# faithokamoto/panman

Measured on NVIDIA B200. Metric: fitch_sankoff_node_column_updates_per_sec, higher is better.
Workload: dtype u16 Fitch sets as 16 bit-planes

## Files before the change

panman_b200/csrc/plane_math.h:

```cpp
#pragma once
#include <stdint.h>

#if defined(__CUDACC__)
#define PMB_HD __host__ __device__ __forceinline__
#else
#define PMB_HD inline
#endif

namespace pmb {

PMB_HD void decode16(const uint32_t c[4], uint32_t d[16]) {
    uint32_t lo[4], hi[4];
    lo[0] = ~c[0] & ~c[1];
    lo[1] = c[0] & ~c[1];
    lo[2] = ~c[0] & c[1];
    lo[3] = c[0] & c[1];
    hi[0] = ~c[2] & ~c[3];
    hi[1] = c[2] & ~c[3];
    hi[2] = ~c[2] & c[3];
    hi[3] = c[2] & c[3];
#pragma unroll
    for (int k = 0; k < 16; k++) d[k] = lo[k & 3] & hi[k >> 2];
}

// ... 10 lines not shown

PMB_HD void lowest16(const uint32_t X[16], uint32_t code[4], uint32_t& any) {
    uint32_t any2[8], any4[4], any8[2];
    uint32_t b0_2[4], b0_3[2], b1_3[2];
#pragma unroll
    for (int j = 0; j < 8; j++) any2[j] = X[2 * j] | X[2 * j + 1];
#pragma unroll
    for (int j = 0; j < 4; j++) {
        any4[j] = any2[2 * j] | any2[2 * j + 1];
        b0_2[j] = (any2[2 * j] & ~X[4 * j]) | (~any2[2 * j] & ~X[4 * j + 2]);
    }
#pragma unroll
    for (int j = 0; j < 2; j++) {
        any8[j] = any4[2 * j] | any4[2 * j + 1];
        b0_3[j] = (any4[2 * j] & b0_2[2 * j]) | (~any4[2 * j] & b0_2[2 * j + 1]);
        b1_3[j] = (any4[2 * j] & ~any2[4 * j]) | (~any4[2 * j] & ~any2[4 * j + 2]);
    }
    any = any8[0] | any8[1];
    code[0] = (any8[0] & b0_3[0]) | (~any8[0] & b0_3[1]);
    code[1] = (any8[0] & b1_3[0]) | (~any8[0] & b1_3[1]);
    code[2] = (any8[0] & ~any4[0]) | (~any8[0] & ~any4[2]);
    code[3] = ~any8[0];
#pragma unroll
    for (int b = 0; b < 4; b++) code[b] &= any;
}

PMB_HD uint32_t differs4(const uint32_t a[4], const uint32_t b[4]) {
    return (a[0] ^ b[0]) | (a[1] ^ b[1]) | (a[2] ^ b[2]) | (a[3] ^ b[3]);
}

PMB_HD uint32_t less4(const uint32_t a[4], const uint32_t b[4]) {
    uint32_t lt = 0;
#pragma unroll
    for (int k = 0; k < 4; k++) {
        uint32_t x = a[k] ^ b[k];
        lt = (x & b[k]) | (~x & lt);
    }
    return lt;
}


struct FitchFold {
    uint32_t A[16], O[16];
    PMB_HD void reset() {
#pragma unroll
        for (int k = 0; k < 16; k++) { A[k] = 0xFFFFFFFFu; O[k] = 0; }
    }
    PMB_HD void add_set(const uint32_t S[16]) {
#pragma unroll
        for (int k = 0; k < 16; k++) { A[k] &= S[k]; O[k] |= S[k]; }
    }
    PMB_HD void add_leaf(const uint32_t c[4], uint32_t present) {
        uint32_t d[16];
        decode16(c, d);
#pragma unroll
        for (int k = 0; k < 16; k++) { A[k] &= d[k] & present; O[k] |= d[k] & present; }
    }
    PMB_HD void finish(uint32_t S[16]) const {
        uint32_t nz = 0;
#pragma unroll
        for (int k = 0; k < 16; k++) nz |= A[k];
#pragma unroll
        for (int k = 0; k < 16; k++) S[k] = A[k] | (O[k] & ~nz);
    }
};

PMB_HD void fitch_leaf_leaf(const uint32_t c1[4], const uint32_t c2[4], uint32_t S[16]) {
    uint32_t d1[16], d2[16];
    decode16(c1, d1);
    decode16(c2, d2);
    const uint32_t ne = differs4(c1, c2);
#pragma unroll
    for (int k = 0; k < 16; k++) S[k] = d1[k] | (d2[k] & ne);
}
PMB_HD void fitch_leaf_set(const uint32_t c[4], const uint32_t X[16], uint32_t S[16]) {
    uint32_t d[16];
    decode16(c, d);
    const uint32_t hit = mux16(X, c);
#pragma unroll
    for (int k = 0; k < 16; k++) S[k] = d[k] | (X[k] & ~hit);
}
PMB_HD void fitch_set_set(const uint32_t X[16], const uint32_t Y[16], uint32_t S[16]) {
    uint32_t nz = 0;
#pragma unroll
    for (int k = 0; k < 16; k++) nz |= X[k] & Y[k];
#pragma unroll
    for (int k = 0; k < 16; k++) S[k] = (X[k] & Y[k]) | ((X[k] | Y[k]) & ~nz);
}

struct FitchInterval {
    uint32_t lo[16], hi[16];
    PMB_HD void reset() {
#pragma unroll
        for (int k = 0; k < 16; k++) { lo[k] = 0; hi[k] = 0xFFFFFFFFu; }
    }
    PMB_HD void step(const uint32_t A[16], const uint32_t O[16]) {
        uint32_t sure = 0, maybe = 0, one = 0, two = 0;
#pragma unroll
        for (int k = 0; k < 16; k++) {
            const uint32_t h = hi[k] & A[k];
            sure |= lo[k] & A[k];
            maybe |= h;
            two |= one & h;
            one |= h;
        }
        const uint32_t single = one & ~two, uni = ~maybe, either = maybe & ~sure;
#pragma unroll
        for (int k = 0; k < 16; k++) {
            const uint32_t l = lo[k], h = hi[k];
            lo[k] = (sure & l & A[k]) | (uni & (l | O[k])) | (either & single & h & A[k] & (l | O[k]));
            hi[k] = (sure & h & A[k]) | (~sure & (h | O[k]));
        }
    }
    PMB_HD uint32_t open() const {
        uint32_t d = 0;
#pragma unroll
        for (int k = 0; k < 16; k++) d |= lo[k] ^ hi[k];
        return d;
    }
};

PMB_HD void fitch_candidates_step(uint32_t Q[16], const uint32_t S[16]) {
    uint32_t outside = 0;
#pragma unroll
    for (int k = 0; k < 16; k++) outside |= Q[k] & ~S[k];
    uint32_t seen = 0;
#pragma unroll
    for (int k = 0; k < 16; k++) {
        const uint32_t lowest = S[k] & ~seen;
        seen |= S[k];
        Q[k] = (Q[k] & S[k]) | (outside & lowest);
    }
}
PMB_HD uint32_t candidates_open(const uint32_t Q[16]) {
    uint32_t one = 0, two = 0;
#pragma unroll
    for (int k = 0; k < 16; k++) {
        two |= one & Q[k];
        one |= Q[k];
    }
    return ~one | two;
}
PMB_HD void encode16(const uint32_t d[16], uint32_t c[4]) {
    c[0] = c[1] = c[2] = c[3] = 0;
#pragma unroll
    for (int k = 0; k < 16; k++) {
        if (k & 1) c[0] |= d[k];
        if (k & 2) c[1] |= d[k];
        if (k & 4) c[2] |= d[k];
        if (k & 8) c[3] |= d[k];
    }
}

PMB_HD void fitch_assign(const uint32_t S[16], const uint32_t P[4], uint32_t pvis, uint32_t F[4], uint32_t& vis) {
    uint32_t low[4], any;
    lowest16(S, low, any);
    uint32_t hit = mux16(S, P);
    vis = pvis & any;
#pragma unroll
    for (int b = 0; b < 4; b++) F[b] = ((hit & P[b]) | (~hit & low[b])) & vis;
}

PMB_HD void fitch_assign_root(const uint32_t S[16], const uint32_t ov[4], uint32_t ov_valid, uint32_t colmask,
                              uint32_t F[4], uint32_t& vis) {
    uint32_t low[4], any;
    lowest16(S, low, any);
    vis = (ov_valid | any) & colmask;
#pragma unroll
    for (int b = 0; b < 4; b++) F[b] = ((ov_valid & ov[b]) | (~ov_valid & low[b])) & vis;
}

PMB_HD void mutation_type(const uint32_t P[4], const uint32_t F[4], uint32_t& t0, uint32_t& t1) {
    uint32_t pgap = ~(P[0] | P[1] | P[2] | P[3]);
    uint32_t fgap = ~(F[0] | F[1] | F[2] | F[3]);
    t1 = pgap;
    t0 = ~pgap & fgap;
}


PMB_HD uint32_t sankoff_none(const uint32_t G[16], const uint32_t H[16]) { return H[0] & ~G[0]; }

template <int B>
struct SankoffFold {
    uint32_t cnt[16][B];
    uint32_t all_none;
    PMB_HD void reset() {
#pragma unroll
        for (int k = 0; k < 16; k++)
#pragma unroll
            for (int b = 0; b < B; b++) cnt[k][b] = 0;
        all_none = 0xFFFFFFFFu;
    }
    PMB_HD void add_bit(int k, uint32_t g) {
        uint32_t carry = g;
#pragma unroll
        for (int b = 0; b < B; b++) {
            uint32_t t = cnt[k][b] & carry;
            cnt[k][b] ^= carry;
            carry = t;
        }
    }
    PMB_HD void add_set(const uint32_t G[16], uint32_t none) {
#pragma unroll
        for (int k = 0; k < 16; k++) add_bit(k, G[k] & ~none);
        all_none &= none;
    }
    PMB_HD void add_leaf(const uint32_t c[4], uint32_t present) {
        uint32_t d[16];
        decode16(c, d);
#pragma unroll
        for (int k = 0; k < 16; k++) add_bit(k, ~d[k] & present);
        all_none &= ~present;
    }
    PMB_HD void finish(uint32_t G[16], uint32_t H[16]) const {
        uint32_t alive[16];
        uint32_t minbit[B];
#pragma unroll
        for (int k = 0; k < 16; k++) alive[k] = 0xFFFFFFFFu;
#pragma unroll
        for (int b = B - 1; b >= 0; b--) {
            uint32_t anyzero = 0;
#pragma unroll
            for (int k = 0; k < 16; k++) anyzero |= alive[k] & ~cnt[k][b];
            minbit[b] = ~anyzero;
#pragma unroll
            for (int k = 0; k < 16; k++) alive[k] &= ~(anyzero & cnt[k][b]);
        }
        uint32_t mp1[B];
        uint32_t carry = 0xFFFFFFFFu;
#pragma unroll
        for (int b = 0; b < B; b++) {
            mp1[b] = minbit[b] ^ carry;
            carry &= minbit[b];
        }
#pragma unroll
        for (int k = 0; k < 16; k++) {
            uint32_t eq1 = ~carry;
#pragma unroll
            for (int b = 0; b < B; b++) eq1 &= ~(cnt[k][b] ^ mp1[b]);
            G[k] = ~alive[k];
            H[k] = ~alive[k] & ~eq1;
        }
        H[0] |= all_none;
        G[0] &= ~all_none;
    }
};

PMB_HD void sankoff_pair(const uint32_t g1[16], uint32_t none1, const uint32_t g2[16], uint32_t none2, uint32_t G[16],
                         uint32_t H[16]) {
    uint32_t any0 = 0, all2 = 0xFFFFFFFFu;
#pragma unroll
    for (int k = 0; k < 16; k++) {
        const uint32_t a = g1[k] & ~none1, b = g2[k] & ~none2;
        any0 |= ~(a | b);
        all2 &= a & b;
    }
#pragma unroll
    for (int k = 0; k < 16; k++) {
        const uint32_t a = g1[k] & ~none1, b = g2[k] & ~none2;
        G[k] = (any0 & (a | b)) | (~any0 & a & b & ~all2);
        H[k] = any0 & a & b;
    }
    const uint32_t both_none = none1 & none2;
    H[0] |= both_none;
    G[0] &= ~both_none;
}
PMB_HD void sankoff_leaf_g(const uint32_t c[4], uint32_t present, uint32_t g[16]) {
    uint32_t d[16];
    decode16(c, d);
#pragma unroll
    for (int k = 0; k < 16; k++) g[k] = ~d[k] & present;
}

PMB_HD void sankoff_assign(const uint32_t G[16], const uint32_t H[16], const uint32_t P[4], uint32_t pvis,
                           uint32_t F[4], uint32_t& vis) {
    uint32_t zero[16], z[4], any;
#pragma unroll
    for (int k = 0; k < 16; k++) zero[k] = ~G[k];
    lowest16(zero, z, any);
    uint32_t gt0 = mux16(G, P), eq2 = mux16(H, P);
    uint32_t keep = ~gt0 | (~eq2 & less4(P, z));
    vis = pvis & ~sankoff_none(G, H);
#pragma unroll
    for (int b = 0; b < 4; b++) F[b] = ((keep & P[b]) | (~keep & z[b])) & vis;
}

PMB_HD void sankoff_candidates_step(uint32_t Q[16], const uint32_t G[16], const uint32_t H[16]) {
    uint32_t to_z = 0, seen = 0;
    uint32_t keep[16], zhot[16];
#pragma unroll
    for (int k = 0; k < 16; k++) {
        const uint32_t zero = ~G[k];
        zhot[k] = zero & ~seen;
        seen |= zero;
        const uint32_t one = G[k] & ~H[k];
        keep[k] = Q[k] & (zero | (one & ~seen));
        to_z |= Q[k] & (H[k] | (one & seen));
    }
#pragma unroll
    for (int k = 0; k < 16; k++) Q[k] = keep[k] | (to_z & zhot[k]);
}

PMB_HD void sankoff_assign_root(const uint32_t G[16], const uint32_t H[16], const uint32_t ov[4], uint32_t ov_valid,
                                uint32_t colmask, uint32_t F[4], uint32_t& vis, uint32_t& undefined) {
    uint32_t zero[16], z[4], any;
#pragma unroll
    for (int k = 0; k < 16; k++) zero[k] = ~G[k];
    lowest16(zero, z, any);
    uint32_t none = sankoff_none(G, H);
    undefined = none & ~ov_valid & colmask;
    vis = (ov_valid | ~none) & colmask;
#pragma unroll
    for (int b = 0; b < 4; b++) F[b] = ((ov_valid & ov[b]) | (~ov_valid & z[b])) & vis;
// ... 4 lines not shown
```

panman_b200/csrc/pmb_api.cu:

```cuda
#include <cuda_runtime.h>

#include <algorithm>
#include <cstdio>
#include <cstdlib>
#include <cstring>
#include <string>
#include <vector>

#include "../../include/panman_b200.h"
#include "pmb_kernels.cuh"
#include "pmb_runs.h"
#include "tree_program.h"

using namespace pmb;

namespace {

struct DevBuf;
static bool g_canary = getenv("PMB_DEBUG_CANARY") != nullptr && getenv("PMB_DEBUG_CANARY")[0] == '1';
static std::vector<DevBuf*> g_canary_bufs;
constexpr size_t CANARY = 256;

struct DevBuf {
    void* p = nullptr;
    size_t cap = 0;
    void* raw = nullptr;
    cudaError_t ensure(size_t bytes) {
        if (bytes <= cap) return cudaSuccess;
        release();
        if (!g_canary) {
            cudaError_t e = cudaMalloc(&p, bytes);
            if (e == cudaSuccess) cap = bytes;
            return e;
        }
        const size_t body = (bytes + 255) / 256 * 256;
        cudaError_t e = cudaMalloc(&raw, body + 2 * CANARY);
        if (e != cudaSuccess) return e;
        cudaMemset(raw, 0xC5, CANARY);
        cudaMemset(static_cast<char*>(raw) + CANARY, 0xAB, body);
        cudaMemset(static_cast<char*>(raw) + CANARY + body, 0xC5, CANARY);
        cudaDeviceSynchronize();
        p = static_cast<char*>(raw) + CANARY;
        cap = bytes;
        g_canary_bufs.push_back(this);
        return cudaSuccess;
    }
    void release() {
        if (raw) {
            cudaFree(raw);
            g_canary_bufs.erase(std::remove(g_canary_bufs.begin(), g_canary_bufs.end(), this), g_canary_bufs.end());
        } else if (p) {
            cudaFree(p);
        }
        p = raw = nullptr;
        cap = 0;
    }
    long long bad_guard_bytes() const {
        if (!raw) return 0;
        const size_t body = (cap + 255) / 256 * 256;
        std::vector<unsigned char> g(2 * CANARY);
        cudaMemcpy(g.data(), raw, CANARY, cudaMemcpyDeviceToHost);
        cudaMemcpy(g.data() + CANARY, static_cast<char*>(raw) + CANARY + body, CANARY, cudaMemcpyDeviceToHost);
        long long bad = 0;
        for (unsigned char c : g) bad += c != 0xC5;
        return bad;
    }
    template <class T> T* as() const { return static_cast<T*>(p); }
};

struct HostBuf {
    void* p = nullptr;
    size_t cap = 0;
    cudaError_t ensure(size_t bytes) {
        if (bytes <= cap) return cudaSuccess;
        if (p) cudaFreeHost(p);
        p = nullptr;
        cap = 0;
        cudaError_t e = cudaMallocHost(&p, bytes ? bytes : 1);
        if (e == cudaSuccess) cap = bytes;
        return e;
    }
    void release() {
        if (p) cudaFreeHost(p);
        p = nullptr;
        cap = 0;
    }
    template <class T> T* as() const { return static_cast<T*>(p); }
};

}

struct pmb_ctx {
    int device = 0;
    cudaStream_t stream = nullptr;
    cudaEvent_t ev[4] = {nullptr, nullptr, nullptr, nullptr};
    std::string err;

    int64_t opt_chunk_nodes = 0;
    int64_t opt_staging_records = 0;
    int64_t opt_inline_nodes = 3;
    int64_t opt_schedule = 1;
    int64_t opt_trace = 0;
    DevBuf d_trace;
    std::vector<unsigned long long> h_trace;
    DevBuf d_scan_state;
    int64_t opt_target_items = 0;
    int64_t opt_reserve_sms = 0;
    int64_t opt_bwd_tail = 20;
    int64_t opt_col_groups = 0;
    static constexpr int MAX_GROUPS = 16;
    cudaStream_t gstream[MAX_GROUPS] = {};
    cudaEvent_t gev_fwd[MAX_GROUPS] = {}, gev_done[MAX_GROUPS] = {}, ev_fork = nullptr;
    cudaEvent_t ev_slab_copied[2] = {nullptr, nullptr}, ev_slab_packed[2] = {nullptr, nullptr};
    int n_sms = 0;
    size_t total_mem = 0;
    struct Occupancy { const void* kernel; size_t smem; int per_sm; };
    std::vector<Occupancy> occupancy;
    unsigned int epoch = 0;
    unsigned int dir_clean_epoch = 0;
    unsigned int dir2_clean_epoch = 0;
    bool sticky_dirty = false;
    bool state_dirty = true;
    unsigned int pack_seq = 0;
    bool async_pending = false;
    bool upload_pending = false;
    cudaStream_t cstream = nullptr;
    cudaStream_t bstream = nullptr;
    cudaEvent_t ev_fwd_done = nullptr, ev_bwd_done = nullptr, ev_compact_done[2] = {nullptr, nullptr};
    DevBuf d_sets2, d_dir2, d_staging2;
    int64_t opt_grid_pct = 0;
    int cur_grid_pct = 100;
    int64_t opt_overlap = 1;
    unsigned int run_seq = 0;
    cudaStream_t merge_stream = nullptr;
    cudaEvent_t ev_merge = nullptr, ev_rm = nullptr;
    cudaStream_t rm_stream = nullptr;
    DevBuf d_merge_err, d_mblock_sums, d_mrel;
    bool async_phase_events = true;
    int async_groups = 1;

    bool have_tree = false;
    int32_t n_nodes = 0, root = -1;
    std::vector<int32_t> child_off, child_idx, leaf_row;
    TreeProgram prog;
    int32_t prog_chunk_nodes = -1, prog_inline_nodes = -1, prog_tail = -1;
    struct ProgramSlot {
        int32_t k = -1, inl = -1, tail = -1;
        unsigned long long used = 0;
        TreeProgram prog;
        DevBuf bufs[9];
    };
    std::vector<ProgramSlot> prog_cache;
    unsigned long long prog_clock = 0;
    static constexpr size_t PROG_CACHE_SLOTS = 6;
    DevBuf d_fwd_ops, d_refs, d_bwd_ops, d_bwd_leaves, d_chunks, d_bwd_order, d_level_order, d_row_slot, d_deps;

    bool have_input = false;
    int64_t n_cols = 0, col_base = 0;
    int32_t T = 0;
    bool have_present = false;
    DevBuf d_leaf_planes, d_present, d_colparams, d_tmp_codes, d_tmp_cols;
    pmb_ctx* lane = nullptr;
    bool is_lane = false;
    int64_t opt_lanes = 1;
    unsigned lane_seq = 0;
    pmb_ctx* last = nullptr;
    unsigned long long input_gen = 1, lane_mirror_gen = 0;
    cudaEvent_t ev_input_ready = nullptr;
    std::vector<int32_t> dfs_rows, h_dfs_slot;
    uint64_t dfs_hash = 0;
    DevBuf d_run_events, d_run_off, d_dfs_slot;

    DevBuf d_done, d_fdone, d_ticket, d_block_sums;
    DevBuf d_mcounts, d_moff, d_mpos, d_mtc;
    DevBuf d_rm_counts, d_rm_off, d_rm_pos, d_rm_info, d_rm_nucs, d_rm_wire, d_rm_flags, d_rm_oidx;
    DevBuf d_col_break;
    bool have_col_break = false;
    HostBuf h_rm_off, h_rm_pos, h_rm_info, h_rm_nucs, h_rm_wire;
    HostBuf h_pack_header;
    DevBuf d_sets, d_fstore, d_states_planes, d_dir, d_staging, d_counters, d_offsets, d_pos, d_tc,
        d_states_u8;
    unsigned long long staging_cap = 0;
    bool staging_floor_dirty = false;
    bool have_result = false;
    int last_algo = 0, last_flags = 0;
    int64_t n_mut = 0;
    pmb_timings timings{};
    HostBuf h_offsets, h_pos, h_tc, h_states, h_counters;
};

namespace {

int fail(pmb_ctx* c, int code, const std::string& msg) {
    if (c) c->err = msg;
    return code;
}

int cuda_fail(pmb_ctx* c, cudaError_t e, const char* what) {
    std::string m = std::string(what) + ": " + cudaGetErrorString(e);
    cudaGetLastError();
    return fail(c, e == cudaErrorMemoryAllocation ? PMB_ERR_OOM : PMB_ERR_CUDA, m);
}

#define PMB_CUDA(call)                                         \
    do {                                                       \
        cudaError_t e__ = (call);                              \
        if (e__ != cudaSuccess) return cuda_fail(c, e__, #call); \
    } while (0)

template <class T>
int upload_vec(pmb_ctx* c, DevBuf& buf, const std::vector<T>& v) {
    size_t bytes = std::max<size_t>(v.size() * sizeof(T), 16);
    PMB_CUDA(buf.ensure(bytes));
    if (!v.empty()) PMB_CUDA(cudaMemcpyAsync(buf.p, v.data(), v.size() * sizeof(T), cudaMemcpyHostToDevice, c->stream));
    return PMB_OK;
}

int32_t pick_chunk_nodes(const pmb_ctx* c) {
    if (c->opt_chunk_nodes > 0) return int32_t(std::min<int64_t>(c->opt_chunk_nodes, 1 << 30));
    const int64_t target_warps = c->opt_target_items > 0 ? c->opt_target_items : 148LL * 32;
    int64_t want_chunks = std::max<int64_t>(1, (target_warps + c->T - 1) / std::max(1, c->T));
    int64_t n_internal = 0;
    for (int32_t v = 0; v < c->n_nodes; v++) n_internal += c->child_off[v + 1] > c->child_off[v];
    if (c->opt_target_items <= 0 && c->opt_overlap > 0 && size_t(n_internal) * size_t(c->T) * 4096 <= (size_t(4) << 30))
        want_chunks = std::min<int64_t>(want_chunks, 160);
    int64_t k = n_internal / want_chunks;
    return int32_t(std::max<int64_t>(8, std::min<int64_t>(k, 512)));
}

int ensure_program(pmb_ctx* c) {
    int32_t k = pick_chunk_nodes(c);
    int32_t inl = int32_t(std::max<int64_t>(0, std::min<int64_t>(c->opt_inline_nodes, 1 << 20)));
    const int64_t resident_warps = int64_t(c->n_sms) * 5 * WARPS_PER_BLOCK;
    const int32_t tail = int32_t(std::min<int64_t>(1 << 30, std::max<int64_t>(0, c->opt_bwd_tail) * resident_warps / 10 / std::max(1, c->T)));
    if (k == c->prog_chunk_nodes && inl == c->prog_inline_nodes && tail == c->prog_tail) return PMB_OK;
    {
        DevBuf* cur[9] = {&c->d_fwd_ops, &c->d_refs, &c->d_bwd_ops, &c->d_bwd_leaves, &c->d_chunks, &c->d_bwd_order, &c->d_level_order,
                          &c->d_row_slot, &c->d_deps};
        auto swap_with = [&](pmb_ctx::ProgramSlot& s) {
            std::swap(s.prog, c->prog);
            for (int i = 0; i < 9; i++) std::swap(s.bufs[i], *cur[i]);
            std::swap(s.k, c->prog_chunk_nodes);
            std::swap(s.inl, c->prog_inline_nodes);
            std::swap(s.tail, c->prog_tail);
            s.used = ++c->prog_clock;
        };
        if (c->prog_chunk_nodes >= 0) {
            if (c->prog_cache.size() < pmb_ctx::PROG_CACHE_SLOTS) {
                c->prog_cache.emplace_back();
                swap_with(c->prog_cache.back());
            } else {
                size_t lru = 0;
                for (size_t i = 1; i < c->prog_cache.size(); i++)
                    if (c->prog_cache[i].used < c->prog_cache[lru].used) lru = i;
                swap_with(c->prog_cache[lru]);
                c->prog_chunk_nodes = -1;
            }
        }
        for (size_t i = 0; i < c->prog_cache.size(); i++) {
            pmb_ctx::ProgramSlot& s = c->prog_cache[i];
            if (s.k == k && s.inl == inl && s.tail == tail) {
                swap_with(s);
                if (s.k < 0) {
                    for (DevBuf& b : s.bufs) b.release();
                    c->prog_cache.erase(c->prog_cache.begin() + long(i));
                }
                return PMB_OK;
            }
        }
        c->prog_chunk_nodes = -1;
    }
    std::string e = build_tree_program(c->n_nodes, c->root, c->child_off.data(), c->child_idx.data(), c->leaf_row.data(), k,
                                       inl, &c->prog, tail);
    if (e.empty() && c->opt_chunk_nodes <= 0 && c->prog.n_chain_segments > 0 && k > 128) {
        e = build_tree_program(c->n_nodes, c->root, c->child_off.data(), c->child_idx.data(), c->leaf_row.data(), 128, inl, &c->prog,
                               tail);
    }
    if (!e.empty()) return fail(c, PMB_ERR_INVALID, e);
    int rc;
    if ((rc = upload_vec(c, c->d_fwd_ops, c->prog.fwd_ops))) return rc;
    if ((rc = upload_vec(c, c->d_refs, c->prog.refs))) return rc;
    if ((rc = upload_vec(c, c->d_bwd_ops, c->prog.bwd_ops))) return rc;
    if ((rc = upload_vec(c, c->d_bwd_leaves, c->prog.bwd_leaves))) return rc;
    if ((rc = upload_vec(c, c->d_chunks, c->prog.chunks))) return rc;
    if ((rc = upload_vec(c, c->d_bwd_order, c->prog.bwd_order))) return rc;
    if ((rc = upload_vec(c, c->d_level_order, c->prog.level_order))) return rc;
    if ((rc = upload_vec(c, c->d_row_slot, c->prog.row_slot))) return rc;
    if ((rc = upload_vec(c, c->d_deps, c->prog.deps))) return rc;
    PMB_CUDA(cudaStreamSynchronize(c->stream));
    c->prog_chunk_nodes = k;
    c->prog_inline_nodes = inl;
    c->prog_tail = tail;
    return PMB_OK;
}

int ensure_flags(pmb_ctx* c, DevBuf& buf, size_t words) {
    size_t bytes = std::max<size_t>(16, words * sizeof(unsigned int));
    if (bytes <= buf.cap) return PMB_OK;
    PMB_CUDA(buf.ensure(bytes));
    PMB_CUDA(cudaMemsetAsync(buf.p, 0, buf.cap, c->stream));
    return PMB_OK;
}

template <class K>
int launch_kernel(pmb_ctx* c, cudaStream_t stream, K kernel, size_t smem, const RunParams& rp_in, int chunk_begin, int n_chunks,
                  int* n_launches) {
    RunParams rp = rp_in;
    dim3 block(WARPS_PER_BLOCK * 32);
    long long warps = (long long)n_chunks * rp.tile_count;
    if (warps <= 0) return PMB_OK;
    unsigned blocks;
    if (rp.ticket) {
        int per_sm = -1;
        const void* key = reinterpret_cast<const void*>(kernel);
        for (const auto& e : c->occupancy)
            if (e.kernel == key && e.smem == smem) per_sm = e.per_sm;
        if (per_sm < 0) {
            PMB_CUDA(cudaOccupancyMaxActiveBlocksPerMultiprocessor(&per_sm, kernel, WARPS_PER_BLOCK * 32, smem));
            c->occupancy.push_back({key, smem, per_sm});
        }
        const long long sms = std::max<long long>(1, c->n_sms - std::max<int64_t>(0, std::min<int64_t>(c->opt_reserve_sms, c->n_sms - 1)));
        long long resident = (long long)std::max(1, per_sm) * sms;
        resident = std::max<long long>(sms, resident * std::max(1, std::min(100, c->cur_grid_pct)) / 100);
        blocks = unsigned(std::min<long long>(resident, (warps + WARPS_PER_BLOCK - 1) / WARPS_PER_BLOCK));
    } else {
        blocks = unsigned((warps + WARPS_PER_BLOCK - 1) / WARPS_PER_BLOCK);
    }
    kernel<<<blocks, block, smem, stream>>>(rp, chunk_begin, n_chunks);
    (*n_launches)++;
    return PMB_OK;
}

template <class K>
int launch_schedule(pmb_ctx* c, cudaStream_t stream, int ticket_slot, K kernel, size_t smem, RunParams rp, bool forward,
                    int* n_launches) {
    const TreeProgram& P = c->prog;
    int rc;
    if (smem > 48 * 1024) PMB_CUDA(cudaFuncSetAttribute(kernel, cudaFuncAttributeMaxDynamicSharedMemorySize, int(smem)));
    if (c->opt_schedule == 1) {
        rp.ticket = c->d_ticket.as<unsigned long long>() + ticket_slot;
        rp.order = forward ? nullptr : c->d_bwd_order.as<int>();
        rp.stage_block = 512;
        if ((rc = launch_kernel(c, stream, kernel, smem, rp, 0, int(P.chunks.size()), n_launches))) return rc;
    } else {
        rp.ticket = nullptr;
        rp.order = c->d_level_order.as<int>();
        rp.stage_block = 32;
        const int L = P.n_levels();
        for (int i = 0; i < L; i++) {
            int l = forward ? i : L - 1 - i;
            int cb = P.level_chunk_begin[l], nc = P.level_chunk_begin[l + 1] - cb;
            if ((rc = launch_kernel(c, stream, kernel, smem, rp, cb, nc, n_launches))) return rc;
        }
    }
    PMB_CUDA(cudaGetLastError());
    return PMB_OK;
}

int launch_pass(pmb_ctx* c, cudaStream_t stream, int ticket_slot, const RunParams& rp, int algo, bool forward, int* n_launches) {
    const TreeProgram& P = c->prog;
    const size_t fwd_smem = size_t(WARPS_PER_BLOCK) * (FWD_DEPTH * (2 + 4) * 32 + FWD_META_U4) * sizeof(uint4);
    const size_t fwd_smem_s = size_t(WARPS_PER_BLOCK) * (FWD_DEPTH * (2 + 5) * 32 + FWD_META_U4) * sizeof(uint4);
    const size_t bwd_smem_f = size_t(WARPS_PER_BLOCK) * FITCH_BWD_PER_WARP * sizeof(uint4);
    const size_t bwd_smem_s = size_t(WARPS_PER_BLOCK) * (BWD_DEPTH * (8 + 2) * 32 + BWD_META_U4 + BWD_STACK_U4) * sizeof(uint4);
    if (algo == PMB_ALGO_FITCH) {
        if (P.n_chain_segments > 0)
            return forward ? launch_schedule(c, stream, ticket_slot, fitch_forward_kernel<true>, fwd_smem, rp, true, n_launches)
                           : launch_schedule(c, stream, ticket_slot, fitch_backward_kernel<true>, bwd_smem_f, rp, false, n_launches);
        return forward ? launch_schedule(c, stream, ticket_slot, fitch_forward_kernel<false>, fwd_smem, rp, true, n_launches)
                       : launch_schedule(c, stream, ticket_slot, fitch_backward_kernel<false>, bwd_smem_f, rp, false, n_launches);
    }
    const bool chains = P.n_chain_segments > 0;
    if (!forward)
        return chains ? launch_schedule(c, stream, ticket_slot, sankoff_backward_kernel<true>, bwd_smem_s, rp, false, n_launches)
                      : launch_schedule(c, stream, ticket_slot, sankoff_backward_kernel<false>, bwd_smem_s, rp, false, n_launches);
#define PMB_SANKOFF_FWD(B)                                                                                                    \
    return chains ? launch_schedule(c, stream, ticket_slot, sankoff_forward_kernel<B, true>, fwd_smem_s, rp, true, n_launches) \
                  : launch_schedule(c, stream, ticket_slot, sankoff_forward_kernel<B, false>, fwd_smem_s, rp, true, n_launches)
    if (P.max_arity <= 3) PMB_SANKOFF_FWD(2);
    if (P.max_arity <= 15) PMB_SANKOFF_FWD(4);
    if (P.max_arity <= 255) PMB_SANKOFF_FWD(8);
    PMB_SANKOFF_FWD(20);
#undef PMB_SANKOFF_FWD
}

int pick_groups(const pmb_ctx* c) {
    int64_t g = c->opt_col_groups;
    if (g <= 0) g = 1;
    g = std::min<int64_t>(g, std::min<int64_t>(c->T, pmb_ctx::MAX_GROUPS));
    return int(std::max<int64_t>(1, g));
}

}

extern "C" {

const char* pmb_version(void) { return "panman_b200 0.1 (sm_100a)"; }

int pmb_create(pmb_ctx** out, int device) {
    if (!out) return PMB_ERR_INVALID;
    *out = nullptr;
    pmb_ctx* c = new pmb_ctx();
    c->device = device;
    cudaError_t e = cudaSetDevice(device);
    if (e == cudaSuccess) e = cudaStreamCreateWithFlags(&c->stream, cudaStreamNonBlocking);
    for (int i = 0; i < 4 && e == cudaSuccess; i++) e = cudaEventCreate(&c->ev[i]);
    if (e != cudaSuccess) {
        c->err = std::string("no usable CUDA device: ") + cudaGetErrorString(e);
        cudaGetLastError();
        c->stream = nullptr;
        *out = c;
        return PMB_ERR_CUDA;
    }
    for (int g = 0; g < pmb_ctx::MAX_GROUPS && e == cudaSuccess; g++) {
        e = cudaStreamCreateWithFlags(&c->gstream[g], cudaStreamNonBlocking);
        if (e == cudaSuccess) e = cudaEventCreateWithFlags(&c->gev_fwd[g], cudaEventDefault);
        if (e == cudaSuccess) e = cudaEventCreateWithFlags(&c->gev_done[g], cudaEventDefault);
    }
    if (e == cudaSuccess) e = cudaEventCreateWithFlags(&c->ev_fork, cudaEventDisableTiming);
    if (e == cudaSuccess) e = cudaEventCreateWithFlags(&c->ev_merge, cudaEventDisableTiming);
    if (e == cudaSuccess) e = cudaEventCreateWithFlags(&c->ev_fwd_done, cudaEventDisableTiming);
    if (e == cudaSuccess) e = cudaEventCreateWithFlags(&c->ev_bwd_done, cudaEventDisableTiming);
    for (int k = 0; k < 2 && e == cudaSuccess; k++) e = cudaEventCreateWithFlags(&c->ev_compact_done[k], cudaEventDisableTiming);
    if (e == cudaSuccess) {
        int lo = 0, hi = 0;
        e = cudaDeviceGetStreamPriorityRange(&lo, &hi);
        if (e == cudaSuccess) e = cudaStreamCreateWithPriority(&c->cstream, cudaStreamNonBlocking, hi);
        if (e == cudaSuccess) e = cudaStreamCreateWithPriority(&c->bstream, cudaStreamNonBlocking, hi < lo ? hi + 1 : hi);
    }
    if (e == cudaSuccess) e = cudaEventCreateWithFlags(&c->ev_rm, cudaEventDisableTiming);
    if (e == cudaSuccess) e = cudaEventCreateWithFlags(&c->ev_input_ready, cudaEventDisableTiming);
    if (e != cudaSuccess) {
        c->err = std::string("stream/event creation failed: ") + cudaGetErrorString(e);
        cudaGetLastError();
        c->stream = nullptr;
        *out = c;
        return PMB_ERR_CUDA;
    }
    cudaDeviceGetAttribute(&c->n_sms, cudaDevAttrMultiProcessorCount, device);
    if (c->n_sms <= 0) c->n_sms = 148;
    {
        size_t free_b = 0;
        if (cudaMemGetInfo(&free_b, &c->total_mem) != cudaSuccess) {
            cudaGetLastError();
            c->total_mem = size_t(64) << 30;
        }
    }
    *out = c;
    return PMB_OK;
}

static void lane_borrowed(pmb_ctx* L, DevBuf** out) {
    DevBuf* b[13] = {&L->d_fwd_ops, &L->d_refs, &L->d_bwd_ops, &L->d_bwd_leaves, &L->d_chunks, &L->d_bwd_order, &L->d_level_order,
                     &L->d_row_slot, &L->d_deps, &L->d_leaf_planes, &L->d_present, &L->d_colparams, &L->d_col_break};
    for (int i = 0; i < 13; i++) out[i] = b[i];
}

static void drop_lane(pmb_ctx* c);
void pmb_destroy(pmb_ctx* c) {
    if (!c) return;
    drop_lane(c);
    if (c->stream) {
        cudaSetDevice(c->device);
        cudaStreamSynchronize(c->stream);
        for (DevBuf* b : {&c->d_fwd_ops, &c->d_refs, &c->d_bwd_ops, &c->d_bwd_leaves, &c->d_chunks, &c->d_bwd_order,
                          &c->d_level_order, &c->d_row_slot, &c->d_deps, &c->d_block_sums, &c->d_leaf_planes,
                          &c->d_present, &c->d_colparams, &c->d_tmp_codes, &c->d_tmp_cols, &c->d_sets, &c->d_sets2, &c->d_fstore,
                          &c->d_states_planes, &c->d_dir, &c->d_staging, &c->d_counters, &c->d_offsets,
                          &c->d_pos, &c->d_tc, &c->d_states_u8, &c->d_done, &c->d_fdone, &c->d_ticket, &c->d_mcounts, &c->d_moff,
                          &c->d_mpos, &c->d_mtc, &c->d_scan_state, &c->d_trace, &c->d_rm_counts, &c->d_rm_off, &c->d_rm_pos,
                          &c->d_rm_info, &c->d_rm_nucs, &c->d_rm_wire, &c->d_rm_flags, &c->d_rm_oidx, &c->d_col_break, &c->d_merge_err, &c->d_mblock_sums, &c->d_mrel,
                          &c->d_run_events, &c->d_run_off, &c->d_dfs_slot, &c->d_dir2, &c->d_staging2})
            b->release();
        for (auto& s : c->prog_cache)
            for (DevBuf& b : s.bufs) b.release();
        for (HostBuf* b : {&c->h_offsets, &c->h_pos, &c->h_tc, &c->h_states, &c->h_counters, &c->h_pack_header, &c->h_rm_off, &c->h_rm_pos,
                           &c->h_rm_info, &c->h_rm_nucs, &c->h_rm_wire}) b->release();
        for (int i = 0; i < 4; i++)
            if (c->ev[i]) cudaEventDestroy(c->ev[i]);
        for (int g = 0; g < pmb_ctx::MAX_GROUPS; g++) {
            if (c->gev_fwd[g]) cudaEventDestroy(c->gev_fwd[g]);
            if (c->gev_done[g]) cudaEventDestroy(c->gev_done[g]);
            if (c->gstream[g]) cudaStreamDestroy(c->gstream[g]);
        }
        if (c->ev_fork) cudaEventDestroy(c->ev_fork);
        if (c->ev_merge) cudaEventDestroy(c->ev_merge);
        if (c->bstream) cudaStreamSynchronize(c->bstream);
        if (c->cstream) cudaStreamSynchronize(c->cstream);
        if (c->ev_fwd_done) cudaEventDestroy(c->ev_fwd_done);
        if (c->ev_bwd_done) cudaEventDestroy(c->ev_bwd_done);
        for (int k = 0; k < 2; k++)
            if (c->ev_compact_done[k]) cudaEventDestroy(c->ev_compact_done[k]);
        if (c->cstream) cudaStreamDestroy(c->cstream);
        if (c->bstream) cudaStreamDestroy(c->bstream);
        if (c->ev_rm) cudaEventDestroy(c->ev_rm);
        if (c->ev_input_ready) cudaEventDestroy(c->ev_input_ready);
        for (int k = 0; k < 2; k++) {
            if (c->ev_slab_copied[k]) cudaEventDestroy(c->ev_slab_copied[k]);
            if (c->ev_slab_packed[k]) cudaEventDestroy(c->ev_slab_packed[k]);
        }
        cudaStreamDestroy(c->stream);
    }
    delete c;
}

const char* pmb_last_error(const pmb_ctx* c) { return c ? c->err.c_str() : "null context"; }

void* pmb_host_alloc(size_t bytes) {
    void* p = nullptr;
    if (cudaMallocHost(&p, bytes ? bytes : 1) != cudaSuccess) {
        cudaGetLastError();
        return nullptr;
    }
    return p;
}

void pmb_host_free(void* p) {
    if (p) cudaFreeHost(p);
}

int pmb_set_option(pmb_ctx* c, const char* key, int64_t value) {
    if (!c || !key) return PMB_ERR_INVALID;
    std::string k(key);
    if (k == "chunk_nodes") c->opt_chunk_nodes = value;
    else if (k == "staging_records") {
        c->opt_staging_records = value;
        c->staging_cap = 0;
    }
    else if (k == "inline_nodes") c->opt_inline_nodes = value;
    else if (k == "schedule") c->opt_schedule = value;
    else if (k == "col_groups") c->opt_col_groups = value;
    else if (k == "bwd_tail") c->opt_bwd_tail = value;
    else if (k == "reserve_sms") c->opt_reserve_sms = value;
    else if (k == "target_items") c->opt_target_items = value;
    else if (k == "trace") c->opt_trace = value;
    else if (k == "overlap") c->opt_overlap = value;
    else if (k == "grid_pct") c->opt_grid_pct = value;
    else if (k == "lanes") c->opt_lanes = value;
    else return fail(c, PMB_ERR_INVALID, "unknown option " + k);
    return PMB_OK;
}

static int set_tree_impl(pmb_ctx* c, int32_t n_nodes, int32_t root, const int32_t* child_offsets, const int32_t* child_index,
                         const int32_t* leaf_row) {
    if (!c) return PMB_ERR_INVALID;
    if (!c->stream) return fail(c, PMB_ERR_CUDA, "no usable CUDA device (pmb_create failed); there is no CPU fallback");
    if (n_nodes < 2 || !child_offsets || !child_index || !leaf_row) return fail(c, PMB_ERR_INVALID, "bad tree arguments");
    TreeProgram probe;
    std::string e = build_tree_program(n_nodes, root, child_offsets, child_index, leaf_row, 64, 3, &probe);
    if (!e.empty()) return fail(c, PMB_ERR_INVALID, e);
    c->n_nodes = n_nodes;
    c->root = root;
    c->child_off.assign(child_offsets, child_offsets + n_nodes + 1);
    c->child_idx.assign(child_index, child_index + child_offsets[n_nodes]);
    c->leaf_row.assign(leaf_row, leaf_row + n_nodes);
    c->dfs_rows = dfs_leaf_rows(n_nodes, root, child_offsets, child_index, leaf_row);
    c->dfs_hash = leaf_order_hash(c->dfs_rows);
    c->prog = std::move(probe);
    c->prog_chunk_nodes = -1;
    if (!c->prog_cache.empty()) {
        cudaDeviceSynchronize();
        for (auto& s : c->prog_cache)
            for (DevBuf& b : s.bufs) b.release();
        c->prog_cache.clear();
    }
    c->have_tree = true;
    c->have_input = false;
    c->have_result = false;
    c->last = nullptr;
    c->input_gen++;
    if (c->lane && c->lane->stream) {
        cudaStreamSynchronize(c->lane->stream);
        cudaStreamSynchronize(c->lane->bstream);
        cudaStreamSynchronize(c->lane->cstream);
        c->lane->have_input = false;
        c->lane->have_result = false;
    }
    return PMB_OK;
}

#define PMB_GUARDED(c, expr)                                                       \
    try {                                                                          \
        return (expr);                                                             \
    } catch (const std::bad_alloc&) {                                              \
        return fail((c), PMB_ERR_OOM, "out of host memory");                       \
    } catch (const std::exception& ex) {                                           \
        return fail((c), PMB_ERR_INVALID, std::string("internal: ") + ex.what()); \
    }

int pmb_set_tree(pmb_ctx* c, int32_t n_nodes, int32_t root, const int32_t* child_offsets, const int32_t* child_index,
                 const int32_t* leaf_row) {
    PMB_GUARDED(c, set_tree_impl(c, n_nodes, root, child_offsets, child_index, leaf_row))
}

static int upload_impl(pmb_ctx* c, int64_t n_cols, int32_t n_rows, const uint8_t* leaf_codes_4bit, int64_t row_stride_bytes,
                       const uint8_t* leaf_present, const uint8_t* parent_code, const int8_t* root_override,
                       const int8_t* fwd_root_ref, int64_t col_base, bool sync, const pmb_runs* runs = nullptr,
                       int64_t runs_col_begin = 0) {
    if (!c) return PMB_ERR_INVALID;
    if (!c->stream) return fail(c, PMB_ERR_CUDA, "no usable CUDA device; there is no CPU fallback");
    if (!c->have_tree) return fail(c, PMB_ERR_NO_TREE, "pmb_set_tree has not been called");
    if (n_cols <= 0 || (!leaf_codes_4bit && !runs) || !parent_code) return fail(c, PMB_ERR_INVALID, "bad input arguments");
    if (n_rows != c->prog.n_rows) return fail(c, PMB_ERR_INVALID, "n_rows does not match the tree's leaf count");
    if (!runs && row_stride_bytes < (n_cols + 1) / 2) return fail(c, PMB_ERR_INVALID, "row_stride_bytes too small");
    if (runs) {
        if (runs->order_hash != c->dfs_hash || runs->n_rows != n_rows)
            return fail(c, PMB_ERR_INVALID, "the batch was encoded for another tree (leaf order differs)");
        if (runs_col_begin < 0 || runs_col_begin % TILE_COLS != 0 || runs_col_begin + n_cols > runs->n_cols ||
            (runs_col_begin + n_cols != runs->n_cols && n_cols % TILE_COLS != 0))
            return fail(c, PMB_ERR_INVALID, "a column range of an encoded batch starts on a multiple of 1024 and ends on one or with the batch");
    }
    if (n_cols > (int64_t(1) << 40)) return fail(c, PMB_ERR_INVALID, "n_cols too large");
    PMB_CUDA(cudaSetDevice(c->device));
    PMB_CUDA(cudaStreamWaitEvent(c->stream, c->ev_bwd_done, 0));
    for (int k = 0; k < 2; k++) PMB_CUDA(cudaStreamWaitEvent(c->stream, c->ev_compact_done[k], 0));
    if (c->lane && c->lane->stream) {
        PMB_CUDA(cudaStreamWaitEvent(c->stream, c->lane->ev_bwd_done, 0));
        for (int k = 0; k < 2; k++) PMB_CUDA(cudaStreamWaitEvent(c->stream, c->lane->ev_compact_done[k], 0));
    }
    c->last = nullptr;
    c->input_gen++;
    c->have_input = false;
    c->have_result = false;
    c->have_col_break = false;
    c->staging_floor_dirty = true;
    c->n_cols = n_cols;
    c->col_base = col_base;
    c->T = int32_t((n_cols + TILE_COLS - 1) / TILE_COLS);
    int rc = ensure_program(c);
    if (rc) return rc;
    const size_t plane_bytes = size_t(n_rows) * c->T * 32 * sizeof(uint4);
    PMB_CUDA(c->d_leaf_planes.ensure(plane_bytes));
    PMB_CUDA(c->d_tmp_cols.ensure(size_t(n_cols) * 3));
    uint8_t* t = c->d_tmp_cols.as<uint8_t>();
    PMB_CUDA(cudaMemcpyAsync(t, parent_code, size_t(n_cols), cudaMemcpyDefault, c->stream));
    if (root_override) PMB_CUDA(cudaMemcpyAsync(t + n_cols, root_override, size_t(n_cols), cudaMemcpyDefault, c->stream));
    if (fwd_root_ref) PMB_CUDA(cudaMemcpyAsync(t + 2 * n_cols, fwd_root_ref, size_t(n_cols), cudaMemcpyDefault, c->stream));
    PMB_CUDA(c->d_colparams.ensure(size_t(c->T) * 128 * sizeof(uint4)));
    {
        long long threads = (long long)c->T * 32 * 32;
        unsigned blocks = unsigned((threads + 255) / 256);
        pack_colparams_kernel<<<blocks, 256, 0, c->stream>>>(t, root_override ? reinterpret_cast<const int8_t*>(t + n_cols) : nullptr,
                                                             fwd_root_ref ? reinterpret_cast<const int8_t*>(t + 2 * n_cols) : nullptr,
                                                             n_cols, c->T, c->d_colparams.as<uint4>());
    }
    PMB_CUDA(cudaGetLastError());
    bool on_device = false;
    if (!runs) {
        cudaPointerAttributes attr{};
        if (cudaPointerGetAttributes(&attr, leaf_codes_4bit) == cudaSuccess)
            on_device = attr.type == cudaMemoryTypeDevice || attr.type == cudaMemoryTypeManaged;
        else
            cudaGetLastError();
    }
    auto pack = [&](const uint8_t* src, int64_t src_stride, int32_t r0, int32_t nr) {
        long long total = (long long)nr * c->T * 32;
        unsigned blocks = unsigned((total + 255) / 256);
        pack_leaves_kernel<<<blocks, 256, 0, c->stream>>>(src, src_stride, r0, nr, n_rows, n_cols, c->T, c->d_row_slot.as<int>(),
                                                          c->d_leaf_planes.as<uint4>());
    };
    if (runs) {
        const long long n_items = (long long)c->T * runs->n_seg, item0 = (runs_col_begin / TILE_COLS) * runs->n_seg;
        const long long ev_base = runs->item_off[item0], n_ev = runs->item_off[item0 + n_items] - ev_base;
        PMB_CUDA(c->d_run_events.ensure(size_t(std::max<long long>(n_ev, 4)) * sizeof(uint32_t)));
        PMB_CUDA(c->d_run_off.ensure(size_t(n_items + 1) * sizeof(long long)));
        PMB_CUDA(c->d_dfs_slot.ensure(size_t(n_rows) * sizeof(int)));
        c->h_dfs_slot.resize(size_t(n_rows));
        for (int32_t i = 0; i < n_rows; i++) c->h_dfs_slot[size_t(i)] = c->prog.row_slot[size_t(c->dfs_rows[size_t(i)])];
        PMB_CUDA(cudaMemcpyAsync(c->d_run_off.p, runs->item_off + item0, size_t(n_items + 1) * sizeof(long long), cudaMemcpyHostToDevice, c->stream));
        PMB_CUDA(cudaMemcpyAsync(c->d_dfs_slot.p, c->h_dfs_slot.data(), size_t(n_rows) * sizeof(int), cudaMemcpyHostToDevice, c->stream));
        const int n_slabs = int(std::max<long long>(1, std::min<long long>(std::min<long long>(8, c->T), n_ev * 4 / (4 << 20))));
        cudaStream_t copy = c->gstream[0];
        for (int k = 0; k < 2; k++)
            if (!c->ev_slab_copied[k]) PMB_CUDA(cudaEventCreateWithFlags(&c->ev_slab_copied[k], cudaEventDisableTiming));
        PMB_CUDA(cudaEventRecord(c->ev_fork, c->stream));
        PMB_CUDA(cudaStreamWaitEvent(copy, c->ev_fork, 0));
        for (int sl = 0; sl < n_slabs; sl++) {
            const long long ia = (long long)c->T * sl / n_slabs * runs->n_seg, ib = (long long)c->T * (sl + 1) / n_slabs * runs->n_seg;
            const long long ea = runs->item_off[item0 + ia] - ev_base, eb = runs->item_off[item0 + ib] - ev_base;
            if (eb > ea) {
                PMB_CUDA(cudaMemcpyAsync(c->d_run_events.as<uint32_t>() + ea, runs->events + ev_base + ea, size_t(eb - ea) * sizeof(uint32_t),
                                         cudaMemcpyHostToDevice, copy));
                PMB_CUDA(cudaEventRecord(c->ev_slab_copied[sl & 1], copy));
                PMB_CUDA(cudaStreamWaitEvent(c->stream, c->ev_slab_copied[sl & 1], 0));
            }
            if (ib > ia) {
                const unsigned blocks = unsigned(((ib - ia) * 32 + 255) / 256);
                expand_runs_kernel<<<blocks, 256, 0, c->stream>>>(c->d_run_events.as<uint32_t>(), c->d_run_off.as<long long>(), ev_base, ia, ib,
                                                                  runs->n_seg, runs->seg_rows, n_rows, c->d_dfs_slot.as<int>(),
                                                                  c->d_colparams.as<uint4>(), c->d_leaf_planes.as<uint4>());
            }
        }
        PMB_CUDA(cudaEventRecord(c->ev_fork, copy));
        PMB_CUDA(cudaStreamWaitEvent(c->stream, c->ev_fork, 0));
    } else if (on_device) {
        pack(leaf_codes_4bit, row_stride_bytes, 0, n_rows);
    } else {
        const size_t row_bytes = size_t((n_cols + 1) / 2), pitch = (row_bytes + 15) / 16 * 16;
        const size_t slab_budget = size_t(32) << 20;
        const int32_t slab_rows = int32_t(std::max<size_t>(1, std::min<size_t>(size_t(n_rows), slab_budget / pitch)));
        const size_t slab_bytes = size_t(slab_rows) * pitch;
        PMB_CUDA(c->d_tmp_codes.ensure(2 * slab_bytes));
        cudaStream_t copy = c->gstream[0];
        for (int k = 0; k < 2; k++) {
            if (!c->ev_slab_copied[k]) PMB_CUDA(cudaEventCreateWithFlags(&c->ev_slab_copied[k], cudaEventDisableTiming));
            if (!c->ev_slab_packed[k]) PMB_CUDA(cudaEventCreateWithFlags(&c->ev_slab_packed[k], cudaEventDisableTiming));
        }
        PMB_CUDA(cudaEventRecord(c->ev_fork, c->stream));
        PMB_CUDA(cudaStreamWaitEvent(copy, c->ev_fork, 0));
        const bool tight = size_t(row_stride_bytes) == pitch;
        int slab = 0;
        for (int32_t r0 = 0; r0 < n_rows; r0 += slab_rows, slab++) {
            const int k = slab & 1;
            const int32_t nr = std::min(slab_rows, n_rows - r0);
            uint8_t* buf = c->d_tmp_codes.as<uint8_t>() + size_t(k) * slab_bytes;
            if (slab >= 2) PMB_CUDA(cudaStreamWaitEvent(copy, c->ev_slab_packed[k], 0));
            const uint8_t* src = leaf_codes_4bit + size_t(r0) * size_t(row_stride_bytes);
            if (tight)
                PMB_CUDA(cudaMemcpyAsync(buf, src, size_t(nr - 1) * pitch + row_bytes, cudaMemcpyHostToDevice, copy));
            else
                PMB_CUDA(cudaMemcpy2DAsync(buf, pitch, src, size_t(row_stride_bytes), row_bytes, size_t(nr), cudaMemcpyHostToDevice, copy));
            PMB_CUDA(cudaEventRecord(c->ev_slab_copied[k], copy));
            PMB_CUDA(cudaStreamWaitEvent(c->stream, c->ev_slab_copied[k], 0));
            pack(buf, int64_t(pitch), r0, nr);
            PMB_CUDA(cudaEventRecord(c->ev_slab_packed[k], c->stream));
        }
    }
    PMB_CUDA(cudaGetLastError());
    c->have_present = leaf_present != nullptr;
    if (leaf_present) {
        std::vector<uint8_t> tmp(static_cast<size_t>(n_rows)), by_slot(static_cast<size_t>(n_rows));
        PMB_CUDA(cudaMemcpy(tmp.data(), leaf_present, size_t(n_rows), cudaMemcpyDefault));
        for (int32_t r = 0; r < n_rows; r++) by_slot[c->prog.row_slot[r]] = tmp[r];
        PMB_CUDA(c->d_present.ensure(size_t(n_rows)));
        PMB_CUDA(cudaMemcpy(c->d_present.p, by_slot.data(), size_t(n_rows), cudaMemcpyHostToDevice));
    }
    PMB_CUDA(cudaEventRecord(c->ev_input_ready, c->stream));
    if (sync) PMB_CUDA(cudaStreamSynchronize(c->stream));
    c->upload_pending = !sync;
    c->have_input = true;
    return PMB_OK;
}

int pmb_upload_nuc(pmb_ctx* c, int64_t n_cols, int32_t n_rows, const uint8_t* leaf_codes_4bit, int64_t row_stride_bytes,
                   const uint8_t* leaf_present, const uint8_t* parent_code, const int8_t* root_override,
                   const int8_t* fwd_root_ref, int64_t col_base) {
    PMB_GUARDED(c, upload_impl(c, n_cols, n_rows, leaf_codes_4bit, row_stride_bytes, leaf_present, parent_code, root_override,
                               fwd_root_ref, col_base, true))
}

int pmb_upload_nuc_async(pmb_ctx* c, int64_t n_cols, int32_t n_rows, const uint8_t* leaf_codes_4bit, int64_t row_stride_bytes,
                         const uint8_t* leaf_present, const uint8_t* parent_code, const int8_t* root_override,
                         const int8_t* fwd_root_ref, int64_t col_base) {
    PMB_GUARDED(c, upload_impl(c, n_cols, n_rows, leaf_codes_4bit, row_stride_bytes, leaf_present, parent_code, root_override,
                               fwd_root_ref, col_base, false))
}

static int run_impl(pmb_ctx* c, int algo, int flags, bool async) {
    if (!c) return PMB_ERR_INVALID;
    if (!c->stream) return fail(c, PMB_ERR_CUDA, "no usable CUDA device; there is no CPU fallback");
    if (!c->have_tree) return fail(c, PMB_ERR_NO_TREE, "pmb_set_tree has not been called");
    if (!c->have_input) return fail(c, PMB_ERR_NO_INPUT, "pmb_upload_nuc has not been called");
    if (algo != PMB_ALGO_FITCH && algo != PMB_ALGO_SANKOFF) return fail(c, PMB_ERR_INVALID, "unknown algo");
    PMB_CUDA(cudaSetDevice(c->device));
    c->have_result = false;
    const TreeProgram& P = c->prog;
    const size_t T = size_t(c->T);
    const size_t set_bytes_per = (algo == PMB_ALGO_FITCH ? 128 : 256) * sizeof(uint4);
    const size_t set_bytes = size_t(P.n_internal) * T * set_bytes_per;
    bool overlap = c->opt_overlap > 0 && c->opt_schedule == 1 && pick_groups(c) == 1 && set_bytes <= std::min(size_t(48) << 30, c->total_mem / 4);
    if (overlap && set_bytes > c->d_sets2.cap && set_bytes > (size_t(8) << 30)) {
        size_t free_b = 0, total_b = 0;
        const size_t need = set_bytes + (set_bytes > c->d_sets.cap ? set_bytes - c->d_sets.cap : 0) + (size_t(16) << 30);
        if (cudaMemGetInfo(&free_b, &total_b) != cudaSuccess) {
            cudaGetLastError();
            overlap = false;
        } else if (free_b + c->d_sets2.cap < need) {
            overlap = false;
        }
    }
    if (set_bytes > c->d_sets.cap || (overlap && set_bytes > c->d_sets2.cap)) {
        PMB_CUDA(cudaStreamSynchronize(c->bstream));
        PMB_CUDA(cudaStreamSynchronize(c->cstream));
    }
    PMB_CUDA(c->d_sets.ensure(set_bytes));
    if (overlap) PMB_CUDA(c->d_sets2.ensure(set_bytes));
    PMB_CUDA(c->d_fstore.ensure(std::max<size_t>(16, size_t(P.n_fslots) * T * FSLOT_WORDS * sizeof(uint32_t))));
    const bool want_states = flags & PMB_FLAG_WANT_STATES;
    if (want_states) PMB_CUDA(c->d_states_planes.ensure(size_t(P.n_nodes) * T * 64 * sizeof(uint4)));
    const size_t dir_bytes = size_t(P.n_nodes) * T * sizeof(unsigned long long);
    if (dir_bytes > c->d_dir.cap) c->dir_clean_epoch = 0;
    PMB_CUDA(c->d_dir.ensure(dir_bytes));
    const bool dbl = overlap;
    if (dbl) {
        if (dir_bytes > c->d_dir2.cap) c->dir2_clean_epoch = 0;
        PMB_CUDA(c->d_dir2.ensure(dir_bytes));
    }
    if (!c->d_counters.p) {
        PMB_CUDA(c->d_counters.ensure(128));
        c->state_dirty = true;
    }
    PMB_CUDA(c->h_counters.ensure(128));
    if (!c->d_ticket.p) c->state_dirty = true;
    PMB_CUDA(c->d_ticket.ensure(128 * sizeof(unsigned long long)));
    {
        int rcf;
        if ((rcf = ensure_flags(c, c->d_done, size_t(P.n_internal) * T))) return rcf;
        if ((rcf = ensure_flags(c, c->d_fdone, size_t(std::max(1, P.n_fslots)) * T))) return rcf;
    }
    PMB_CUDA(c->d_offsets.ensure(size_t(P.n_nodes + 1) * sizeof(long long)));
    if (c->staging_cap == 0 || c->staging_floor_dirty) {
        unsigned long long cells = (unsigned long long)P.n_nodes * (unsigned long long)c->n_cols;
        unsigned long long cap = c->opt_staging_records > 0 ? (unsigned long long)c->opt_staging_records
                                                            : std::max<unsigned long long>(1ull << 20, cells / 32) +
                                                                  (unsigned long long)c->n_sms * 8 * WARPS_PER_BLOCK * 512ull;
        c->staging_cap = c->opt_staging_records > 0 && c->staging_cap == 0 ? cap : std::max(c->staging_cap, cap);
        c->staging_floor_dirty = false;
    }

    RunParams rp{};
    rp.fwd_ops = c->d_fwd_ops.as<FwdOp>();
    rp.refs = c->d_refs.as<uint32_t>();
    rp.bwd_ops = c->d_bwd_ops.as<BwdOp>();
    rp.bwd_leaves = c->d_bwd_leaves.as<BwdLeaf>();
    rp.chunks = c->d_chunks.as<Chunk>();
    rp.deps = c->d_deps.as<int>();
    rp.leaf_planes = c->d_leaf_planes.as<uint4>();
    rp.leaf_present = c->have_present ? c->d_present.as<uint8_t>() : nullptr;
    const int parity = int(c->run_seq & 1u);
    const bool second = dbl && parity;
    rp.sets = (overlap && parity) ? c->d_sets2.as<uint4>() : c->d_sets.as<uint4>();
    rp.fstore = c->d_fstore.as<uint32_t>();
    rp.order = nullptr;
    rp.stage_block = 512;
    rp.colparams = c->d_colparams.as<uint4>();
    rp.states = want_states ? c->d_states_planes.as<uint4>() : nullptr;
    rp.dir = second ? c->d_dir2.as<unsigned long long>() : c->d_dir.as<unsigned long long>();
    unsigned long long* const run_words = c->d_counters.as<unsigned long long>() + (second ? 8 : 0);
    rp.pool_count = run_words;
    rp.error = reinterpret_cast<unsigned int*>(run_words + 1);
    rp.done = c->d_done.as<unsigned int>();
    rp.fdone = c->d_fdone.as<unsigned int>();
    rp.ticket = nullptr;
    rp.T = c->T;
    rp.n_ops = P.n_internal;
    rp.n_rows = P.n_rows;
    rp.n_fslots = std::max(1, P.n_fslots);
    rp.n_refs_total = int(P.refs.size());
    rp.flags = ((flags & PMB_FLAG_BLOCK_MODE) ? RUN_BLOCK_MODE : 0) | (want_states ? RUN_WANT_STATES : 0);

    int n_launches = 0;
    int rc = 0;
    const size_t trace_items = size_t(P.chunks.size()) * T;
    rp.trace = nullptr;
    if (c->opt_trace) {
        PMB_CUDA(c->d_trace.ensure(trace_items * 2 * 4 * sizeof(unsigned long long)));
        PMB_CUDA(cudaMemsetAsync(c->d_trace.p, 0, trace_items * 2 * 4 * sizeof(unsigned long long), c->stream));
        rp.trace = c->d_trace.as<unsigned long long>();
    }
    const int G = pick_groups(c);
    auto group_range = [&](int g, int* tb, int* tc) {
        *tb = int((long long)c->T * g / G);
        *tc = int((long long)c->T * (g + 1) / G) - *tb;
    };
    if (c->state_dirty) {
        PMB_CUDA(cudaStreamSynchronize(c->bstream));
        PMB_CUDA(cudaStreamSynchronize(c->cstream));
        PMB_CUDA(cudaMemsetAsync(c->d_ticket.p, 0, 128 * sizeof(unsigned long long), c->stream));
        PMB_CUDA(cudaMemsetAsync(c->d_counters.p, 0, 128, c->stream));
        unsigned int* init = c->h_counters.as<unsigned int>() + 16;
        init[0] = 0xFFFFFFFFu;
        PMB_CUDA(cudaMemcpyAsync(c->d_counters.as<char>() + 12, init, 4, cudaMemcpyHostToDevice, c->stream));
        PMB_CUDA(cudaMemcpyAsync(c->d_counters.as<char>() + 20, init, 4, cudaMemcpyHostToDevice, c->stream));
        PMB_CUDA(cudaMemcpyAsync(c->d_counters.as<char>() + 64 + 12, init, 4, cudaMemcpyHostToDevice, c->stream));
        c->dir_clean_epoch = 0;
        c->dir2_clean_epoch = 0;
    }
    if (c->sticky_dirty && !c->async_pending) {
        unsigned int* init = c->h_counters.as<unsigned int>() + 18;
        init[0] = 0u;
        init[1] = 0xFFFFFFFFu;
        PMB_CUDA(cudaMemcpyAsync(c->d_counters.as<char>() + 16, init, 8, cudaMemcpyHostToDevice, c->stream));
        c->sticky_dirty = false;
    }
    c->state_dirty = true;
    PMB_CUDA(cudaStreamWaitEvent(c->stream, c->ev_compact_done[parity], 0));
    if (!overlap) PMB_CUDA(cudaStreamWaitEvent(c->stream, c->ev_bwd_done, 0));
    PMB_CUDA(cudaEventRecord(c->ev[0], c->stream));
    rp.epoch = ++c->epoch;
    const unsigned int fwd_epoch = rp.epoch;
    const int ticket_set = 64 * parity;
    c->run_seq++;
    cudaStream_t const bwd_stream = G == 1 ? c->bstream : c->stream;
    c->cur_grid_pct = c->opt_grid_pct > 0 ? int(c->opt_grid_pct)
                                          : (async && overlap && P.n_chain_segments == 0 ? (c->T < 24 ? 70 : 80) : 100);
    unsigned int* const run_error = rp.error;
    unsigned int* const fwd_error = reinterpret_cast<unsigned int*>(c->d_counters.as<unsigned long long>() + 2);
    for (int attempt = 0;; attempt++) {
        PMB_CUDA(c->d_staging.ensure(size_t(c->staging_cap) * sizeof(uint16_t)));
        if (dbl) PMB_CUDA(c->d_staging2.ensure(size_t(c->staging_cap) * sizeof(uint16_t)));
        PMB_CUDA(c->d_pos.ensure(size_t(c->staging_cap) * sizeof(int32_t)));
        PMB_CUDA(c->d_tc.ensure(size_t(c->staging_cap)));
        rp.staging = second ? c->d_staging2.as<uint16_t>() : c->d_staging.as<uint16_t>();
        rp.staging_cap = c->staging_cap;
        const unsigned int bwd_epoch = ++c->epoch;
        rp.dir_tag = bwd_epoch & DIR_TAG_MASK;
        const bool phase_events = !async || G > 1;
        if (G > 1) PMB_CUDA(cudaEventRecord(c->ev_fork, c->stream));
        for (int g = 0; g < G; g++) {
            cudaStream_t st = G == 1 ? c->stream : c->gstream[g];
            if (G > 1) PMB_CUDA(cudaStreamWaitEvent(st, c->ev_fork, 0));
            group_range(g, &rp.tile_begin, &rp.tile_count);
            rp.trace_base = (unsigned long long)P.chunks.size() * rp.tile_begin;
            if (attempt == 0) {
                rp.epoch = fwd_epoch;
                rp.error = fwd_error;
                if ((rc = launch_pass(c, st, ticket_set + 2 * g, rp, algo, true, &n_launches))) return rc;
                rp.error = run_error;
            }
            if (phase_events) PMB_CUDA(cudaEventRecord(c->gev_fwd[g], st));
            if (G == 1) {
                PMB_CUDA(cudaEventRecord(c->ev_fwd_done, st));
                st = bwd_stream;
                PMB_CUDA(cudaStreamWaitEvent(st, c->ev_fwd_done, 0));
            }
            for (int k = 0; k < 2; k++)
                if (!dbl || k == parity) PMB_CUDA(cudaStreamWaitEvent(st, c->ev_compact_done[k], 0));
            unsigned int& clean_epoch = second ? c->dir2_clean_epoch : c->dir_clean_epoch;
            if (g == 0 && (clean_epoch == 0 || bwd_epoch - clean_epoch >= DIR_TAG_MASK - 8u)) {
                DevBuf& dirbuf = second ? c->d_dir2 : c->d_dir;
                PMB_CUDA(cudaMemsetAsync(dirbuf.p, 0, dirbuf.cap, st));
                clean_epoch = bwd_epoch;
                if (G > 1) {
                    PMB_CUDA(cudaEventRecord(c->ev_fork, st));
                    for (int g2 = 1; g2 < G; g2++) PMB_CUDA(cudaStreamWaitEvent(c->gstream[g2], c->ev_fork, 0));
                }
            }
            rp.epoch = bwd_epoch;
            rp.trace_base = trace_items + (unsigned long long)P.chunks.size() * rp.tile_begin;
            if ((rc = launch_pass(c, st, ticket_set + 2 * g + 1 + 32 * (attempt & 1), rp, algo, false, &n_launches))) return rc;
            if (phase_events) PMB_CUDA(cudaEventRecord(c->gev_done[g], st));
            if (G > 1) PMB_CUDA(cudaStreamWaitEvent(c->stream, c->gev_done[g], 0));
        }
        if (phase_events) PMB_CUDA(cudaEventRecord(c->ev[2], bwd_stream));
        c->async_phase_events = phase_events;
        PMB_CUDA(cudaEventRecord(c->ev_bwd_done, bwd_stream));
        PMB_CUDA(cudaStreamWaitEvent(c->cstream, c->ev_bwd_done, 0));
        {
            const unsigned long long n_entries = (unsigned long long)P.n_nodes * (unsigned long long)c->T;
            const unsigned groups = unsigned((n_entries + CPT_GROUP - 1) / CPT_GROUP);
            if (size_t(groups) * 12 + 16 > c->d_scan_state.cap) PMB_CUDA(cudaStreamSynchronize(c->cstream));
            PMB_CUDA(c->d_scan_state.ensure(size_t(groups) * 12 + 16));
            unsigned long long* gprefix = c->d_scan_state.as<unsigned long long>();
            unsigned int* gtotals = reinterpret_cast<unsigned int*>(gprefix + groups);
            compact_count_kernel<<<(groups + 7) / 8, 256, 0, c->cstream>>>(n_entries, rp.dir, rp.dir_tag, gtotals, groups);
            compact_scan_kernel<<<1, 1024, 0, c->cstream>>>(gtotals, int(groups), gprefix, c->d_offsets.as<long long>() + P.n_nodes);
            compact_copy_kernel<<<groups, CPT_GROUP, 0, c->cstream>>>(
                P.n_nodes, c->T, gprefix, c->d_offsets.as<long long>(), rp.dir, rp.dir_tag, rp.staging, c->col_base,
                c->d_pos.as<int32_t>(), c->d_tc.as<uint8_t>(), c->d_counters.as<unsigned long long>(), run_words, rp.staging_cap,
                c->d_ticket.as<unsigned long long>() + ticket_set, 64);
            n_launches += 2;
            n_launches += 1;
        }
        PMB_CUDA(cudaGetLastError());
        PMB_CUDA(cudaEventRecord(c->ev[3], c->cstream));
        PMB_CUDA(cudaEventRecord(c->ev_compact_done[parity], c->cstream));
        c->state_dirty = false;
        if (async) {
            c->async_pending = true;
            c->async_groups = G;
            c->timings.n_launches = n_launches;
            c->timings.n_levels = P.n_levels();
            c->last_algo = algo;
            c->last_flags = flags;
            c->n_mut = -1;
            c->have_result = true;
            return PMB_OK;
        }
        PMB_CUDA(cudaMemcpyAsync(c->h_counters.p, c->d_counters.as<char>() + 32, 16, cudaMemcpyDeviceToHost, c->cstream));
        PMB_CUDA(cudaMemcpyAsync(c->h_counters.as<char>() + 16, c->d_offsets.as<long long>() + P.n_nodes, 8, cudaMemcpyDeviceToHost,
                                 c->cstream));
        PMB_CUDA(cudaMemcpyAsync(c->h_counters.as<char>() + 24, c->d_counters.as<char>() + 16, 4, cudaMemcpyDeviceToHost, c->cstream));
        PMB_CUDA(cudaStreamSynchronize(c->cstream));
        PMB_CUDA(cudaStreamSynchronize(c->stream));
        c->upload_pending = false;
        unsigned long long total = *c->h_counters.as<unsigned long long>();
        unsigned int eflags = c->h_counters.as<unsigned int>()[2], ecol = c->h_counters.as<unsigned int>()[3];
        eflags |= c->h_counters.as<unsigned int>()[6] & 2u;
        if (eflags || total > c->staging_cap) c->sticky_dirty = true;
        if (eflags & 2u) return fail(c, PMB_ERR_INTERNAL, "scheduler watchdog fired: a dependency flag never arrived");
        if (eflags & 1u) {
            char buf[160];
            snprintf(buf, sizeof buf, "Sankoff root has no finite cost at column %lld and no root override was given",
                     (long long)ecol + (long long)c->col_base);
            return fail(c, PMB_ERR_SANKOFF_ROOT, buf);
        }
        if (total > c->staging_cap) {
            if (attempt >= 4) return fail(c, PMB_ERR_INTERNAL, "staging pool overflow persisted");
            c->staging_cap = total + total / 8 + (unsigned long long)c->n_sms * 8 * WARPS_PER_BLOCK * 512ull;
            continue;
        }
        c->n_mut = *reinterpret_cast<long long*>(c->h_counters.as<char>() + 16);
        break;
    }
    float to_bwd_end = 0.f;
    c->timings.forward_ms = 0.f;
    for (int g = 0; g < G; g++) {
        float f = 0.f;
        PMB_CUDA(cudaEventElapsedTime(&f, c->ev[0], c->gev_fwd[g]));
        c->timings.forward_ms = std::max(c->timings.forward_ms, f);
    }
    PMB_CUDA(cudaEventElapsedTime(&to_bwd_end, c->ev[0], c->ev[2]));
    c->timings.backward_ms = to_bwd_end - c->timings.forward_ms;
    PMB_CUDA(cudaEventElapsedTime(&c->timings.compact_ms, c->ev[2], c->ev[3]));
    PMB_CUDA(cudaEventElapsedTime(&c->timings.total_ms, c->ev[0], c->ev[3]));
    if (c->opt_trace) {
        c->h_trace.resize(trace_items * 2 * 4);
        PMB_CUDA(cudaMemcpy(c->h_trace.data(), c->d_trace.p, c->h_trace.size() * sizeof(unsigned long long), cudaMemcpyDeviceToHost));
    }
    c->timings.n_launches = n_launches;
    c->timings.n_levels = P.n_levels();
    c->last_algo = algo;
    c->last_flags = flags;
    c->have_result = true;
    return PMB_OK;
}

static pmb_ctx* result_ctx(pmb_ctx* c) { return c && c->last ? c->last : c; }
static const pmb_ctx* result_cctx(const pmb_ctx* c) { return c && c->last ? c->last : c; }
static bool lane_pending(const pmb_ctx* c) { return c && c->lane && (c->lane->async_pending || c->lane->upload_pending); }

int pmb_run_resident(pmb_ctx* c, int algo, int flags) {
    if (c && (c->async_pending || lane_pending(c))) {
        int rc = pmb_wait(c);
        if (rc) return rc;
    }
    if (c) c->last = nullptr;
    return run_impl(c, algo, flags, false);
}

static bool lanes_apply(const pmb_ctx* c, int algo, int flags) {
    if (!c || !c->stream || c->is_lane || c->opt_lanes <= 0 || !c->have_tree || !c->have_input) return false;
    if (c->opt_schedule != 1 || c->opt_overlap <= 0 || c->opt_trace || (flags & PMB_FLAG_WANT_STATES)) return false;
    if (algo != PMB_ALGO_FITCH && algo != PMB_ALGO_SANKOFF) return false;
    if (c->prog.n_chain_segments > 0 || pick_groups(c) != 1) return false;
    const size_t set_bytes = size_t(c->prog.n_internal) * size_t(c->T) * (algo == PMB_ALGO_FITCH ? 128 : 256) * sizeof(uint4);
    return set_bytes <= std::min(size_t(4) << 30, c->total_mem / 16);
}

static int run_on_lane(pmb_ctx* c, int algo, int flags) {
    if (!c->lane) {
        pmb_ctx* L = nullptr;
        int rc = pmb_create(&L, c->device);
        if (rc) {
            c->err = std::string("second pass lane: ") + (L ? L->err : std::string("out of memory"));
            if (L) pmb_destroy(L);
            return rc;
        }
        L->is_lane = true;
        L->opt_lanes = 0;
        c->lane = L;
    }
    pmb_ctx* L = c->lane;
    PMB_CUDA(cudaSetDevice(c->device));
    L->opt_chunk_nodes = c->opt_chunk_nodes;
    L->opt_staging_records = c->opt_staging_records;
    L->opt_inline_nodes = c->opt_inline_nodes;
    L->opt_schedule = c->opt_schedule;
    L->opt_target_items = c->opt_target_items;
    L->opt_reserve_sms = c->opt_reserve_sms;
    L->opt_bwd_tail = c->opt_bwd_tail;
    L->opt_col_groups = c->opt_col_groups;
    L->opt_grid_pct = c->opt_grid_pct;
    L->opt_overlap = c->opt_overlap;
    if (L->lane_mirror_gen != c->input_gen) {
        L->n_nodes = c->n_nodes;
        L->root = c->root;
        L->prog = c->prog;
        L->have_tree = true;
        L->n_cols = c->n_cols;
        L->col_base = c->col_base;
        L->T = c->T;
        L->have_present = c->have_present;
        L->have_input = true;
        L->staging_floor_dirty = true;
        DevBuf* dst[13];
        lane_borrowed(L, dst);
        DevBuf* src[13];
        lane_borrowed(c, src);
        for (int i = 0; i < 13; i++) {
            dst[i]->p = src[i]->p;
            dst[i]->cap = src[i]->cap;
            dst[i]->raw = nullptr;
        }
        L->have_col_break = c->have_col_break;
        L->lane_mirror_gen = c->input_gen;
    }
    L->staging_cap = std::max(L->staging_cap, c->staging_cap);
    PMB_CUDA(cudaStreamWaitEvent(L->stream, c->ev_input_ready, 0));
    int rc = run_impl(L, algo, flags, true);
    if (rc) {
        c->err = L->err;
        return rc;
    }
    c->last = L;
    c->have_result = true;
    c->last_algo = algo;
    c->last_flags = flags;
    return PMB_OK;
}

static void drop_lane(pmb_ctx* c) {
    if (!c->lane) return;
    pmb_ctx* L = c->lane;
    if (L->stream) {
        cudaSetDevice(c->device);
        cudaStreamSynchronize(L->stream);
        cudaStreamSynchronize(L->bstream);
        cudaStreamSynchronize(L->cstream);
    }
    DevBuf* b[13];
    lane_borrowed(L, b);
    for (DevBuf* x : b) { x->p = nullptr; x->raw = nullptr; x->cap = 0; }
    if (c->last == L) c->last = nullptr;
    c->lane = nullptr;
    pmb_destroy(L);
}

int pmb_run_resident_async(pmb_ctx* c, int algo, int flags) {
    if (lanes_apply(c, algo, flags)) {
        if (c->lane_seq++ & 1u) {
            int rc;
            try {
                rc = run_on_lane(c, algo, flags);
            } catch (const std::bad_alloc&) {
                rc = PMB_ERR_OOM;
            } catch (const std::exception& ex) {
                return fail(c, PMB_ERR_INVALID, std::string("internal: ") + ex.what());
            }
            if (rc != PMB_ERR_OOM) return rc;
            drop_lane(c);
            c->opt_lanes = 0;
            c->err.clear();
        }
    } else if (c) {
        c->lane_seq = 0;
    }
    if (c) c->last = nullptr;
    return run_impl(c, algo, flags, true);
}

static int wait_one(pmb_ctx* c);

int pmb_wait(pmb_ctx* c) {
    if (!c) return PMB_ERR_INVALID;
    int rc = wait_one(c);
    if (c->lane && c->lane->stream) {
        const int rc2 = wait_one(c->lane);
        if (rc2 && !rc) {
            c->err = c->lane->err;
            rc = rc2;
        }
    }
    return rc;
}

int pmb_join(pmb_ctx* c) {
    if (!c) return PMB_ERR_INVALID;
    if (!c->stream) return fail(c, PMB_ERR_CUDA, "no usable CUDA device; there is no CPU fallback");
    PMB_CUDA(cudaSetDevice(c->device));
    PMB_CUDA(cudaStreamWaitEvent(c->stream, c->ev[3], 0));
    if (c->lane && c->lane->stream) PMB_CUDA(cudaStreamWaitEvent(c->stream, c->lane->ev[3], 0));
    return PMB_OK;
}

static int wait_one(pmb_ctx* c) {
    if (!c) return PMB_ERR_INVALID;
    if (!c->stream) return fail(c, PMB_ERR_CUDA, "no usable CUDA device; there is no CPU fallback");
    if (!c->async_pending) {
        if (c->upload_pending) {
            PMB_CUDA(cudaSetDevice(c->device));
            PMB_CUDA(cudaStreamSynchronize(c->stream));
            c->upload_pending = false;
        }
        return PMB_OK;
    }
    PMB_CUDA(cudaSetDevice(c->device));
    c->upload_pending = false;
    const int N = c->prog.n_nodes;
    PMB_CUDA(cudaStreamSynchronize(c->stream));
    PMB_CUDA(cudaMemcpyAsync(c->h_counters.p, c->d_counters.as<char>() + 32, 8, cudaMemcpyDeviceToHost, c->cstream));
    PMB_CUDA(cudaMemcpyAsync(c->h_counters.as<char>() + 16, c->d_counters.as<char>() + 16, 8, cudaMemcpyDeviceToHost, c->cstream));
    PMB_CUDA(cudaMemcpyAsync(c->h_counters.as<char>() + 32, c->d_offsets.as<long long>() + N, 8, cudaMemcpyDeviceToHost, c->cstream));
    PMB_CUDA(cudaStreamSynchronize(c->cstream));
    c->async_pending = false;
    const unsigned int sticky = c->h_counters.as<unsigned int>()[4], scol = c->h_counters.as<unsigned int>()[5];
    unsigned int sticky_init[2] = {0u, 0xFFFFFFFFu};
    PMB_CUDA(cudaMemcpy(c->d_counters.as<char>() + 16, sticky_init, 8, cudaMemcpyHostToDevice));
    if (sticky & 2u) { c->have_result = false; return fail(c, PMB_ERR_INTERNAL, "scheduler watchdog fired: a dependency flag never arrived"); }
    if (sticky & 1u) {
        char buf[160];
        snprintf(buf, sizeof buf, "Sankoff root has no finite cost at column %lld and no root override was given",
                 (long long)scol + (long long)c->col_base);
        c->have_result = false;
        return fail(c, PMB_ERR_SANKOFF_ROOT, buf);
    }
    if (sticky & 4u) {
        c->have_result = false;
        const unsigned long long total = *c->h_counters.as<unsigned long long>();
        c->staging_cap = std::max<unsigned long long>(c->staging_cap * 4, total + total / 8 + (unsigned long long)c->n_sms * 8 * WARPS_PER_BLOCK * 512ull);
        return fail(c, PMB_ERR_STAGING, "the mutation staging pool overflowed during an asynchronous run; rerun (the pool was grown)");
    }
    c->n_mut = *reinterpret_cast<long long*>(c->h_counters.as<char>() + 32);
    PMB_CUDA(cudaEventElapsedTime(&c->timings.total_ms, c->ev[0], c->ev[3]));
    c->timings.forward_ms = c->timings.backward_ms = c->timings.compact_ms = 0.f;
    if (!c->async_phase_events) return PMB_OK;
    PMB_CUDA(cudaEventElapsedTime(&c->timings.compact_ms, c->ev[2], c->ev[3]));
    float to_bwd_end = 0.f;
    for (int g = 0; g < c->async_groups; g++) {
        float f = 0.f;
        PMB_CUDA(cudaEventElapsedTime(&f, c->ev[0], c->gev_fwd[g]));
        c->timings.forward_ms = std::max(c->timings.forward_ms, f);
    }
    PMB_CUDA(cudaEventElapsedTime(&to_bwd_end, c->ev[0], c->ev[2]));
    c->timings.backward_ms = to_bwd_end - c->timings.forward_ms;
    return PMB_OK;
}

static int result_device_one(pmb_ctx* c, pmb_result* out);
int pmb_result_device(pmb_ctx* c, pmb_result* out) {
    pmb_ctx* r = result_ctx(c);
    const int rc = result_device_one(r, out);
    if (rc && r != c) c->err = r->err;
    return rc;
}
static int result_device_one(pmb_ctx* c, pmb_result* out) {
    if (!c || !out) return PMB_ERR_INVALID;
    if (!c->have_result) return fail(c, PMB_ERR_NO_INPUT, "no result: call pmb_run_resident first");
    out->n_mut = c->n_mut;
    out->n_nodes = c->prog.n_nodes;
    out->reserved = 0;
    out->node_offsets = reinterpret_cast<const int64_t*>(c->d_offsets.p);
    out->pos = c->d_pos.as<int32_t>();
    out->type_code = c->d_tc.as<uint8_t>();
    out->states = nullptr;
    out->n_cols = c->n_cols;
    return PMB_OK;
}

static int download_one(pmb_ctx* c, pmb_result* out);
int pmb_download(pmb_ctx* c, pmb_result* out) {
    if (!c || !out) return PMB_ERR_INVALID;
    if (c->stream && c->have_result && (c->async_pending || lane_pending(c))) {
        int rcw = pmb_wait(c);
        if (rcw) return rcw;
    }
    pmb_ctx* r = result_ctx(c);
    const int rc = download_one(r, out);
    if (rc && r != c) c->err = r->err;
    return rc;
}
static int download_one(pmb_ctx* c, pmb_result* out) {
    if (!c || !out) return PMB_ERR_INVALID;
    if (!c->stream) return fail(c, PMB_ERR_CUDA, "no usable CUDA device; there is no CPU fallback");
    if (!c->have_result) return fail(c, PMB_ERR_NO_INPUT, "no result: call pmb_run_resident first");
    if (c->async_pending) {
        int rcw = wait_one(c);
        if (rcw) return rcw;
    }
    PMB_CUDA(cudaSetDevice(c->device));
    const size_t n = size_t(c->n_mut), N = size_t(c->prog.n_nodes);
    PMB_CUDA(c->h_offsets.ensure((N + 1) * sizeof(int64_t)));
    PMB_CUDA(c->h_pos.ensure(std::max<size_t>(n, 1) * sizeof(int32_t)));
    PMB_CUDA(c->h_tc.ensure(std::max<size_t>(n, 1)));
    PMB_CUDA(cudaMemcpyAsync(c->h_offsets.p, c->d_offsets.p, (N + 1) * sizeof(int64_t), cudaMemcpyDeviceToHost, c->cstream));
    if (n) {
        PMB_CUDA(cudaMemcpyAsync(c->h_pos.p, c->d_pos.p, n * sizeof(int32_t), cudaMemcpyDeviceToHost, c->cstream));
        PMB_CUDA(cudaMemcpyAsync(c->h_tc.p, c->d_tc.p, n, cudaMemcpyDeviceToHost, c->cstream));
    }
    out->states = nullptr;
    if (c->last_flags & PMB_FLAG_WANT_STATES) {
        const size_t cells = N * size_t(c->n_cols);
        PMB_CUDA(c->d_states_u8.ensure(cells));
        PMB_CUDA(c->h_states.ensure(cells));
        unsigned blocks = unsigned((cells + 255) / 256);
        unpack_states_kernel<<<blocks, 256, 0, c->cstream>>>(c->d_states_planes.as<uint4>(), c->prog.n_nodes, c->n_cols, c->T,
                                                            c->d_states_u8.as<uint8_t>());
        PMB_CUDA(cudaGetLastError());
        PMB_CUDA(cudaMemcpyAsync(c->h_states.p, c->d_states_u8.p, cells, cudaMemcpyDeviceToHost, c->cstream));
        out->states = c->h_states.as<uint8_t>();
    }
    PMB_CUDA(cudaStreamSynchronize(c->cstream));
    out->n_mut = c->n_mut;
    out->n_nodes = c->prog.n_nodes;
    out->reserved = 0;
    out->node_offsets = c->h_offsets.as<int64_t>();
    out->pos = c->h_pos.as<int32_t>();
    out->type_code = c->h_tc.as<uint8_t>();
    out->n_cols = c->n_cols;
    return PMB_OK;
}

int pmb_run_nuc(pmb_ctx* c, int algo, int64_t n_cols, int32_t n_rows, const uint8_t* leaf_codes_4bit, int64_t row_stride_bytes,
                const uint8_t* leaf_present, const uint8_t* parent_code, const int8_t* root_override,
                const int8_t* fwd_root_ref, int64_t col_base, int flags, pmb_result* out) {
    int rc = pmb_upload_nuc(c, n_cols, n_rows, leaf_codes_4bit, row_stride_bytes, leaf_present, parent_code, root_override,
                            fwd_root_ref, col_base);
    if (rc) return rc;
    if ((rc = pmb_run_resident(c, algo, flags))) return rc;
    return pmb_download(c, out);
}

int pmb_upload_runs(pmb_ctx* c, const pmb_runs* runs, int64_t col_begin, int64_t n_cols, const uint8_t* leaf_present,
                    const uint8_t* parent_code, const int8_t* root_override, const int8_t* fwd_root_ref, int64_t col_base) {
    if (!runs) return c ? fail(c, PMB_ERR_INVALID, "null runs") : PMB_ERR_INVALID;
    PMB_GUARDED(c, upload_impl(c, n_cols, runs->n_rows, nullptr, 0, leaf_present, parent_code, root_override, fwd_root_ref, col_base, true,
                               runs, col_begin))
}

int pmb_upload_runs_async(pmb_ctx* c, const pmb_runs* runs, int64_t col_begin, int64_t n_cols, const uint8_t* leaf_present,
                          const uint8_t* parent_code, const int8_t* root_override, const int8_t* fwd_root_ref, int64_t col_base) {
    if (!runs) return c ? fail(c, PMB_ERR_INVALID, "null runs") : PMB_ERR_INVALID;
    PMB_GUARDED(c, upload_impl(c, n_cols, runs->n_rows, nullptr, 0, leaf_present, parent_code, root_override, fwd_root_ref, col_base, false,
                               runs, col_begin))
}

int pmb_run_runs(pmb_ctx* c, int algo, const pmb_runs* runs, const uint8_t* leaf_present, const uint8_t* parent_code,
                 const int8_t* root_override, const int8_t* fwd_root_ref, int64_t col_base, int flags, pmb_result* out) {
    if (!runs) return c ? fail(c, PMB_ERR_INVALID, "null runs") : PMB_ERR_INVALID;
    int rc = pmb_upload_runs(c, runs, 0, runs->n_cols, leaf_present, parent_code, root_override, fwd_root_ref, col_base);
    if (rc) return rc;
    if ((rc = pmb_run_resident(c, algo, flags))) return rc;
    return pmb_download(c, out);
}

static int run_block_impl(pmb_ctx* c, int algo, int64_t n_blocks, int32_t n_rows, const uint8_t* leaf_block_state,
                          const int8_t* root_override, pmb_result* out) {
    if (!c || !leaf_block_state || !out || n_blocks <= 0 || n_rows <= 0) return c ? fail(c, PMB_ERR_INVALID, "bad block arguments") : PMB_ERR_INVALID;
    const int64_t stride = (n_blocks + 1) / 2;
    std::vector<uint8_t> codes4(size_t(n_rows) * size_t(stride), 0), parent(size_t(n_blocks), 0);
    for (int32_t r = 0; r < n_rows; r++)
        for (int64_t b = 0; b < n_blocks; b++) {
            const uint8_t st = leaf_block_state[size_t(r) * size_t(n_blocks) + size_t(b)];
            if (st > 2) return fail(c, PMB_ERR_INVALID, "block states are 0 (absent), 1 (forward) or 2 (reverse)");
            codes4[size_t(r) * size_t(stride) + size_t(b >> 1)] |= uint8_t(st << (4 * (b & 1)));
        }
    return pmb_run_nuc(c, algo, n_blocks, n_rows, codes4.data(), stride, nullptr, parent.data(), root_override, nullptr, 0,
                       PMB_FLAG_BLOCK_MODE, out);
}

int pmb_run_block(pmb_ctx* c, int algo, int64_t n_blocks, int32_t n_rows, const uint8_t* leaf_block_state, const int8_t* root_override,
                  pmb_result* out) {
    PMB_GUARDED(c, run_block_impl(c, algo, n_blocks, n_rows, leaf_block_state, root_override, out))
}

long long pmb_debug_trace(const pmb_ctx* c, unsigned long long* out, long long max_words) {
    if (!c || !out) return 0;
    long long n = std::min<long long>(max_words, (long long)c->h_trace.size());
// ... 88 lines not shown
    out->pos = c->d_mpos.as<int32_t>();
    out->type_code = c->d_mtc.as<uint8_t>();
    out->states = nullptr;
    out->n_cols = 0;
    return PMB_OK;
}

int pmb_merge_status(pmb_ctx* c) {
    if (!c) return PMB_ERR_INVALID;
    if (!c->stream) return fail(c, PMB_ERR_CUDA, "no usable CUDA device; there is no CPU fallback");
    if (!c->merge_stream || !c->d_merge_err.p) return PMB_OK;
    PMB_CUDA(cudaSetDevice(c->device));
    unsigned int flags = 0;
    PMB_CUDA(cudaMemcpyAsync(&flags, c->d_merge_err.p, 4, cudaMemcpyDeviceToHost, c->merge_stream));
    PMB_CUDA(cudaStreamSynchronize(c->merge_stream));
    if (!flags) return PMB_OK;
    PMB_CUDA(cudaMemsetAsync(c->d_merge_err.p, 0, 16, c->merge_stream));
    if (flags & 2u) return fail(c, PMB_ERR_INVALID, "a merged shard was packed for a different tree (node count mismatch)");
    return fail(c, PMB_ERR_CAPACITY, "a column-range shard held more records than the capacity it was packed with (or its pass "
                                     "overflowed the staging pool): it was skipped; reserve more and repeat the step");
}

int pmb_set_column_breaks(pmb_ctx* c, const uint8_t* col_break) {
    if (!c) return PMB_ERR_INVALID;
    if (!c->stream) return fail(c, PMB_ERR_CUDA, "no usable CUDA device; there is no CPU fallback");
    if (!c->have_input) return fail(c, PMB_ERR_NO_INPUT, "pmb_upload_nuc has not been called");
    PMB_CUDA(cudaSetDevice(c->device));
    c->have_col_break = false;
    if (!col_break) return PMB_OK;
    PMB_CUDA(c->d_col_break.ensure(size_t(c->n_cols)));
    PMB_CUDA(cudaMemcpyAsync(c->d_col_break.p, col_break, size_t(c->n_cols), cudaMemcpyDefault, c->stream));
    PMB_CUDA(cudaStreamSynchronize(c->stream));
    c->have_col_break = true;
    c->input_gen++;
    return PMB_OK;
}

static int merge_runs_one(pmb_ctx* c, int source, int to_host, pmb_nucmut_result* out);
int pmb_merge_runs(pmb_ctx* c, int source, int to_host, pmb_nucmut_result* out) {
    pmb_ctx* r = source == 0 ? result_ctx(c) : c;
    if (r != c) {
        if (c->async_pending || lane_pending(c)) {
            int rcw = pmb_wait(c);
            if (rcw) return rcw;
        }
        r->have_col_break = c->have_col_break;
        r->d_col_break.p = c->d_col_break.p;
        r->d_col_break.cap = c->d_col_break.cap;
        r->d_col_break.raw = nullptr;
    }
    const int rc = merge_runs_one(r, source, to_host, out);
    if (rc && r != c) c->err = r->err;
    return rc;
}
static int merge_runs_one(pmb_ctx* c, int source, int to_host, pmb_nucmut_result* out) {
    if (!c || !out || (source != 0 && source != 1)) return PMB_ERR_INVALID;
    if (!c->stream) return fail(c, PMB_ERR_CUDA, "no usable CUDA device; there is no CPU fallback");
    if (!c->have_tree) return fail(c, PMB_ERR_NO_TREE, "pmb_set_tree has not been called");
    if (source == 0 && !c->have_result) return fail(c, PMB_ERR_NO_INPUT, "no result: call pmb_run_resident first");
    if (source == 1 && (!c->d_moff.p || !c->merge_stream)) return fail(c, PMB_ERR_NO_INPUT, "no merged shards: call pmb_merge_packed first");
    PMB_CUDA(cudaSetDevice(c->device));
    if (source == 0 && c->async_pending) {
        int rcw = wait_one(c);
        if (rcw) return rcw;
    }
    cudaStream_t st = source == 0 ? c->cstream : c->merge_stream;
    if (c->rm_stream && c->rm_stream != st) PMB_CUDA(cudaStreamWaitEvent(st, c->ev_rm, 0));
    const int N = c->prog.n_nodes;
    const long long* off = source == 0 ? c->d_offsets.as<long long>() : c->d_moff.as<long long>();
    const int32_t* pos = source == 0 ? c->d_pos.as<int32_t>() : c->d_mpos.as<int32_t>();
    const uint8_t* tc = source == 0 ? c->d_tc.as<uint8_t>() : c->d_mtc.as<uint8_t>();
    const size_t cap = std::max<size_t>(1, source == 0 ? size_t(c->n_mut) : c->d_mtc.cap);
    const size_t n_blocks = (cap + RM_BLOCK - 1) / RM_BLOCK;
    const size_t scratch_bytes = n_blocks * (8 + 8 + 8 + 4) + 64;
    const bool grow = size_t(N + 1) * sizeof(long long) > c->d_rm_off.cap || cap * sizeof(int32_t) > c->d_rm_pos.cap ||
                      cap > c->d_rm_info.cap || cap * sizeof(uint32_t) > c->d_rm_nucs.cap || cap * sizeof(uint32_t) > c->d_rm_wire.cap ||
                      cap > c->d_rm_flags.cap || cap * sizeof(long long) > c->d_rm_oidx.cap || scratch_bytes > c->d_rm_counts.cap;
    if (grow && c->rm_stream) PMB_CUDA(cudaStreamSynchronize(c->rm_stream));
    PMB_CUDA(c->d_rm_off.ensure(size_t(N + 1) * sizeof(long long)));
    PMB_CUDA(c->d_rm_pos.ensure(cap * sizeof(int32_t)));
    PMB_CUDA(c->d_rm_info.ensure(cap));
    PMB_CUDA(c->d_rm_nucs.ensure(cap * sizeof(uint32_t)));
    PMB_CUDA(c->d_rm_wire.ensure(cap * sizeof(uint32_t)));
    PMB_CUDA(c->d_rm_flags.ensure(cap));
    PMB_CUDA(c->d_rm_oidx.ensure(cap * sizeof(long long)));
    PMB_CUDA(c->d_rm_counts.ensure(scratch_bytes));
    long long* last = c->d_rm_counts.as<long long>();
    long long* carry = last + n_blocks;
    unsigned long long* base = reinterpret_cast<unsigned long long*>(carry + n_blocks);
    unsigned int* counts = reinterpret_cast<unsigned int*>(base + n_blocks);
    uint8_t* flags = c->d_rm_flags.as<uint8_t>();
    const uint8_t* brk = (source == 0 && c->have_col_break) ? c->d_col_break.as<uint8_t>() : nullptr;
    PMB_CUDA(cudaMemsetAsync(flags, 0, cap, st));
    rm_mark_starts_kernel<<<(N + 255) / 256, 256, 0, st>>>(off, N, flags);
    rm_block_last_kernel<<<unsigned(n_blocks), RM_THREADS, 0, st>>>(off, N, pos, tc, flags, brk, c->col_base, last);
    rm_scan_max_kernel<<<1, 1024, 0, st>>>(last, int(n_blocks), carry);
    rm_flags_kernel<<<unsigned(n_blocks), RM_THREADS, 0, st>>>(off, N, pos, tc, flags, brk, c->col_base, carry, counts);
    compact_scan_kernel<<<1, 1024, 0, st>>>(counts, int(n_blocks), base, c->d_rm_off.as<long long>() + N);
    rm_fill_kernel<<<unsigned(n_blocks), RM_THREADS, 0, st>>>(off, N, pos, tc, flags, base, c->d_rm_oidx.as<long long>(),
                                                             c->d_rm_pos.as<int32_t>(), c->d_rm_info.as<uint8_t>(), c->d_rm_nucs.as<uint32_t>(),
                                                             c->d_rm_wire.as<uint32_t>());
    rm_node_offsets_kernel<<<(N + 255) / 256, 256, 0, st>>>(off, N, c->d_rm_oidx.as<long long>(), c->d_rm_off.as<long long>());
    PMB_CUDA(cudaGetLastError());
    PMB_CUDA(cudaEventRecord(c->ev_rm, st));
    c->rm_stream = st;
    out->n_nodes = N;
    out->reserved = 0;
    if (!to_host) {
        out->n = -1;
        out->node_offsets = reinterpret_cast<const int64_t*>(c->d_rm_off.p);
        out->nuc_position = c->d_rm_pos.as<int32_t>();
        out->mut_info = c->d_rm_info.as<uint8_t>();
        out->nucs = c->d_rm_nucs.as<uint32_t>();
        out->mut_info_wire = c->d_rm_wire.as<uint32_t>();
        return PMB_OK;
    }
    if (source == 1) {
        int rcm = pmb_merge_status(c);
        if (rcm) return rcm;
    }
    PMB_CUDA(c->h_rm_off.ensure(size_t(N + 1) * sizeof(int64_t)));
    PMB_CUDA(cudaMemcpyAsync(c->h_rm_off.p, c->d_rm_off.p, size_t(N + 1) * sizeof(int64_t), cudaMemcpyDeviceToHost, st));
    PMB_CUDA(cudaStreamSynchronize(st));
    const size_t m = size_t(c->h_rm_off.as<int64_t>()[N]);
    PMB_CUDA(c->h_rm_pos.ensure(std::max<size_t>(m, 1) * sizeof(int32_t)));
    PMB_CUDA(c->h_rm_info.ensure(std::max<size_t>(m, 1)));
    PMB_CUDA(c->h_rm_nucs.ensure(std::max<size_t>(m, 1) * sizeof(uint32_t)));
    PMB_CUDA(c->h_rm_wire.ensure(std::max<size_t>(m, 1) * sizeof(uint32_t)));
    if (m) {
        PMB_CUDA(cudaMemcpyAsync(c->h_rm_pos.p, c->d_rm_pos.p, m * sizeof(int32_t), cudaMemcpyDeviceToHost, st));
        PMB_CUDA(cudaMemcpyAsync(c->h_rm_info.p, c->d_rm_info.p, m, cudaMemcpyDeviceToHost, st));
        PMB_CUDA(cudaMemcpyAsync(c->h_rm_nucs.p, c->d_rm_nucs.p, m * sizeof(uint32_t), cudaMemcpyDeviceToHost, st));
        PMB_CUDA(cudaMemcpyAsync(c->h_rm_wire.p, c->d_rm_wire.p, m * sizeof(uint32_t), cudaMemcpyDeviceToHost, st));
        PMB_CUDA(cudaStreamSynchronize(st));
    }
    out->n = int64_t(m);
    out->node_offsets = c->h_rm_off.as<int64_t>();
    out->nuc_position = c->h_rm_pos.as<int32_t>();
    out->mut_info = c->h_rm_info.as<uint8_t>();
    out->nucs = c->h_rm_nucs.as<uint32_t>();
    out->mut_info_wire = c->h_rm_wire.as<uint32_t>();
    return PMB_OK;
}

int pmb_last_timings(const pmb_ctx* c, pmb_timings* out) {
    if (!c || !out) return PMB_ERR_INVALID;
    *out = result_cctx(c)->timings;
    return PMB_OK;
}

int64_t pmb_algorithmic_bytes(const pmb_ctx* c, int algo) {
    if (!c || !c->have_tree || !c->have_input) return 0;
    const int64_t L = c->prog.n_rows, I = c->prog.n_internal;
    const int64_t per_col = L + (algo == PMB_ALGO_SANKOFF ? 8 : 4) * I;
    const pmb_ctx* r = result_cctx(c);
    return c->n_cols * per_col + 8 * (r->have_result ? std::max<int64_t>(0, r->n_mut) : 0);
}

}
```

panman_b200/csrc/pmb_kernels.cuh:

```cuda
#pragma once
#include <cuda_runtime.h>
#include <stdint.h>

#include "plane_math.h"
#include "tree_program.h"

namespace pmb {

constexpr int TILE_COLS = 1024;
constexpr int WARPS_PER_BLOCK = 4;
constexpr unsigned FULL = 0xFFFFFFFFu;
constexpr int FSLOT_WORDS = 160;

enum : int { RUN_BLOCK_MODE = 1, RUN_WANT_STATES = 2 };

struct RunParams {
    const FwdOp* fwd_ops;
    const uint32_t* refs;
    const BwdOp* bwd_ops;
    const BwdLeaf* bwd_leaves;
    const Chunk* chunks;
    const int* deps;
    const uint4* leaf_planes;
    const uint8_t* leaf_present;
    uint4* sets;
    uint32_t* fstore;
    const uint4* colparams;
    uint4* states;
    unsigned long long* dir;
    uint16_t* staging;
    unsigned long long* pool_count;
    unsigned long long staging_cap;
    unsigned int* error;
    unsigned int* done;
    unsigned int* fdone;
    unsigned long long* ticket;
    const int* order;
    unsigned int epoch;
    unsigned int dir_tag;
    int T;
    int n_ops, n_rows, n_fslots;
    int n_refs_total;
    int flags;
    int stage_block;
    int tile_begin, tile_count;
    unsigned long long* trace;
    unsigned long long trace_base;
};

struct TraceItem {
    unsigned long long t0 = 0, w = 0;
    unsigned waited = 0;
};
__device__ __forceinline__ unsigned smid() {
    unsigned r;
    asm volatile("mov.u32 %0, %%smid;" : "=r"(r));
    return r;
}

__device__ __forceinline__ size_t set_index(const RunParams& p, unsigned op, int tile) { return (size_t)tile * p.n_ops + op; }
__device__ __forceinline__ size_t leaf_index(const RunParams& p, unsigned slot, int tile) { return (size_t)tile * p.n_rows + slot; }
__device__ __forceinline__ size_t fslot_index(const RunParams& p, unsigned f, int tile) { return (size_t)tile * p.n_fslots + f; }

__device__ __forceinline__ uint4 ld_stream(const uint4* p) { return __ldcs(p); }
__device__ __forceinline__ uint4 ld_l2(const uint4* p) { return __ldcg(p); }

__device__ __forceinline__ void load_planes16(const uint4* base, int lane, uint32_t S[16]) {
#pragma unroll
    for (int j = 0; j < 4; j++) {
        uint4 v = ld_l2(base + j * 32 + lane);
        S[4 * j + 0] = v.x; S[4 * j + 1] = v.y; S[4 * j + 2] = v.z; S[4 * j + 3] = v.w;
    }
}
__device__ __forceinline__ void store_planes16(uint4* base, int lane, const uint32_t S[16]) {
#pragma unroll
    for (int j = 0; j < 4; j++) base[j * 32 + lane] = make_uint4(S[4 * j], S[4 * j + 1], S[4 * j + 2], S[4 * j + 3]);
}
__device__ __forceinline__ void unpack16(const uint4 v[4], uint32_t S[16]) {
#pragma unroll
    for (int j = 0; j < 4; j++) { S[4 * j] = v[j].x; S[4 * j + 1] = v[j].y; S[4 * j + 2] = v[j].z; S[4 * j + 3] = v[j].w; }
}

__device__ __forceinline__ unsigned long long global_ns();
struct ItemIter {
    bool taken = false;
};
__device__ __forceinline__ bool next_item(const RunParams& p, ItemIter& it, int chunk_begin, int n_chunks, int& chunk,
                                          int& tile, int lane, TraceItem& tr) {
    unsigned long long w;
    if (p.ticket) {
        if (lane == 0) w = atomicAdd(p.ticket, 1ull);
        w = __shfl_sync(FULL, w, 0);
    } else {
        if (it.taken) return false;
        it.taken = true;
        w = (unsigned long long)blockIdx.x * WARPS_PER_BLOCK + (threadIdx.x >> 5);
    }
    if (w >= (unsigned long long)n_chunks * (unsigned long long)p.tile_count) return false;
    int c = chunk_begin + int(w / (unsigned)p.tile_count);
    chunk = p.order ? __ldg(p.order + c) : c;
    tile = p.tile_begin + int(w % (unsigned)p.tile_count);
    if (p.trace) {
        tr.t0 = global_ns();
        tr.w = w;
        tr.waited = 0;
    }
    return true;
}
__device__ __forceinline__ void trace_end(const RunParams& p, const TraceItem& tr, int chunk, int tile, int lane) {
    if (p.trace && lane == 0) {
        unsigned long long* q = p.trace + (p.trace_base + tr.w) * 4;
        q[0] = tr.t0;
        q[1] = global_ns();
        q[2] = ((unsigned long long)(unsigned)chunk << 32) | (unsigned)tile;
        q[3] = ((unsigned long long)smid() << 32) | tr.waited;
    }
}

__device__ __forceinline__ unsigned ld_acquire(const unsigned* p) {
    unsigned v;
    asm volatile("ld.acquire.gpu.global.u32 %0, [%1];" : "=r"(v) : "l"(p) : "memory");
    return v;
}
__device__ __forceinline__ void st_release(unsigned* p, unsigned v) {
    asm volatile("st.release.gpu.global.u32 [%0], %1;" ::"l"(p), "r"(v) : "memory");
}
__device__ __forceinline__ unsigned long long global_ns() {
    unsigned long long t;
    asm volatile("mov.u64 %0, %%globaltimer;" : "=l"(t));
    return t;
}

__device__ __noinline__ bool wait_flag_slow(const unsigned* flag, unsigned epoch, unsigned* error, int lane, unsigned* waited) {
    unsigned ok = 1;
    if (lane == 0) {
        unsigned long long t0 = global_ns();
        unsigned spins = 0;
        while (ld_acquire(flag) != epoch) {
            __nanosleep(64);
            if ((++spins & 255u) == 0) {
                if ((*reinterpret_cast<volatile unsigned*>(error) & 2u) || global_ns() - t0 > 20000000000ull) {
                    atomicOr(error, 2u);
                    ok = 0;
                    break;
                }
            }
        }
        *waited += unsigned(global_ns() - t0);
    }
    ok = __shfl_sync(FULL, ok, 0);
    __syncwarp();
    return ok != 0;
}
__device__ __forceinline__ bool wait_flag(const unsigned* flag, unsigned epoch, unsigned* error, int lane, TraceItem& tr) {
    unsigned v = 0;
    if (lane == 0) v = ld_acquire(flag);
    v = __shfl_sync(FULL, v, 0);
    if (v == epoch) {
        __syncwarp();
        return true;
    }
    return wait_flag_slow(flag, epoch, error, lane, &tr.waited);
}
struct DepCursor {
    int upto = 0;
};
__device__ __forceinline__ bool wait_dep(const RunParams& p, const Chunk& ck, const unsigned* done_tile, DepCursor& dc, int k,
                                         int lane, TraceItem& tr) {
    if (k < dc.upto) return true;
    unsigned long long t0 = 0;
    unsigned spins = 0;
    for (;;) {
        const int i = dc.upto + lane;
        bool ok = false;
        if (i < ck.dep_count) ok = ld_acquire(done_tile + __ldg(p.deps + ck.dep_begin + i)) == p.epoch;
        const unsigned b = __ballot_sync(FULL, ok);
        dc.upto += (b == FULL) ? 32 : (__ffs(~b) - 1);
        if (k < dc.upto) break;
// ... 31 lines not shown
struct StageCursor {
    unsigned long long base = 0;
    int left = 0;
};
__device__ __forceinline__ void emit(const RunParams& p, StageCursor& sc, int node, int tile, int lane, uint32_t mut,
                                     const uint32_t P[4], const uint32_t F[4]) {
    if (__ballot_sync(FULL, mut != 0) == 0) return;
    int cnt = __popc(mut);
    int incl = cnt;
#pragma unroll
    for (int d = 1; d < 32; d <<= 1) {
        int t = __shfl_up_sync(FULL, incl, d);
        if (lane >= d) incl += t;
    }
    const int total = __shfl_sync(FULL, incl, 31);
    if (total > sc.left) {
        const int take = max(total, p.stage_block);
        unsigned long long b = 0;
        if (lane == 0) b = atomicAdd(p.pool_count, (unsigned long long)take);
        sc.base = __shfl_sync(FULL, b, 0);
        sc.left = take;
    }
    const unsigned long long base = sc.base;
    sc.base += total;
    sc.left -= total;
    if (lane == 0)
        p.dir[(size_t)node * p.T + tile] = ((unsigned long long)p.dir_tag << DIR_TAG_SHIFT) | (base << 11) | (unsigned long long)total;
    if (base + (unsigned long long)total > p.staging_cap) return;
    uint32_t t0, t1;
    mutation_type(P, F, t0, t1);
    uint16_t* dst = p.staging + base + (incl - cnt);
    uint32_t m = mut;
    while (m) {
        int b = __ffs(m) - 1;
        m &= m - 1;
        uint32_t code = ((F[0] >> b) & 1u) | (((F[1] >> b) & 1u) << 1) | (((F[2] >> b) & 1u) << 2) | (((F[3] >> b) & 1u) << 3);
        uint32_t type = ((t0 >> b) & 1u) | (((t1 >> b) & 1u) << 1);
        *dst++ = uint16_t((lane * 32 + b) | (code << 10) | (type << 14));
    }
}

__device__ __forceinline__ void store_state(const RunParams& p, int node, int tile, int lane, const uint32_t F[4], uint32_t vis) {
    uint4* s = p.states + ((size_t)node * p.T + tile) * 64;
    s[lane] = make_uint4(F[0], F[1], F[2], F[3]);
    s[32 + lane] = make_uint4(vis, 0, 0, 0);
}

__device__ __forceinline__ void cp_async16(uint4* smem_dst, const uint4* gsrc) {
    unsigned d = (unsigned)__cvta_generic_to_shared(smem_dst);
    asm volatile("cp.async.cg.shared.global [%0], [%1], 16;" ::"r"(d), "l"(gsrc) : "memory");
}
__device__ __forceinline__ void cp_async_commit() { asm volatile("cp.async.commit_group;" ::: "memory"); }
__device__ __forceinline__ void cp_async_wait_pending(int n) {
    switch (n) {
    case 0: asm volatile("cp.async.wait_group 0;" ::: "memory"); break;
    case 1: asm volatile("cp.async.wait_group 1;" ::: "memory"); break;
    case 2: asm volatile("cp.async.wait_group 2;" ::: "memory"); break;
    case 3: asm volatile("cp.async.wait_group 3;" ::: "memory"); break;
    case 4: asm volatile("cp.async.wait_group 4;" ::: "memory"); break;
    case 5: asm volatile("cp.async.wait_group 5;" ::: "memory"); break;
    case 6: asm volatile("cp.async.wait_group 6;" ::: "memory"); break;
    default: asm volatile("cp.async.wait_group 7;" ::: "memory"); break;
    }
}

#ifndef PMB_BULK
#define PMB_BULK 0
#endif
__device__ __forceinline__ unsigned smem_addr(const void* p) { return (unsigned)__cvta_generic_to_shared(p); }
__device__ __forceinline__ void mbar_init(unsigned long long* bar, unsigned count) {
    asm volatile("mbarrier.init.shared::cta.b64 [%0], %1;" ::"r"(smem_addr(bar)), "r"(count) : "memory");
}
__device__ __forceinline__ void mbar_expect_tx(unsigned long long* bar, unsigned bytes) {
    asm volatile("mbarrier.arrive.expect_tx.shared::cta.b64 _, [%0], %1;" ::"r"(smem_addr(bar)), "r"(bytes) : "memory");
}
__device__ __forceinline__ void bulk_copy(void* smem_dst, const void* gsrc, unsigned bytes, unsigned long long* bar) {
    asm volatile("cp.async.bulk.shared::cluster.global.mbarrier::complete_tx::bytes [%0], [%1], %2, [%3];" ::"r"(smem_addr(smem_dst)),
                 "l"(gsrc), "r"(bytes), "r"(smem_addr(bar))
                 : "memory");
}
__device__ __forceinline__ void mbar_wait(unsigned long long* bar, unsigned parity) {
    asm volatile(
        "{\n"
        ".reg .pred P1;\n"
        "WAIT_%=:\n"
        "mbarrier.try_wait.parity.shared::cta.b64 P1, [%0], %1;\n"
        "@P1 bra DONE_%=;\n"
        "bra WAIT_%=;\n"
        "DONE_%=:\n"
        "}\n" ::"r"(smem_addr(bar)),
        "r"(parity)
        : "memory");
}

#ifndef PMB_BWD_DEPTH
#define PMB_BWD_DEPTH 2
#endif
#ifndef PMB_FWD_DEPTH
#define PMB_FWD_DEPTH 3
#endif
#ifndef PMB_META_OPS
#define PMB_META_OPS 16
#endif
constexpr int FWD_DEPTH = PMB_FWD_DEPTH;
constexpr int BWD_DEPTH = PMB_BWD_DEPTH;

template <int N>
__device__ __forceinline__ void cp_async_wait() { asm volatile("cp.async.wait_group %0;" ::"n"(N) : "memory"); }
template <int DEPTH>
__device__ __forceinline__ void cp_async_wait_stage(int ops_left_after) {
    if (ops_left_after >= DEPTH - 1) cp_async_wait<DEPTH - 1>();
    else cp_async_wait<0>();
}

constexpr int META_OPS = PMB_META_OPS, META_REFS = 3 * PMB_META_OPS, META_LEAVES = 2 * PMB_META_OPS;
constexpr int FWD_META_U4 = 2 * META_OPS + META_REFS / 4;
constexpr int BWD_META_U4 = 2 * META_OPS + META_LEAVES / 2;
constexpr int BWD_STACK_U4 = BWD_STACK_DEPTH * FSLOT_WORDS / 4;

struct FwdMeta {
    int4* ops;
    uint32_t* refs;
    int wb;
    unsigned rb;
};
__device__ __forceinline__ void fwd_meta_load(const RunParams& p, FwdMeta& m, int wb, int op_end, int lane) {
    __syncwarp();
    m.wb = wb;
    int4 h0 = make_int4(0, 0, 0, 0), h1 = h0;
    if (lane < META_OPS && wb + lane < op_end) {
        h0 = __ldg(reinterpret_cast<const int4*>(p.fwd_ops + wb + lane));
        h1 = __ldg(reinterpret_cast<const int4*>(p.fwd_ops + wb + lane) + 1);
    }
    if (lane < META_OPS) {
        m.ops[2 * lane] = h0;
        m.ops[2 * lane + 1] = h1;
    }
    m.rb = (unsigned)__shfl_sync(FULL, h0.x, 0);
#pragma unroll
    for (int d = lane; d < META_REFS; d += 32) {
        const unsigned i = m.rb + d;
        m.refs[d] = i < (unsigned)p.n_refs_total ? __ldg(p.refs + i) : 0u;
    }
    __syncwarp();
}
__device__ __forceinline__ uint32_t fwd_ref(const RunParams& p, const FwdMeta& m, unsigned i) {
    const unsigned d = i - m.rb;
    return d < (unsigned)META_REFS ? m.refs[d] : __ldg(p.refs + i);
}

struct BwdMeta {
    int4* ops;
    int2* leaves;
    int lo;
    unsigned lb;
};
__device__ __forceinline__ void bwd_meta_load(const RunParams& p, BwdMeta& m, int top, int op_begin, int lane) {
    __syncwarp();
    m.lo = max(op_begin, top - (META_OPS - 1));
    int4 h0 = make_int4(0, 0, 0, 0), h1 = h0;
    if (lane < META_OPS && m.lo + lane <= top) {
        h0 = __ldg(reinterpret_cast<const int4*>(p.bwd_ops + m.lo + lane));
        h1 = __ldg(reinterpret_cast<const int4*>(p.bwd_ops + m.lo + lane) + 1);
    }
    if (lane < META_OPS) {
        m.ops[2 * lane] = h0;
        m.ops[2 * lane + 1] = h1;
    }
    m.lb = (unsigned)__shfl_sync(FULL, h0.w, 0);
#pragma unroll
    for (int d = lane; d < META_LEAVES; d += 32) {
        const unsigned i = m.lb + d;
        m.leaves[d] = i < (unsigned)p.n_rows ? __ldg(reinterpret_cast<const int2*>(p.bwd_leaves + i)) : make_int2(0, 0);
    }
    __syncwarp();
}
struct BwdHead {
    int4 b0;
    int4 b1;
};
__device__ __forceinline__ int2 bwd_leaf(const RunParams& p, const BwdMeta& m, unsigned i) {
    const unsigned d = i - m.lb;
    return d < (unsigned)META_LEAVES ? m.leaves[d] : __ldg(reinterpret_cast<const int2*>(p.bwd_leaves + i));
}

struct TileCtx {
    const uint4* leaf;
    uint4* sets;
    unsigned* done;
};
template <int JROW>
__device__ __forceinline__ TileCtx tile_ctx(const RunParams& p, int tile, int lane) {
    TileCtx t;
    t.leaf = p.leaf_planes + (size_t)tile * p.n_rows * 32 + lane;
    t.sets = p.sets + (size_t)tile * p.n_ops * (JROW * 32) + lane;
    t.done = p.done + (size_t)tile * p.n_ops;
    return t;
}

__device__ __forceinline__ bool fwd_set_prefetched(uint32_t ref, int op) {
    return (ref & REF_EXT) || int(ref & REF_IDX_MASK) + FWD_DEPTH <= op;
}
template <int JS, int JROW>
__device__ __forceinline__ bool fwd_issue_set(const RunParams& p, const Chunk& ck, const TileCtx& tc, DepCursor& dc, uint4* st,
                                              uint32_t ref, uint32_t row_idx, int op, int lane, TraceItem& tr) {
    if (!fwd_set_prefetched(ref, op)) return true;
    if (ref & REF_EXT) {
        if (!wait_dep(p, ck, tc.done, dc, int(ref & REF_IDX_MASK), lane, tr)) return false;
    }
    const uint4* row = tc.sets + (size_t)row_idx * (JROW * 32);
#pragma unroll
    for (int j = 0; j < JS; j++) cp_async16(st + (2 + j) * 32, row + j * 32);
    return true;
}
template <int JS, int JROW>
__device__ __forceinline__ bool fwd_issue(const RunParams& p, const Chunk& ck, const FwdMeta& m, const TileCtx& tc, DepCursor& dc,
                                          uint4* st, int op, int lane, TraceItem& tr) {
    const int4 w0 = m.ops[2 * (op - m.wb)], w1 = m.ops[2 * (op - m.wb) + 1];
    const uint32_t r0 = (uint32_t)w1.x, r1 = (uint32_t)w1.y;
    bool ok = true;
    switch ((w0.z >> OPF_TYPE_SHIFT) & 15) {
    case FT_LEAF_LEAF:
        cp_async16(st, tc.leaf + (size_t)(r0 & REF_IDX_MASK) * 32);
        cp_async16(st + 32, tc.leaf + (size_t)(r1 & REF_IDX_MASK) * 32);
        break;
    case FT_LEAF_ACC:
        cp_async16(st, tc.leaf + (size_t)(r0 & REF_IDX_MASK) * 32);
        break;
    case FT_LEAF_INT:
        cp_async16(st, tc.leaf + (size_t)(r0 & REF_IDX_MASK) * 32);
        ok = fwd_issue_set<JS, JROW>(p, ck, tc, dc, st, r1, (uint32_t)w1.w, op, lane, tr);
        break;
    case FT_INT_ACC:
        ok = fwd_issue_set<JS, JROW>(p, ck, tc, dc, st, r0, (uint32_t)w1.z, op, lane, tr);
        break;
    default: {
        int nl = 0, ni = 0;
        for (int r = 0; r < w0.y && (nl < 2 || ni < 1); r++) {
            const uint32_t ref = fwd_ref(p, m, w0.x + r);
            const uint32_t kind = ref >> 30;
            if (kind == REF_LEAF) {
                if (nl < 2) cp_async16(st + nl * 32, tc.leaf + (size_t)(ref & REF_IDX_MASK) * 32);
                nl++;
            } else if (kind == REF_INT) {
                if (ni == 0) ok = fwd_issue_set<JS, JROW>(p, ck, tc, dc, st, ref, ref_row(p, ck, ref), op, lane, tr) && ok;
                ni++;
            }
        }
    }
    }
    cp_async_commit();
    return ok;
}
__device__ __forceinline__ void stage_set16(const uint4* st, uint32_t X[16]) {
#pragma unroll
    for (int j = 0; j < 4; j++) {
        const uint4 v = st[(2 + j) * 32];
        X[4 * j] = v.x; X[4 * j + 1] = v.y; X[4 * j + 2] = v.z; X[4 * j + 3] = v.w;
    }
}
__device__ __forceinline__ void row_set16(const uint4* row, uint32_t X[16]) {
#pragma unroll
    for (int j = 0; j < 4; j++) {
        const uint4 v = ld_l2(row + j * 32);
        X[4 * j] = v.x; X[4 * j + 1] = v.y; X[4 * j + 2] = v.z; X[4 * j + 3] = v.w;
    }
}

__device__ __forceinline__ bool fwd_on_path(const RunParams& p, const int4 w0, int op, int head) {
    for (int r = 0; r < w0.y; r++) {
        const uint32_t ref = __ldg(p.refs + w0.x + r), kind = ref >> 30;
        if (kind == REF_CHAIN) return true;
        if (head < 0) continue;
        if (kind == REF_ACC && head == op - 1) return true;
        if (kind == REF_INT && !(ref & REF_EXT) && int(ref & REF_IDX_MASK) == head) return true;
    }
    return false;
}
template <bool ACC_REGS>
__device__ __forceinline__ bool fitch_fold_known(const RunParams& p, const Chunk& ck, const TileCtx& tc, DepCursor& dc, const int4 w0,
                                                 int op, int head, const uint32_t acc[16], int lane, FitchFold& fold, TraceItem& tr) {
    fold.reset();
    for (int r = 0; r < w0.y; r++) {
        const uint32_t ref = __ldg(p.refs + w0.x + r), kind = ref >> 30, idx = ref & REF_IDX_MASK;
        if (kind == REF_CHAIN) continue;
        if (kind == REF_LEAF) {
            const uint4 c = ld_stream(tc.leaf + (size_t)idx * 32);
            const uint32_t cc[4] = {c.x, c.y, c.z, c.w};
            fold.add_leaf(cc, FULL);
        } else if (kind == REF_ACC) {
            if (head >= 0 && head == op - 1) continue;
            if (ACC_REGS) {
                fold.add_set(acc);
            } else {
                uint32_t S[16];
                row_set16(tc.sets + (size_t)(op - 1) * 128, S);
                fold.add_set(S);
            }
        } else {
            if (!(ref & REF_EXT) && head >= 0 && int(idx) == head) continue;
            if (ref & REF_EXT) {
                if (!wait_dep(p, ck, tc.done, dc, int(idx), lane, tr)) return false;
            }
            uint32_t S[16];
            row_set16(tc.sets + (size_t)ref_row(p, ck, ref) * 128, S);
            fold.add_set(S);
        }
    }
    return true;
}
__device__ __forceinline__ void fitch_root_ref(const RunParams& p, int tile, int lane, uint32_t S[16]) {
    const uint4* cp = p.colparams + (size_t)tile * 128;
    uint4 rc = __ldg(cp + 64 + lane);
    uint32_t rv = __ldg(cp + 96 + lane).y;
    uint32_t r4[4] = {rc.x, rc.y, rc.z, rc.w}, d[16];
    decode16(r4, d);
#pragma unroll
    for (int k = 0; k < 16; k++) S[k] = (rv & d[k]) | (~rv & S[k]);
}
__device__ __forceinline__ void store_set16(uint4* out, const uint32_t S[16]) {
#pragma unroll
    for (int j = 0; j < 4; j++) out[j * 32] = make_uint4(S[4 * j], S[4 * j + 1], S[4 * j + 2], S[4 * j + 3]);
}

constexpr int FITCH_FWD_STAGE = (2 + 4) * 32, FITCH_FWD_PER_WARP = FWD_DEPTH * FITCH_FWD_STAGE + FWD_META_U4;
template <bool SPEC>
__device__ __forceinline__ bool fitch_forward_item(const RunParams& p, uint4* ring, int chunk, int tile, int lane, TraceItem& tr) {
    constexpr int JS = 4, STAGE = FITCH_FWD_STAGE;
    FwdMeta m;
    m.ops = reinterpret_cast<int4*>(ring + FWD_DEPTH * STAGE);
    m.refs = reinterpret_cast<uint32_t*>(m.ops + 2 * META_OPS);
    uint4* const ring_l = ring + lane;
    {
        const Chunk ck = p.chunks[chunk];
        const TileCtx tc = tile_ctx<4>(p, tile, lane);
        DepCursor dc;
        uint32_t acc[16];
#pragma unroll
        for (int k = 0; k < 16; k++) acc[k] = 0;
        const bool spec = SPEC && ck.chain_op >= 0 && p.leaf_present == nullptr;
        int first = ck.op_begin, resolved = -1;
        if (spec) {
            FitchInterval iv;
            iv.reset();
            int head = -1;
            first = ck.op_end;
            for (int op = ck.op_begin; op < ck.op_end; op++) {
                const int4 w0 = __ldg(reinterpret_cast<const int4*>(p.fwd_ops + op));
                const bool on_path = fwd_on_path(p, w0, op, head);
                FitchFold fold;
                if (!fitch_fold_known<true>(p, ck, tc, dc, w0, op, head, acc, lane, fold, tr)) return false;
                if (!on_path) {
                    fold.finish(acc);
                    store_set16(tc.sets + (size_t)op * 128, acc);
                    continue;
                }
                iv.step(fold.A, fold.O);
                if ((w0.z & OPF_ROOT) && !(p.flags & RUN_BLOCK_MODE)) {
                    fitch_root_ref(p, tile, lane, iv.lo);
                    fitch_root_ref(p, tile, lane, iv.hi);
                }
                head = op;
                if (!__any_sync(FULL, iv.open() != 0)) {
#pragma unroll
                    for (int k = 0; k < 16; k++) acc[k] = iv.lo[k];
                    store_set16(tc.sets + (size_t)op * 128, acc);
                    if (w0.z & OPF_SIGNAL) signal_flag(tc.done + op, p.epoch, lane);
                    resolved = op;
                    first = op + 1;
                    break;
                }
            }
        }
        if (first < ck.op_end) fwd_meta_load(p, m, first, ck.op_end, lane);
        for (int i = 0; i < FWD_DEPTH && first + i < ck.op_end; i++) {
            if (!fwd_issue<JS, 4>(p, ck, m, tc, dc, ring_l + i * STAGE, first + i, lane, tr)) return false;
        }
        int stage = 0;
        for (int op = first; op < ck.op_end; op++) {
            if (op + FWD_DEPTH >= m.wb + META_OPS && m.wb + META_OPS < ck.op_end) fwd_meta_load(p, m, op, ck.op_end, lane);
            const int4 w0 = m.ops[2 * (op - m.wb)], w1 = m.ops[2 * (op - m.wb) + 1];
            cp_async_wait_stage<FWD_DEPTH>(ck.op_end - 1 - op);
            uint4* st = ring_l + stage * STAGE;
            const int type = p.leaf_present ? FT_GENERIC : ((w0.z >> OPF_TYPE_SHIFT) & 15);
            if (type == FT_LEAF_LEAF) {
                const uint4 l0 = st[0], l1 = st[32];
                const uint32_t c0[4] = {l0.x, l0.y, l0.z, l0.w}, c1[4] = {l1.x, l1.y, l1.z, l1.w};
                fitch_leaf_leaf(c0, c1, acc);
            } else if (type == FT_LEAF_ACC) {
                const uint4 l0 = st[0];
                const uint32_t c0[4] = {l0.x, l0.y, l0.z, l0.w};
                uint32_t X[16];
#pragma unroll
                for (int k = 0; k < 16; k++) X[k] = acc[k];
                fitch_leaf_set(c0, X, acc);
            } else if (type == FT_LEAF_INT || type == FT_INT_ACC) {
                const uint32_t ref = (uint32_t)(type == FT_LEAF_INT ? w1.y : w1.x);
                uint32_t X[16];
                if (fwd_set_prefetched(ref, op)) stage_set16(st, X);
                else row_set16(tc.sets + (size_t)(ref & REF_IDX_MASK) * 128, X);
                if (type == FT_LEAF_INT) {
                    const uint4 l0 = st[0];
                    const uint32_t c0[4] = {l0.x, l0.y, l0.z, l0.w};
                    fitch_leaf_set(c0, X, acc);
                } else {
                    uint32_t Y[16];
#pragma unroll
                    for (int k = 0; k < 16; k++) Y[k] = acc[k];
                    fitch_set_set(X, Y, acc);
                }
            } else {
                FitchFold fold;
                fold.reset();
                int nl = 0, ni = 0;
                for (int r = 0; r < w0.y; r++) {
                    const uint32_t ref = fwd_ref(p, m, w0.x + r);
                    const uint32_t kind = ref >> 30, idx = ref & REF_IDX_MASK;
                    if (kind == REF_LEAF) {
                        uint4 c;
                        if (nl < 2) c = st[nl * 32];
                        else c = ld_stream(tc.leaf + (size_t)idx * 32);
                        nl++;
                        uint32_t cc[4] = {c.x, c.y, c.z, c.w};
                        fold.add_leaf(cc, leaf_present_mask(p, idx));
                    } else if (kind == REF_ACC) {
                        fold.add_set(acc);
                    } else if (SPEC && kind == REF_CHAIN) {
                        if (!wait_flag(tc.done + idx, p.epoch, p.error, lane, tr)) return false;
                        uint32_t S[16];
                        row_set16(tc.sets + (size_t)idx * 128, S);
                        fold.add_set(S);
                    } else {
                        uint32_t S[16];
                        if (ni == 0 && fwd_set_prefetched(ref, op)) {
                            stage_set16(st, S);
                        } else {
                            if (ref & REF_EXT) {
                                if (!wait_dep(p, ck, tc.done, dc, int(idx), lane, tr)) return false;
                            }
                            row_set16(tc.sets + (size_t)ref_row(p, ck, ref) * 128, S);
                        }
                        ni++;
                        fold.add_set(S);
                    }
                }
                fold.finish(acc);
            }
            if ((w0.z & OPF_ROOT) && !(p.flags & RUN_BLOCK_MODE)) fitch_root_ref(p, tile, lane, acc);
            store_set16(tc.sets + (size_t)op * 128, acc);
            if (w0.z & OPF_SIGNAL) signal_flag(tc.done + op, p.epoch, lane);
            if (op + FWD_DEPTH < ck.op_end) {
                if (!fwd_issue<JS, 4>(p, ck, m, tc, dc, st, op + FWD_DEPTH, lane, tr)) return false;
            }
            stage = (stage + 1 == FWD_DEPTH) ? 0 : stage + 1;
        }
        if (spec) {
            if (!wait_flag(tc.done + ck.chain_row, p.epoch, p.error, lane, tr)) return false;
            uint32_t S[16];
            row_set16(tc.sets + (size_t)ck.chain_row * 128, S);
            const int end = resolved >= 0 ? resolved : ck.op_end;
            int head = -1;
            for (int op = ck.chain_op; op < end; op++) {
                const int4 w0 = __ldg(reinterpret_cast<const int4*>(p.fwd_ops + op));
                if (!fwd_on_path(p, w0, op, head)) continue;
                FitchFold fold;
                if (!fitch_fold_known<false>(p, ck, tc, dc, w0, op, head, acc, lane, fold, tr)) return false;
                fold.add_set(S);
                fold.finish(S);
                if ((w0.z & OPF_ROOT) && !(p.flags & RUN_BLOCK_MODE)) fitch_root_ref(p, tile, lane, S);
                store_set16(tc.sets + (size_t)op * 128, S);
                if (w0.z & OPF_SIGNAL) signal_flag(tc.done + op, p.epoch, lane);
                head = op;
            }
        }
        trace_end(p, tr, chunk, tile, lane);
    }
    return true;
}

template <bool SPEC>
__global__ void __launch_bounds__(WARPS_PER_BLOCK * 32, SPEC ? 4 : 5) fitch_forward_kernel(RunParams p, int chunk_begin, int n_chunks) {
    extern __shared__ uint4 smem[];
    const int lane = threadIdx.x & 31;
    uint4* ring = smem + (size_t)(threadIdx.x >> 5) * FITCH_FWD_PER_WARP;
    ItemIter it;
    TraceItem tr;
    int chunk, tile;
    while (next_item(p, it, chunk_begin, n_chunks, chunk, tile, lane, tr))
        if (!fitch_forward_item<SPEC>(p, ring, chunk, tile, lane, tr)) return;
}

template <int J>
__device__ __forceinline__ void bwd_issue(const BwdMeta& m, const TileCtx& tc, uint4* st, int op) {
    const uint4* srow = tc.sets + (size_t)op * (J * 32);
#pragma unroll
    for (int j = 0; j < J; j++) cp_async16(st + j * 32, srow + j * 32);
    const int4 b1 = m.ops[2 * (op - m.lo) + 1];
    if (b1.x > 0) cp_async16(st + J * 32, tc.leaf + (size_t)b1.z * 32);
    if (b1.x > 1) cp_async16(st + (J + 1) * 32, tc.leaf + (size_t)b1.w * 32);
    cp_async_commit();
}

template <int J>
__device__ __forceinline__ void bwd_issue_bulk(const BwdMeta& m, const uint4* sets_base, const uint4* leaf_base, uint4* stage_base,
                                               unsigned long long* bar, int op, int lane) {
    __syncwarp();
    if (lane == 0) {
        const int4 b1 = m.ops[2 * (op - m.lo) + 1];
        const int nl = min(b1.x, 2);
        mbar_expect_tx(bar, unsigned(J * 512 + nl * 512));
        bulk_copy(stage_base, sets_base + (size_t)op * (J * 32), J * 512, bar);
        if (nl > 0) bulk_copy(stage_base + J * 32, leaf_base + (size_t)b1.z * 32, 512, bar);
        if (nl > 1) bulk_copy(stage_base + (J + 1) * 32, leaf_base + (size_t)b1.w * 32, 512, bar);
    }
}

__device__ __forceinline__ bool bwd_parent_slot(const RunParams& p, const BwdHead& h, int tile, int lane, uint32_t P[4],
                                                uint32_t& pvis, TraceItem& tr) {
    const size_t fi = fslot_index(p, h.b0.y, tile);
    if (h.b1.y & OPF_PARENT_EXT) {
        if (!wait_flag(p.fdone + fi, p.epoch, p.error, lane, tr)) return false;
    }
    const uint32_t* fs = p.fstore + fi * FSLOT_WORDS;
    uint4 a = ld_l2(reinterpret_cast<const uint4*>(fs) + lane);
    pvis = __ldcg(fs + 128 + lane);
    P[0] = a.x; P[1] = a.y; P[2] = a.z; P[3] = a.w;
    return true;
}

__device__ __forceinline__ void bwd_finish_op(const RunParams& p, const BwdMeta& m, const TileCtx& tc, StageCursor& sc,
                                              const BwdHead& h, const uint4* leaf_stage, uint32_t* stack, int tile, int lane,
                                              const uint32_t P[4], const uint32_t F[4], uint32_t vis, bool sankoff_block,
                                              bool own_record = true) {
    if (own_record) emit(p, sc, h.b0.x, tile, lane, vis & differs4(F, P), P, F);
    if (h.b1.y & OPF_PUSH) {
        uint32_t* e = stack + ((h.b1.y >> OPF_PUSH_SHIFT) & 15) * FSLOT_WORDS;
        reinterpret_cast<uint4*>(e)[lane] = make_uint4(F[0], F[1], F[2], F[3]);
        e[128 + lane] = vis;
    }
    if (h.b0.z >= 0) {
        const size_t fi = fslot_index(p, h.b0.z, tile);
        uint32_t* fs = p.fstore + fi * FSLOT_WORDS;
        reinterpret_cast<uint4*>(fs)[lane] = make_uint4(F[0], F[1], F[2], F[3]);
        fs[128 + lane] = vis;
        if (h.b1.y & OPF_SIGNAL_F) signal_flag(p.fdone + fi, p.epoch, lane);
    }
    const bool plain = p.states == nullptr && p.leaf_present == nullptr;
    if (p.states) store_state(p, h.b0.x, tile, lane, F, vis);
    int l0 = 0;
    if (plain) {
        const int nfast = min(h.b1.x, 2);
        for (; l0 < nfast; l0++) {
            const uint4 c = leaf_stage[l0 * 32];
            const uint32_t cc[4] = {c.x, c.y, c.z, c.w};
            const uint32_t mut = vis & differs4(cc, F);
            if (__ballot_sync(FULL, mut != 0)) emit(p, sc, bwd_leaf(p, m, h.b0.w + l0).y, tile, lane, mut, F, cc);
        }
    }
    for (int l = l0; l < h.b1.x; l++) {
        const int2 lf = bwd_leaf(p, m, h.b0.w + l);
        uint4 c;
        if (l < 2) c = leaf_stage[l * 32];
        else c = ld_stream(tc.leaf + (size_t)lf.x * 32);
        uint32_t cc[4] = {c.x, c.y, c.z, c.w};
        uint32_t present = leaf_present_mask(p, lf.x);
        if (sankoff_block && !present) {
            cc[0] = cc[1] = cc[2] = cc[3] = 0;
            present = FULL;
        }
        const uint32_t lvis = vis & present;
        emit(p, sc, lf.y, tile, lane, lvis & differs4(cc, F), F, cc);
        if (p.states) {
            uint32_t m4[4] = {cc[0] & lvis, cc[1] & lvis, cc[2] & lvis, cc[3] & lvis};
            store_state(p, lf.y, tile, lane, m4, lvis);
        }
    }
}

constexpr int FITCH_BWD_STAGE = (4 + 2) * 32,
              FITCH_BWD_PER_WARP = BWD_DEPTH * FITCH_BWD_STAGE + BWD_META_U4 + BWD_STACK_U4 + (PMB_BULK ? (BWD_DEPTH * 8 + 15) / 16 : 0);
template <bool SPEC>
__device__ __forceinline__ bool fitch_backward_item(const RunParams& p, uint4* ring, StageCursor& sc, int chunk, int tile, int lane,
                                                    TraceItem& tr, unsigned& phases) {
    constexpr int J = 4, STAGE = FITCH_BWD_STAGE;
    BwdMeta m;
    m.ops = reinterpret_cast<int4*>(ring + BWD_DEPTH * STAGE);
    m.leaves = reinterpret_cast<int2*>(m.ops + 2 * META_OPS);
    uint32_t* stack = reinterpret_cast<uint32_t*>(ring + BWD_DEPTH * STAGE + BWD_META_U4);
    uint4* const ring_l = ring + lane;
#if PMB_BULK
    unsigned long long* const bars = reinterpret_cast<unsigned long long*>(ring + BWD_DEPTH * STAGE + BWD_META_U4 + BWD_STACK_U4);
    const uint4* const sets_base = p.sets + (size_t)tile * p.n_ops * (J * 32);
    const uint4* const leaf_base = p.leaf_planes + (size_t)tile * p.n_rows * 32;
#endif
    {
        const Chunk ck = p.chunks[chunk];
        const TileCtx tc = tile_ctx<J>(p, tile, lane);
        const int last = ck.op_end - 1;
        uint32_t accF[4] = {0, 0, 0, 0}, accVis = 0;
        int resolved = -1;
        uint32_t specF[4] = {0, 0, 0, 0}, specVis = 0;
        if (SPEC && p.leaf_present == nullptr && (ck.flags & CHUNK_CHAIN_TOP)) {
            uint32_t Q[16];
#pragma unroll
            for (int k = 0; k < 16; k++) Q[k] = FULL;
            for (int op = last; op >= ck.op_begin; op--) {
                if (op != last && !(__ldg(&p.bwd_ops[op].flags) & OPF_HEAVY)) continue;
                uint32_t S[16];
                row_set16(tc.sets + (size_t)op * 128, S);
                fitch_candidates_step(Q, S);
                if (!__any_sync(FULL, candidates_open(Q) != 0)) {
                    resolved = op;
                    encode16(Q, specF);
                    specVis = __ldg(p.colparams + (size_t)tile * 128 + 96 + lane).z;
#pragma unroll
                    for (int k = 0; k < 4; k++) specF[k] &= specVis;
                    break;
                }
            }
        }
        for (int range = (resolved >= 0 ? 0 : 1); range < 2; range++) {
        const int hi = range == 0 ? resolved : last;
        const int lo = (range == 1 && resolved >= 0) ? resolved : ck.op_begin;
        bwd_meta_load(p, m, hi, lo, lane);
#if PMB_BULK
        for (int i = 0; i < BWD_DEPTH && hi - i >= lo; i++) bwd_issue_bulk<J>(m, sets_base, leaf_base, ring + i * STAGE, bars + i, hi - i, lane);
#else
        for (int i = 0; i < BWD_DEPTH && hi - i >= lo; i++) bwd_issue<J>(m, tc, ring_l + i * STAGE, hi - i);
#endif
        int stage = 0;
        for (int op = hi; op >= lo; op--) {
            if (op - BWD_DEPTH < m.lo && m.lo > lo) bwd_meta_load(p, m, op, lo, lane);
            BwdHead h;
            h.b0 = m.ops[2 * (op - m.lo)];
            h.b1 = m.ops[2 * (op - m.lo) + 1];
            const bool given = range == 0 && op == resolved, own_only = range == 1 && op == resolved;
            uint32_t P[4] = {0, 0, 0, 0}, pvis = 0, F[4], vis;
            if (given) {
            } else if (h.b0.y == PARENT_ACC) {
                P[0] = accF[0]; P[1] = accF[1]; P[2] = accF[2]; P[3] = accF[3];
                pvis = accVis;
            } else if (h.b0.y <= PARENT_STACK0) {
                const uint32_t* e = stack + (PARENT_STACK0 - h.b0.y) * FSLOT_WORDS;
                const uint4 a = reinterpret_cast<const uint4*>(e)[lane];
                pvis = e[128 + lane];
                P[0] = a.x; P[1] = a.y; P[2] = a.z; P[3] = a.w;
            } else if (h.b0.y >= 0) {
                if (!bwd_parent_slot(p, h, tile, lane, P, pvis, tr)) return false;
            }
#if PMB_BULK
            mbar_wait(bars + stage, (phases >> stage) & 1u);
            phases ^= 1u << stage;
#else
            cp_async_wait_stage<BWD_DEPTH>(op - lo);
#endif
            uint4* st = ring_l + stage * STAGE;
            uint32_t S[16];
#pragma unroll
            for (int j = 0; j < 4; j++) {
                const uint4 v = st[j * 32];
                S[4 * j] = v.x; S[4 * j + 1] = v.y; S[4 * j + 2] = v.z; S[4 * j + 3] = v.w;
            }
            if (given) {
                F[0] = specF[0]; F[1] = specF[1]; F[2] = specF[2]; F[3] = specF[3];
                vis = specVis;
            } else if (h.b0.y == PARENT_ROOT) {
                const uint4* cp = p.colparams + (size_t)tile * 128;
                uint4 pc = __ldg(cp + lane), ov = __ldg(cp + 32 + lane), fl = __ldg(cp + 96 + lane);
                P[0] = pc.x; P[1] = pc.y; P[2] = pc.z; P[3] = pc.w;
                uint32_t o4[4] = {ov.x, ov.y, ov.z, ov.w};
                const uint32_t ov_valid = fl.x & fl.z, colmask = fl.z;
                if (p.flags & RUN_BLOCK_MODE) {
                    uint32_t v0;
                    fitch_assign(S, P, colmask, F, v0);
                    vis = (v0 | ov_valid) & colmask;
#pragma unroll
                    for (int k = 0; k < 4; k++) F[k] = ((ov_valid & o4[k]) | (~ov_valid & F[k])) & vis;
                } else {
                    fitch_assign_root(S, o4, ov_valid, colmask, F, vis);
                }
            } else {
                fitch_assign(S, P, pvis, F, vis);
            }
            if (own_only) emit(p, sc, h.b0.x, tile, lane, vis & differs4(F, P), P, F);
            else bwd_finish_op(p, m, tc, sc, h, st + J * 32, stack, tile, lane, P, F, vis, false, !given);
#if PMB_BULK
            if (op - BWD_DEPTH >= lo) bwd_issue_bulk<J>(m, sets_base, leaf_base, ring + stage * STAGE, bars + stage, op - BWD_DEPTH, lane);
#else
            if (op - BWD_DEPTH >= lo) bwd_issue<J>(m, tc, st, op - BWD_DEPTH);
#endif
            stage = (stage + 1 == BWD_DEPTH) ? 0 : stage + 1;
            accF[0] = F[0]; accF[1] = F[1]; accF[2] = F[2]; accF[3] = F[3];
            accVis = vis;
        }
        }
        trace_end(p, tr, chunk, tile, lane);
    }
    return true;
}

template <bool SPEC>
__global__ void __launch_bounds__(WARPS_PER_BLOCK * 32) fitch_backward_kernel(RunParams p, int chunk_begin, int n_chunks) {
    extern __shared__ uint4 smem[];
    const int lane = threadIdx.x & 31;
    uint4* ring = smem + (size_t)(threadIdx.x >> 5) * FITCH_BWD_PER_WARP;
    unsigned phases = 0;
#if PMB_BULK
    {
        unsigned long long* bars = reinterpret_cast<unsigned long long*>(ring + BWD_DEPTH * FITCH_BWD_STAGE + BWD_META_U4 + BWD_STACK_U4);
        if (lane == 0) {
            for (int s = 0; s < BWD_DEPTH; s++) mbar_init(bars + s, 1);
            asm volatile("fence.mbarrier_init.release.cluster;" ::: "memory");
        }
        __syncwarp();
    }
#endif
    ItemIter it;
    TraceItem tr;
    StageCursor sc;
    int chunk, tile;
    while (next_item(p, it, chunk_begin, n_chunks, chunk, tile, lane, tr))
        if (!fitch_backward_item<SPEC>(p, ring, sc, chunk, tile, lane, tr, phases)) return;
}

template <int B>
__device__ __forceinline__ bool sankoff_forward_op(const RunParams& p, const Chunk& ck, DepCursor& dc, const FwdMeta& m,
                                                   const TileCtx& tc, const int4 w0, int op, const uint4* st, int lane,
                                                   uint32_t accG[16], uint32_t accH[16], TraceItem& tr) {
    SankoffFold<B> fold;
    fold.reset();
    int nl = 0, ni = 0;
    for (int r = 0; r < w0.y; r++) {
        const uint32_t ref = fwd_ref(p, m, w0.x + r);
        const uint32_t kind = ref >> 30, idx = ref & REF_IDX_MASK;
        if (kind == REF_LEAF) {
            uint4 c;
            if (nl < 2) c = st[nl * 32];
            else c = ld_stream(tc.leaf + (size_t)idx * 32);
            nl++;
            uint32_t present = leaf_present_mask(p, idx);
            uint32_t cc[4] = {c.x, c.y, c.z, c.w};
            if ((p.flags & RUN_BLOCK_MODE) && !present) {
                cc[0] = cc[1] = cc[2] = cc[3] = 0;
                present = FULL;
            }
            fold.add_leaf(cc, present);
        } else if (kind == REF_ACC) {
            fold.add_set(accG, sankoff_none(accG, accH));
        } else if (kind == REF_CHAIN) {
            if (!wait_flag(tc.done + idx, p.epoch, p.error, lane, tr)) return false;
            const uint4* row = tc.sets + (size_t)idx * 256;
            uint32_t G[16];
            row_set16(row, G);
            const uint32_t h0 = ld_l2(row + 128).x;
            fold.add_set(G, h0 & ~G[0]);
        } else {
            uint32_t G[16], h0;
            if (ni == 0 && fwd_set_prefetched(ref, op)) {
                stage_set16(st, G);
                h0 = st[(2 + 4) * 32].x;
            } else {
                if (ref & REF_EXT) {
                    if (!wait_dep(p, ck, tc.done, dc, int(idx), lane, tr)) return false;
                }
                const uint4* row = tc.sets + (size_t)ref_row(p, ck, ref) * 256;
                row_set16(row, G);
                h0 = ld_l2(row + 128).x;
            }
            ni++;
            fold.add_set(G, h0 & ~G[0]);
        }
    }
    fold.finish(accG, accH);
    return true;
}

__device__ __forceinline__ void store_gh(uint4* out, const uint32_t G[16], const uint32_t H[16]) {
#pragma unroll
    for (int j = 0; j < 4; j++) {
        out[j * 32] = make_uint4(G[4 * j], G[4 * j + 1], G[4 * j + 2], G[4 * j + 3]);
        out[(4 + j) * 32] = make_uint4(H[4 * j], H[4 * j + 1], H[4 * j + 2], H[4 * j + 3]);
    }
}
__device__ __forceinline__ bool sankoff_eval_small(const RunParams& p, const Chunk& ck, const TileCtx& tc, DepCursor& dc, const int4 w0,
                                                   uint32_t accG[16], uint32_t accH[16], int lane, TraceItem& tr) {
    SankoffFold<2> fold;
    fold.reset();
    for (int r = 0; r < w0.y; r++) {
        const uint32_t ref = __ldg(p.refs + w0.x + r), kind = ref >> 30, idx = ref & REF_IDX_MASK;
        if (kind == REF_LEAF) {
            const uint4 c = ld_stream(tc.leaf + (size_t)idx * 32);
            const uint32_t cc[4] = {c.x, c.y, c.z, c.w};
            fold.add_leaf(cc, FULL);
        } else if (kind == REF_ACC) {
            fold.add_set(accG, 0u);
        } else {
            if (ref & REF_EXT) {
                if (!wait_dep(p, ck, tc.done, dc, int(idx), lane, tr)) return false;
            }
            uint32_t G[16];
            row_set16(tc.sets + (size_t)ref_row(p, ck, ref) * 256, G);
            fold.add_set(G, 0u);
        }
    }
    fold.finish(accG, accH);
    return true;
}
template <bool ACC_REGS>
__device__ __forceinline__ bool sankoff_known_child(const RunParams& p, const Chunk& ck, const TileCtx& tc, DepCursor& dc, const int4 w0,
                                                    int op, int head, const uint32_t accG[16], int lane, uint32_t g[16], TraceItem& tr) {
    for (int r = 0; r < w0.y; r++) {
        const uint32_t ref = __ldg(p.refs + w0.x + r), kind = ref >> 30, idx = ref & REF_IDX_MASK;
        if (kind == REF_CHAIN) continue;
        if (kind == REF_LEAF) {
            const uint4 c = ld_stream(tc.leaf + (size_t)idx * 32);
            const uint32_t cc[4] = {c.x, c.y, c.z, c.w};
            sankoff_leaf_g(cc, FULL, g);
        } else if (kind == REF_ACC) {
            if (head >= 0 && head == op - 1) continue;
            if (ACC_REGS) {
#pragma unroll
                for (int k = 0; k < 16; k++) g[k] = accG[k];
            } else {
                row_set16(tc.sets + (size_t)(op - 1) * 256, g);
            }
        } else {
            if (!(ref & REF_EXT) && head >= 0 && int(idx) == head) continue;
            if (ref & REF_EXT) {
                if (!wait_dep(p, ck, tc.done, dc, int(idx), lane, tr)) return false;
            }
            row_set16(tc.sets + (size_t)ref_row(p, ck, ref) * 256, g);
        }
    }
    return true;
}

template <int MAXB, bool SPEC>
__global__ void __launch_bounds__(WARPS_PER_BLOCK * 32) sankoff_forward_kernel(RunParams p, int chunk_begin, int n_chunks) {
    extern __shared__ uint4 smem[];
    constexpr int JS = 5, STAGE = (2 + JS) * 32, PER_WARP = FWD_DEPTH * STAGE + FWD_META_U4;
    const int lane = threadIdx.x & 31;
    uint4* ring = smem + (size_t)(threadIdx.x >> 5) * PER_WARP;
// ... 260 lines not shown
__device__ __forceinline__ unsigned long long block_reduce_sum(unsigned long long v, unsigned long long* sh) {
#pragma unroll
    for (int d = 16; d > 0; d >>= 1) v += __shfl_down_sync(FULL, v, d);
    if ((threadIdx.x & 31) == 0) sh[threadIdx.x >> 5] = v;
    __syncthreads();
    unsigned long long t = (threadIdx.x < 32) ? sh[threadIdx.x] : 0ull;
    if (threadIdx.x < 32) {
#pragma unroll
        for (int d = 16; d > 0; d >>= 1) t += __shfl_down_sync(FULL, t, d);
        if (threadIdx.x == 0) sh[32] = t;
    }
    __syncthreads();
    unsigned long long r = sh[32];
    __syncthreads();
    return r;
}

__global__ void __launch_bounds__(SCAN_BLOCK) scan_sums_kernel(const unsigned int* counts, int n, unsigned long long* block_sums) {
    __shared__ unsigned long long sh[33];
    const int base = blockIdx.x * SCAN_TILE + threadIdx.x * SCAN_ITEMS;
    unsigned long long s = 0;
#pragma unroll
    for (int k = 0; k < SCAN_ITEMS; k++)
        if (base + k < n) s += counts[base + k];
    s = block_reduce_sum(s, sh);
    if (threadIdx.x == 0) block_sums[blockIdx.x] = s;
}

__global__ void __launch_bounds__(SCAN_BLOCK) scan_apply_kernel(const unsigned int* counts, int n, const unsigned long long* block_sums,
                                                                long long* offsets) {
    __shared__ unsigned long long sh[33];
    __shared__ unsigned long long warp_tot[32];
    unsigned long long before = 0;
    for (int b = threadIdx.x; b < (int)blockIdx.x; b += SCAN_BLOCK) before += block_sums[b];
    before = block_reduce_sum(before, sh);
    const int base = blockIdx.x * SCAN_TILE + threadIdx.x * SCAN_ITEMS;
    unsigned long long v[SCAN_ITEMS], s = 0;
#pragma unroll
    for (int k = 0; k < SCAN_ITEMS; k++) {
        v[k] = (base + k < n) ? counts[base + k] : 0u;
        s += v[k];
    }
    unsigned long long incl = s;
    const int lane = threadIdx.x & 31, warp = threadIdx.x >> 5;
#pragma unroll
    for (int d = 1; d < 32; d <<= 1) {
        unsigned long long t = __shfl_up_sync(FULL, incl, d);
        if (lane >= d) incl += t;
    }
    if (lane == 31) warp_tot[warp] = incl;
    __syncthreads();
    if (warp == 0) {
        unsigned long long w = warp_tot[lane], wi = w;
#pragma unroll
        for (int d = 1; d < 32; d <<= 1) {
            unsigned long long t = __shfl_up_sync(FULL, wi, d);
            if (lane >= d) wi += t;
        }
        warp_tot[lane] = wi - w;
    }
    __syncthreads();
    unsigned long long run = before + warp_tot[warp] + (incl - s);
#pragma unroll
    for (int k = 0; k < SCAN_ITEMS; k++) {
        if (base + k < n) offsets[base + k] = (long long)run;
        run += v[k];
        if (base + k == n - 1) offsets[n] = (long long)run;
    }
}

constexpr int CPT_GROUP = 256;

__device__ __forceinline__ unsigned long long dir_valid(unsigned long long d, unsigned dir_tag) {
    if (unsigned(d >> DIR_TAG_SHIFT) != dir_tag) return 0ull;
    return d & ((1ull << DIR_TAG_SHIFT) - 1ull);
}

__global__ void __launch_bounds__(256) compact_count_kernel(unsigned long long n_entries, const unsigned long long* dir, unsigned dir_tag,
                                                           unsigned int* group_totals, unsigned n_groups) {
    const unsigned g = (blockIdx.x * 256u + threadIdx.x) >> 5, lane = threadIdx.x & 31;
    if (g >= n_groups) return;
    const unsigned long long e0 = (unsigned long long)g * CPT_GROUP + lane * 8u;
    unsigned sum = 0;
    if (e0 + 8 <= n_entries) {
#pragma unroll
        for (int k = 0; k < 8; k += 2) {
            const uint4 v = __ldcg(reinterpret_cast<const uint4*>(dir + e0 + k));
            sum += unsigned(dir_valid((unsigned long long)v.x | ((unsigned long long)v.y << 32), dir_tag) & 0x7FFull);
            sum += unsigned(dir_valid((unsigned long long)v.z | ((unsigned long long)v.w << 32), dir_tag) & 0x7FFull);
        }
    } else {
        for (int k = 0; k < 8; k++)
            if (e0 + k < n_entries) sum += unsigned(dir_valid(__ldcg(dir + e0 + k), dir_tag) & 0x7FFull);
    }
#pragma unroll
    for (int s = 16; s > 0; s >>= 1) sum += __shfl_down_sync(FULL, sum, s);
    if (lane == 0) group_totals[g] = sum;
}

constexpr int SCAN1_ITEMS = 8;
__global__ void __launch_bounds__(1024) compact_scan_kernel(const unsigned int* block_totals, int n_blocks, unsigned long long* block_prefix,
                                                            long long* offsets_end) {
    __shared__ unsigned long long s_w[32];
    __shared__ unsigned long long s_carry;
    const int tid = threadIdx.x, lane = tid & 31, warp = tid >> 5;
    if (tid == 0) s_carry = 0;
    __syncthreads();
    for (int b0 = 0; b0 < n_blocks; b0 += 1024 * SCAN1_ITEMS) {
        const int b = b0 + tid * SCAN1_ITEMS;
        unsigned v[SCAN1_ITEMS];
        unsigned long long sum = 0;
#pragma unroll
        for (int k = 0; k < SCAN1_ITEMS; k++) {
            v[k] = b + k < n_blocks ? block_totals[b + k] : 0u;
            sum += v[k];
        }
        unsigned long long incl = sum;
#pragma unroll
        for (int s = 1; s < 32; s <<= 1) {
            unsigned long long t = __shfl_up_sync(FULL, incl, s);
            if (lane >= s) incl += t;
        }
        if (lane == 31) s_w[warp] = incl;
        __syncthreads();
        if (warp == 0) {
            unsigned long long w = s_w[lane], wi = w;
#pragma unroll
            for (int s = 1; s < 32; s <<= 1) {
                unsigned long long t = __shfl_up_sync(FULL, wi, s);
                if (lane >= s) wi += t;
            }
            s_w[lane] = wi - w;
        }
        __syncthreads();
        const unsigned long long carry = s_carry;
        unsigned long long run = carry + s_w[warp] + incl - sum;
#pragma unroll
        for (int k = 0; k < SCAN1_ITEMS; k++) {
            if (b + k < n_blocks) block_prefix[b + k] = run;
            run += v[k];
        }
        __syncthreads();
        if (tid == 1023) s_carry = run;
        __syncthreads();
    }
    if (tid == 0) *offsets_end = (long long)s_carry;
}

__global__ void __launch_bounds__(CPT_GROUP) compact_copy_kernel(int n_nodes, int T, const unsigned long long* group_prefix,
                                                                long long* offsets, const unsigned long long* dir, unsigned dir_tag,
                                                                const uint16_t* staging, long long col_base, int32_t* pos,
                                                                uint8_t* type_code, unsigned long long* counters,
                                                                unsigned long long* run_words, unsigned long long staging_cap,
                                                                unsigned long long* tickets, int n_tickets) {
    __shared__ unsigned s_w[CPT_GROUP / 32];
    __shared__ unsigned s_last;
    const int tid = threadIdx.x, lane = tid & 31, warp = tid >> 5;
    const unsigned long long n_entries = (unsigned long long)n_nodes * (unsigned long long)T;
    const unsigned long long e = (unsigned long long)blockIdx.x * CPT_GROUP + tid;
    const unsigned long long d = e < n_entries ? dir_valid(__ldcg(dir + e), dir_tag) : 0ull;
    const unsigned cnt = unsigned(d & 0x7FFull);
    unsigned incl = cnt;
#pragma unroll
    for (int s = 1; s < 32; s <<= 1) {
        unsigned t = __shfl_up_sync(FULL, incl, s);
        if (lane >= s) incl += t;
    }
    if (lane == 31) s_w[warp] = incl;
    __syncthreads();
    unsigned before = 0;
#pragma unroll
    for (int w = 0; w < CPT_GROUP / 32; w++)
        if (w < warp) before += s_w[w];
    if (e < n_entries) {
        const unsigned long long at = group_prefix[blockIdx.x] + before + (incl - cnt);
        unsigned long long node, tile;
        if (n_entries <= 0xFFFFFFFFull) {
            node = unsigned(e) / unsigned(T);
            tile = unsigned(e) - unsigned(node) * unsigned(T);
        } else {
            node = e / (unsigned long long)T;
            tile = e - node * (unsigned long long)T;
        }
        if (tile == 0) offsets[node] = (long long)at;
        if (cnt && run_words[0] <= staging_cap) {
            const uint16_t* src = staging + (d >> 11);
            const long long cb = col_base + (long long)tile * TILE_COLS;
            for (unsigned q0 = 0; q0 < cnt; q0 += 4) {
                uint32_t r[4];
#pragma unroll
                for (int i = 0; i < 4; i++) r[i] = q0 + i < cnt ? src[q0 + i] : 0u;
#pragma unroll
                for (int i = 0; i < 4; i++)
                    if (q0 + i < cnt) {
                        pos[at + q0 + i] = int32_t(cb + (r[i] & 1023u));
                        type_code[at + q0 + i] = uint8_t(((r[i] >> 14) << 4) | ((r[i] >> 10) & 15u));
                    }
            }
        }
    }
    __syncthreads();
    unsigned int* done_blocks = reinterpret_cast<unsigned int*>(counters + 3);
    if (tid == 0) {
        __threadfence();
        s_last = atomicAdd(done_blocks, 1u) == gridDim.x - 1 ? 1u : 0u;
    }
    __syncthreads();
    if (s_last) {
        if (tid == 0) {
            unsigned int* error = reinterpret_cast<unsigned int*>(run_words + 1);
            unsigned int* sticky = reinterpret_cast<unsigned int*>(counters + 2);
            const unsigned long long pool = run_words[0];
            const unsigned int er0 = error[0], er1 = error[1];
            const unsigned int st = er0 | (pool > staging_cap ? 4u : 0u);
            if (st) sticky[0] |= st;
            if ((er0 & 1u) && er1 < sticky[1]) sticky[1] = er1;
            counters[4] = pool;
            reinterpret_cast<unsigned int*>(counters + 5)[0] = er0;
            reinterpret_cast<unsigned int*>(counters + 5)[1] = er1;
            run_words[0] = 0ull;
            error[0] = 0u;
            error[1] = 0xFFFFFFFFu;
            done_blocks[0] = 0u;
        }
        for (int i = tid; i < n_tickets; i += CPT_GROUP) tickets[i] = 0ull;
    }
}


__host__ __device__ inline size_t packed_pos_offset(long long n_nodes) { return (16 + size_t(n_nodes + 1) * 8 + 15) / 16 * 16; }
__host__ __device__ inline size_t packed_tc_offset(long long n_nodes, long long cap) {
    return (packed_pos_offset(n_nodes) + size_t(cap) * 4 + 15) / 16 * 16;
}
__host__ __device__ inline size_t packed_bytes(long long n_nodes, long long cap) {
    return (packed_tc_offset(n_nodes, cap) + size_t(cap) + 15) / 16 * 16;
}

constexpr long long PACK_HDR_BAD = -1;
__global__ void pack_result_kernel(const long long* offsets, const int32_t* pos, const uint8_t* type_code, long long n_nodes,
                                   long long cap, long long src_cap, const unsigned long long* counters, unsigned char* out) {
    const long long total = offsets[n_nodes];
    const bool ok = total >= 0 && total <= cap && total <= src_cap && counters[4] <= (unsigned long long)src_cap;
    const long long n = ok ? total : 0;
    long long* hdr = reinterpret_cast<long long*>(out);
    long long* off_out = hdr + 2;
    int32_t* pos_out = reinterpret_cast<int32_t*>(out + packed_pos_offset(n_nodes));
    uint8_t* tc_out = out + packed_tc_offset(n_nodes, cap);
    const long long stride = (long long)gridDim.x * blockDim.x;
    const long long i0 = (long long)blockIdx.x * blockDim.x + threadIdx.x;
    if (i0 == 0) {
        hdr[0] = ok ? total : PACK_HDR_BAD;
        hdr[1] = n_nodes;
    }
    if (!ok) return;
    for (long long i = i0; i <= n_nodes; i += stride) off_out[i] = offsets[i];
    const long long n4 = n / 4;
    const int4* pos4 = reinterpret_cast<const int4*>(pos);
    int4* pos_out4 = reinterpret_cast<int4*>(pos_out);
    for (long long i = i0; i < n4; i += stride) pos_out4[i] = pos4[i];
    const long long n16 = n / 16;
    const uint4* tc16 = reinterpret_cast<const uint4*>(type_code);
    uint4* tc_out16 = reinterpret_cast<uint4*>(tc_out);
    for (long long i = i0; i < n16; i += stride) tc_out16[i] = tc16[i];
    for (long long i = n4 * 4 + i0; i < n; i += stride) pos_out[i] = pos[i];
    for (long long i = n16 * 16 + i0; i < n; i += stride) tc_out[i] = type_code[i];
}

__device__ __forceinline__ bool shard_ok(const unsigned char* shard, int n_nodes, long long cap) {
    const long long* hdr = reinterpret_cast<const long long*>(shard);
    return hdr[1] == n_nodes && hdr[0] >= 0 && hdr[0] <= cap;
}

__global__ void merge_count_kernel(const unsigned char* packed, size_t shard_bytes, int n_shards, int n_nodes, long long cap,
                                   unsigned int* counts, unsigned int* rel, unsigned int* merge_err) {
    int v = blockIdx.x * blockDim.x + threadIdx.x;
    if (v >= n_nodes) return;
    unsigned int c = 0;
    for (int k = 0; k < n_shards; k++) {
        const unsigned char* sh = packed + k * shard_bytes;
        rel[(size_t)k * n_nodes + v] = c;
        if (!shard_ok(sh, n_nodes, cap)) {
            if (v == 0) atomicOr(merge_err, reinterpret_cast<const long long*>(sh)[1] == n_nodes ? 1u : 2u);
            continue;
        }
        const long long* off = reinterpret_cast<const long long*>(sh + 16);
        c += (unsigned int)(off[v + 1] - off[v]);
    }
    counts[v] = c;
}

__global__ void merge_copy_kernel(const unsigned char* packed, size_t shard_bytes, int n_nodes, long long cap, const long long* merged_off,
                                  const unsigned int* rel, int32_t* pos, uint8_t* type_code) {
    const int k = blockIdx.y;
    const unsigned char* sh = packed + (size_t)k * shard_bytes;
    if (!shard_ok(sh, n_nodes, cap)) return;
    const long long n = reinterpret_cast<const long long*>(sh)[0];
    const long long* off = reinterpret_cast<const long long*>(sh + 16);
    const int32_t* spos = reinterpret_cast<const int32_t*>(sh + packed_pos_offset(n_nodes));
    const uint8_t* stc = sh + packed_tc_offset(n_nodes, cap);
    const unsigned int* relk = rel + (size_t)k * n_nodes;
    const long long stride = (long long)gridDim.x * blockDim.x * 4;
    for (long long j0 = ((long long)blockIdx.x * blockDim.x + threadIdx.x) * 4; j0 < n; j0 += stride) {
        int lo = 0, hi = n_nodes;
        while (hi - lo > 1) {
            const int mid = (lo + hi) >> 1;
            if (__ldg(off + mid) <= j0) lo = mid;
            else hi = mid;
        }
        int v = lo;
        long long end = __ldg(off + v + 1);
        long long dst = __ldg(merged_off + v) + __ldg(relk + v) - __ldg(off + v);
        const long long j1 = min(n, j0 + 4);
        for (long long j = j0; j < j1; j++) {
            while (j >= end) {
                v++;
                end = __ldg(off + v + 1);
                dst = __ldg(merged_off + v) + __ldg(relk + v) - __ldg(off + v);
            }
            pos[dst + j] = spos[j];
            type_code[dst + j] = stc[j];
        }
    }
}

constexpr int RM_THREADS = 256, RM_ITEMS = 8, RM_BLOCK = RM_THREADS * RM_ITEMS;

__global__ void rm_mark_starts_kernel(const long long* off, int n_nodes, uint8_t* flags) {
    const int v = blockIdx.x * blockDim.x + threadIdx.x;
    if (v < n_nodes && off[v] < off[v + 1]) flags[off[v]] = 1;
}
__device__ __forceinline__ bool rm_is_break(long long i, const int32_t* pos, const uint8_t* tc, const uint8_t* flags,
                                            const uint8_t* col_break, long long col_base) {
    if (flags[i] & 1) return true;
    const int32_t p = pos[i];
    return p != pos[i - 1] + 1 || (tc[i] >> 4) != (tc[i - 1] >> 4) || (col_break && col_break[p - col_base]);
}
__global__ void __launch_bounds__(RM_THREADS) rm_block_last_kernel(const long long* off, int n_nodes, const int32_t* pos, const uint8_t* tc,
                                                                   const uint8_t* flags, const uint8_t* col_break, long long col_base,
                                                                   long long* last) {
    __shared__ long long s_w[RM_THREADS / 32];
    const long long n = off[n_nodes], i0 = ((long long)blockIdx.x * RM_THREADS + threadIdx.x) * RM_ITEMS;
    long long m = -1;
    for (int k = 0; k < RM_ITEMS; k++)
        if (i0 + k < n && rm_is_break(i0 + k, pos, tc, flags, col_break, col_base)) m = i0 + k;
#pragma unroll
    for (int d = 16; d > 0; d >>= 1) m = max(m, __shfl_down_sync(FULL, m, d));
    if ((threadIdx.x & 31) == 0) s_w[threadIdx.x >> 5] = m;
    __syncthreads();
    if (threadIdx.x == 0) {
        for (int w = 1; w < RM_THREADS / 32; w++) m = max(m, s_w[w]);
        last[blockIdx.x] = m;
    }
}
__global__ void __launch_bounds__(1024) rm_scan_max_kernel(const long long* last, int n_blocks, long long* carry) {
    __shared__ long long s_w[32];
    __shared__ long long s_carry;
    const int tid = threadIdx.x, lane = tid & 31, warp = tid >> 5;
    if (tid == 0) s_carry = -1;
    __syncthreads();
    for (int b0 = 0; b0 < n_blocks; b0 += 1024) {
        const int b = b0 + tid;
        const long long v = b < n_blocks ? last[b] : -1;
        long long incl = v;
#pragma unroll
        for (int d = 1; d < 32; d <<= 1) {
            const long long t = __shfl_up_sync(FULL, incl, d);
            if (lane >= d) incl = max(incl, t);
        }
        if (lane == 31) s_w[warp] = incl;
        __syncthreads();
        long long before = s_carry;
        for (int w = 0; w < warp; w++) before = max(before, s_w[w]);
        long long excl = __shfl_up_sync(FULL, incl, 1);
        if (lane == 0) excl = -1;
        if (b < n_blocks) carry[b] = max(before, excl);
        __syncthreads();
        if (tid == 1023) s_carry = max(before, incl);
        __syncthreads();
    }
}
__global__ void __launch_bounds__(RM_THREADS) rm_flags_kernel(const long long* off, int n_nodes, const int32_t* pos, const uint8_t* tc,
                                                              uint8_t* flags, const uint8_t* col_break, long long col_base,
                                                              const long long* carry, unsigned int* counts) {
    __shared__ long long s_w[RM_THREADS / 32];
    __shared__ unsigned s_c[RM_THREADS / 32];
    const int tid = threadIdx.x, lane = tid & 31, warp = tid >> 5;
    const long long n = off[n_nodes], i0 = ((long long)blockIdx.x * RM_THREADS + tid) * RM_ITEMS;
    long long rs[RM_ITEMS], m = -1;
#pragma unroll
    for (int k = 0; k < RM_ITEMS; k++) {
        if (i0 + k < n && rm_is_break(i0 + k, pos, tc, flags, col_break, col_base)) m = i0 + k;
        rs[k] = m;
    }
    long long incl = m;
#pragma unroll
// ... 211 lines not shown
```

Before: 2544 billion.

## Store Fitch sets compactly as lowest-code plus exception pool for non-singletons

Internal-node Fitch sets used to be stored as 16 full bit-planes. They are now stored as a 4-plane code plus a per-node header bitmask, and only lanes holding non-singleton sets spill their full planes into a shared pool with an overflow counter. The backward pass loads one uint4 per lane, or four from the pool for exception lanes, and takes a cheaper assignment path when the whole warp is singleton. This cuts set-matrix memory traffic and footprint. In exchange it adds pool allocation, overflow detection with forward re-runs or async failure, and extra header bookkeeping.

```diff
diff --git a/panman_b200/csrc/plane_math.h b/panman_b200/csrc/plane_math.h
--- a/panman_b200/csrc/plane_math.h
+++ b/panman_b200/csrc/plane_math.h
@@ -186,6 +186,23 @@
     }
 }
 
+
+PMB_HD uint32_t fitch_nonsingle(const uint32_t S[16]) {
+    uint32_t one = 0, two = 0;
+#pragma unroll
+    for (int k = 0; k < 16; k++) {
+        two |= one & S[k];
+        one |= S[k];
+    }
+    return ~one | two;
+}
+PMB_HD uint32_t fitch_encode(const uint32_t S[16], uint32_t c[4]) {
+    uint32_t any;
+    lowest16(S, c, any);
+    return fitch_nonsingle(S);
+}
+PMB_HD uint32_t fitch_code_pair(const uint32_t a[4], const uint32_t b[4]) { return differs4(a, b); }
+
 PMB_HD void fitch_assign(const uint32_t S[16], const uint32_t P[4], uint32_t pvis, uint32_t F[4], uint32_t& vis) {
     uint32_t low[4], any;
     lowest16(S, low, any);
@@ -193,6 +210,11 @@
     vis = pvis & any;
 #pragma unroll
     for (int b = 0; b < 4; b++) F[b] = ((hit & P[b]) | (~hit & low[b])) & vis;
+}
+PMB_HD void fitch_assign_single(const uint32_t c[4], uint32_t pvis, uint32_t F[4], uint32_t& vis) {
+    vis = pvis;
+#pragma unroll
+    for (int b = 0; b < 4; b++) F[b] = c[b] & pvis;
 }
 
 PMB_HD void fitch_assign_root(const uint32_t S[16], const uint32_t ov[4], uint32_t ov_valid, uint32_t colmask,
diff --git a/panman_b200/csrc/pmb_api.cu b/panman_b200/csrc/pmb_api.cu
--- a/panman_b200/csrc/pmb_api.cu
+++ b/panman_b200/csrc/pmb_api.cu
@@ -98,6 +98,7 @@
 
     int64_t opt_chunk_nodes = 0;
     int64_t opt_staging_records = 0;
+    int64_t opt_set_pool_lanes = 0;
     int64_t opt_inline_nodes = 3;
     int64_t opt_schedule = 1;
     int64_t opt_trace = 0;
@@ -127,7 +128,7 @@
     cudaStream_t cstream = nullptr;
     cudaStream_t bstream = nullptr;
     cudaEvent_t ev_fwd_done = nullptr, ev_bwd_done = nullptr, ev_compact_done[2] = {nullptr, nullptr};
-    DevBuf d_sets2, d_dir2, d_staging2;
+    DevBuf d_sets2, d_dir2, d_staging2, d_set_pool2;
     int64_t opt_grid_pct = 0;
     int cur_grid_pct = 100;
     int64_t opt_overlap = 1;
@@ -182,6 +183,10 @@
         d_states_u8;
     unsigned long long staging_cap = 0;
     bool staging_floor_dirty = false;
+    DevBuf d_set_pool;
+    unsigned long long set_pool_cap = 0;
+    bool set_pool_floor_dirty = false;
+    unsigned long long set_pool_slots = 0;
     bool have_result = false;
     int last_algo = 0, last_flags = 0;
     int64_t n_mut = 0;
@@ -359,7 +364,7 @@
 
 int launch_pass(pmb_ctx* c, cudaStream_t stream, int ticket_slot, const RunParams& rp, int algo, bool forward, int* n_launches) {
     const TreeProgram& P = c->prog;
-    const size_t fwd_smem = size_t(WARPS_PER_BLOCK) * (FWD_DEPTH * (2 + 4) * 32 + FWD_META_U4) * sizeof(uint4);
+    const size_t fwd_smem = size_t(WARPS_PER_BLOCK) * FITCH_FWD_PER_WARP * sizeof(uint4);
     const size_t fwd_smem_s = size_t(WARPS_PER_BLOCK) * (FWD_DEPTH * (2 + 5) * 32 + FWD_META_U4) * sizeof(uint4);
     const size_t bwd_smem_f = size_t(WARPS_PER_BLOCK) * FITCH_BWD_PER_WARP * sizeof(uint4);
     const size_t bwd_smem_s = size_t(WARPS_PER_BLOCK) * (BWD_DEPTH * (8 + 2) * 32 + BWD_META_U4 + BWD_STACK_U4) * sizeof(uint4);
@@ -470,7 +475,8 @@
                           &c->d_pos, &c->d_tc, &c->d_states_u8, &c->d_done, &c->d_fdone, &c->d_ticket, &c->d_mcounts, &c->d_moff,
                           &c->d_mpos, &c->d_mtc, &c->d_scan_state, &c->d_trace, &c->d_rm_counts, &c->d_rm_off, &c->d_rm_pos,
                           &c->d_rm_info, &c->d_rm_nucs, &c->d_rm_wire, &c->d_rm_flags, &c->d_rm_oidx, &c->d_col_break, &c->d_merge_err, &c->d_mblock_sums, &c->d_mrel,
-                          &c->d_run_events, &c->d_run_off, &c->d_dfs_slot, &c->d_dir2, &c->d_staging2})
+                          &c->d_run_events, &c->d_run_off, &c->d_dfs_slot, &c->d_dir2, &c->d_staging2, &c->d_set_pool,
+                          &c->d_set_pool2})
             b->release();
         for (auto& s : c->prog_cache)
             for (DevBuf& b : s.bufs) b.release();
@@ -526,6 +532,10 @@
     else if (k == "staging_records") {
         c->opt_staging_records = value;
         c->staging_cap = 0;
+    }
+    else if (k == "set_pool_lanes") {
+        c->opt_set_pool_lanes = value;
+        c->set_pool_cap = 0;
     }
     else if (k == "inline_nodes") c->opt_inline_nodes = value;
     else if (k == "schedule") c->opt_schedule = value;
@@ -624,6 +634,7 @@
     c->have_result = false;
     c->have_col_break = false;
     c->staging_floor_dirty = true;
+    c->set_pool_floor_dirty = true;
     c->n_cols = n_cols;
     c->col_base = col_base;
     c->T = int32_t((n_cols + TILE_COLS - 1) / TILE_COLS);
@@ -756,6 +767,15 @@
                                fwd_root_ref, col_base, false))
 }
 
+static size_t set_matrix_bytes(int algo, size_t n_internal, size_t T) {
+    if (algo == PMB_ALGO_FITCH) return n_internal * T * (32 * sizeof(uint4) + 8) + 16;
+    return n_internal * T * 256 * sizeof(uint4);
+}
+static unsigned long long set_pool_slack(const pmb_ctx* c) { return (unsigned long long)c->n_sms * 8 * WARPS_PER_BLOCK * FITCH_POOL_BLOCK; }
+static void grow_set_pool(pmb_ctx* c, unsigned long long reserved) {
+    c->set_pool_cap = std::min<unsigned long long>(0xF0000000ull, std::max(c->set_pool_cap * 2, reserved + reserved / 8 + set_pool_slack(c)));
+}
+
 static int run_impl(pmb_ctx* c, int algo, int flags, bool async) {
     if (!c) return PMB_ERR_INVALID;
     if (!c->stream) return fail(c, PMB_ERR_CUDA, "no usable CUDA device; there is no CPU fallback");
@@ -766,25 +786,34 @@
     c->have_result = false;
     const TreeProgram& P = c->prog;
     const size_t T = size_t(c->T);
-    const size_t set_bytes_per = (algo == PMB_ALGO_FITCH ? 128 : 256) * sizeof(uint4);
-    const size_t set_bytes = size_t(P.n_internal) * T * set_bytes_per;
+    const bool fitch = algo == PMB_ALGO_FITCH;
+    if (fitch && (c->set_pool_cap == 0 || c->set_pool_floor_dirty)) {
+        const unsigned long long lanes = (unsigned long long)P.n_internal * T * 32;
+        const unsigned long long cap = c->opt_set_pool_lanes > 0 ? (unsigned long long)c->opt_set_pool_lanes : lanes / 8 + set_pool_slack(c);
+        c->set_pool_cap = std::min<unsigned long long>(0xF0000000ull, c->opt_set_pool_lanes > 0 && c->set_pool_cap == 0 ? cap : std::max(c->set_pool_cap, cap));
+        c->set_pool_floor_dirty = false;
+    }
+    const size_t mat_bytes = set_matrix_bytes(algo, P.n_internal, T), pool_bytes = fitch ? size_t(c->set_pool_cap) * 64 : 0;
+    const size_t set_bytes = mat_bytes + pool_bytes;
     bool overlap = c->opt_overlap > 0 && c->opt_schedule == 1 && pick_groups(c) == 1 && set_bytes <= std::min(size_t(48) << 30, c->total_mem / 4);
-    if (overlap && set_bytes > c->d_sets2.cap && set_bytes > (size_t(8) << 30)) {
+    const size_t have1 = c->d_sets.cap + c->d_set_pool.cap, have2 = c->d_sets2.cap + c->d_set_pool2.cap;
+    if (overlap && set_bytes > have2 && set_bytes > (size_t(8) << 30)) {
         size_t free_b = 0, total_b = 0;
-        const size_t need = set_bytes + (set_bytes > c->d_sets.cap ? set_bytes - c->d_sets.cap : 0) + (size_t(16) << 30);
+        const size_t need = set_bytes + (set_bytes > have1 ? set_bytes - have1 : 0) + (size_t(16) << 30);
         if (cudaMemGetInfo(&free_b, &total_b) != cudaSuccess) {
             cudaGetLastError();
             overlap = false;
-        } else if (free_b + c->d_sets2.cap < need) {
+        } else if (free_b + have2 < need) {
             overlap = false;
         }
     }
-    if (set_bytes > c->d_sets.cap || (overlap && set_bytes > c->d_sets2.cap)) {
+    if (mat_bytes > c->d_sets.cap || (overlap && mat_bytes > c->d_sets2.cap) || pool_bytes > c->d_set_pool.cap ||
+        (overlap && pool_bytes > c->d_set_pool2.cap)) {
         PMB_CUDA(cudaStreamSynchronize(c->bstream));
         PMB_CUDA(cudaStreamSynchronize(c->cstream));
     }
-    PMB_CUDA(c->d_sets.ensure(set_bytes));
-    if (overlap) PMB_CUDA(c->d_sets2.ensure(set_bytes));
+    PMB_CUDA(c->d_sets.ensure(mat_bytes));
+    if (overlap) PMB_CUDA(c->d_sets2.ensure(mat_bytes));
     PMB_CUDA(c->d_fstore.ensure(std::max<size_t>(16, size_t(P.n_fslots) * T * FSLOT_WORDS * sizeof(uint32_t))));
     const bool want_states = flags & PMB_FLAG_WANT_STATES;
     if (want_states) PMB_CUDA(c->d_states_planes.ensure(size_t(P.n_nodes) * T * 64 * sizeof(uint4)));
@@ -830,6 +859,7 @@
     const int parity = int(c->run_seq & 1u);
     const bool second = dbl && parity;
     rp.sets = (overlap && parity) ? c->d_sets2.as<uint4>() : c->d_sets.as<uint4>();
+    rp.set_pool_count = fitch ? c->d_counters.as<unsigned long long>() + 10 + parity : nullptr;
     rp.fstore = c->d_fstore.as<uint32_t>();
     rp.order = nullptr;
     rp.stage_block = 512;
@@ -892,11 +922,20 @@
     const int ticket_set = 64 * parity;
     c->run_seq++;
     cudaStream_t const bwd_stream = G == 1 ? c->bstream : c->stream;
+    if (getenv("PMB_XGRID")) c->opt_grid_pct = atoi(getenv("PMB_XGRID"));
     c->cur_grid_pct = c->opt_grid_pct > 0 ? int(c->opt_grid_pct)
                                           : (async && overlap && P.n_chain_segments == 0 ? (c->T < 24 ? 70 : 80) : 100);
     unsigned int* const run_error = rp.error;
     unsigned int* const fwd_error = reinterpret_cast<unsigned int*>(c->d_counters.as<unsigned long long>() + 2);
+    bool redo_fwd = false;
+    unsigned int fwd_epoch_now = fwd_epoch;
     for (int attempt = 0;; attempt++) {
+        if (fitch) {
+            DevBuf& pool = (overlap && parity) ? c->d_set_pool2 : c->d_set_pool;
+            PMB_CUDA(pool.ensure(size_t(c->set_pool_cap) * 64));
+            rp.set_pool = pool.as<uint4>();
+            rp.set_pool_cap = c->set_pool_cap;
+        }
         PMB_CUDA(c->d_staging.ensure(size_t(c->staging_cap) * sizeof(uint16_t)));
         if (dbl) PMB_CUDA(c->d_staging2.ensure(size_t(c->staging_cap) * sizeof(uint16_t)));
         PMB_CUDA(c->d_pos.ensure(size_t(c->staging_cap) * sizeof(int32_t)));
@@ -912,8 +951,8 @@
             if (G > 1) PMB_CUDA(cudaStreamWaitEvent(st, c->ev_fork, 0));
             group_range(g, &rp.tile_begin, &rp.tile_count);
             rp.trace_base = (unsigned long long)P.chunks.size() * rp.tile_begin;
-            if (attempt == 0) {
-                rp.epoch = fwd_epoch;
+            if (attempt == 0 || redo_fwd) {
+                rp.epoch = fwd_epoch_now;
                 rp.error = fwd_error;
                 if ((rc = launch_pass(c, st, ticket_set + 2 * g, rp, algo, true, &n_launches))) return rc;
                 rp.error = run_error;
@@ -958,7 +997,7 @@
             compact_copy_kernel<<<groups, CPT_GROUP, 0, c->cstream>>>(
                 P.n_nodes, c->T, gprefix, c->d_offsets.as<long long>(), rp.dir, rp.dir_tag, rp.staging, c->col_base,
                 c->d_pos.as<int32_t>(), c->d_tc.as<uint8_t>(), c->d_counters.as<unsigned long long>(), run_words, rp.staging_cap,
-                c->d_ticket.as<unsigned long long>() + ticket_set, 64);
+                c->d_ticket.as<unsigned long long>() + ticket_set, 64, rp.set_pool_count, rp.set_pool_cap);
             n_launches += 2;
             n_launches += 1;
         }
@@ -981,6 +1020,7 @@
         PMB_CUDA(cudaMemcpyAsync(c->h_counters.as<char>() + 16, c->d_offsets.as<long long>() + P.n_nodes, 8, cudaMemcpyDeviceToHost,
                                  c->cstream));
         PMB_CUDA(cudaMemcpyAsync(c->h_counters.as<char>() + 24, c->d_counters.as<char>() + 16, 4, cudaMemcpyDeviceToHost, c->cstream));
+        PMB_CUDA(cudaMemcpyAsync(c->h_counters.as<char>() + 32, c->d_counters.as<char>() + 48, 8, cudaMemcpyDeviceToHost, c->cstream));
         PMB_CUDA(cudaStreamSynchronize(c->cstream));
         PMB_CUDA(cudaStreamSynchronize(c->stream));
         c->upload_pending = false;
@@ -989,6 +1029,18 @@
         eflags |= c->h_counters.as<unsigned int>()[6] & 2u;
         if (eflags || total > c->staging_cap) c->sticky_dirty = true;
         if (eflags & 2u) return fail(c, PMB_ERR_INTERNAL, "scheduler watchdog fired: a dependency flag never arrived");
+        c->set_pool_slots = *reinterpret_cast<unsigned long long*>(c->h_counters.as<char>() + 32);
+        redo_fwd = (eflags & 8u) != 0;
+        if (redo_fwd) {
+            if (attempt >= 4) return fail(c, PMB_ERR_INTERNAL, "exception pool overflow persisted");
+            grow_set_pool(c, c->set_pool_slots);
+            if (size_t(c->set_pool_cap) * 64 > ((overlap && parity) ? c->d_set_pool2.cap : c->d_set_pool.cap)) {
+                PMB_CUDA(cudaStreamSynchronize(c->bstream));
+                PMB_CUDA(cudaStreamSynchronize(c->cstream));
+            }
+            fwd_epoch_now = ++c->epoch;
+            continue;
+        }
         if (eflags & 1u) {
             char buf[160];
             snprintf(buf, sizeof buf, "Sankoff root has no finite cost at column %lld and no root override was given",
@@ -1044,7 +1096,8 @@
     if (c->opt_schedule != 1 || c->opt_overlap <= 0 || c->opt_trace || (flags & PMB_FLAG_WANT_STATES)) return false;
     if (algo != PMB_ALGO_FITCH && algo != PMB_ALGO_SANKOFF) return false;
     if (c->prog.n_chain_segments > 0 || pick_groups(c) != 1) return false;
-    const size_t set_bytes = size_t(c->prog.n_internal) * size_t(c->T) * (algo == PMB_ALGO_FITCH ? 128 : 256) * sizeof(uint4);
+    const size_t set_bytes = set_matrix_bytes(algo, size_t(c->prog.n_internal), size_t(c->T)) +
+                             (algo == PMB_ALGO_FITCH ? size_t(c->set_pool_cap) * 64 : 0);
     return set_bytes <= std::min(size_t(4) << 30, c->total_mem / 16);
 }
 
@@ -1065,6 +1118,7 @@
     PMB_CUDA(cudaSetDevice(c->device));
     L->opt_chunk_nodes = c->opt_chunk_nodes;
     L->opt_staging_records = c->opt_staging_records;
+    L->opt_set_pool_lanes = c->opt_set_pool_lanes;
     L->opt_inline_nodes = c->opt_inline_nodes;
     L->opt_schedule = c->opt_schedule;
     L->opt_target_items = c->opt_target_items;
@@ -1084,6 +1138,7 @@
         L->have_present = c->have_present;
         L->have_input = true;
         L->staging_floor_dirty = true;
+        L->set_pool_floor_dirty = true;
         DevBuf* dst[13];
         lane_borrowed(L, dst);
         DevBuf* src[13];
@@ -1097,6 +1152,7 @@
         L->lane_mirror_gen = c->input_gen;
     }
     L->staging_cap = std::max(L->staging_cap, c->staging_cap);
+    L->set_pool_cap = std::max(L->set_pool_cap, c->set_pool_cap);
     PMB_CUDA(cudaStreamWaitEvent(L->stream, c->ev_input_ready, 0));
     int rc = run_impl(L, algo, flags, true);
     if (rc) {
@@ -1192,7 +1248,9 @@
     PMB_CUDA(cudaMemcpyAsync(c->h_counters.p, c->d_counters.as<char>() + 32, 8, cudaMemcpyDeviceToHost, c->cstream));
     PMB_CUDA(cudaMemcpyAsync(c->h_counters.as<char>() + 16, c->d_counters.as<char>() + 16, 8, cudaMemcpyDeviceToHost, c->cstream));
     PMB_CUDA(cudaMemcpyAsync(c->h_counters.as<char>() + 32, c->d_offsets.as<long long>() + N, 8, cudaMemcpyDeviceToHost, c->cstream));
+    PMB_CUDA(cudaMemcpyAsync(c->h_counters.as<char>() + 40, c->d_counters.as<char>() + 48, 8, cudaMemcpyDeviceToHost, c->cstream));
     PMB_CUDA(cudaStreamSynchronize(c->cstream));
+    c->set_pool_slots = *reinterpret_cast<unsigned long long*>(c->h_counters.as<char>() + 40);
     c->async_pending = false;
     const unsigned int sticky = c->h_counters.as<unsigned int>()[4], scol = c->h_counters.as<unsigned int>()[5];
     unsigned int sticky_init[2] = {0u, 0xFFFFFFFFu};
@@ -1204,6 +1262,11 @@
                  (long long)scol + (long long)c->col_base);
         c->have_result = false;
         return fail(c, PMB_ERR_SANKOFF_ROOT, buf);
+    }
+    if (sticky & 8u) {
+        c->have_result = false;
+        grow_set_pool(c, std::max(c->set_pool_slots, c->set_pool_cap * 2));
+        return fail(c, PMB_ERR_STAGING, "the Fitch set-exception pool overflowed during an asynchronous run; rerun (the pool was grown)");
     }
     if (sticky & 4u) {
         c->have_result = false;
@@ -1598,9 +1661,10 @@
 int64_t pmb_algorithmic_bytes(const pmb_ctx* c, int algo) {
     if (!c || !c->have_tree || !c->have_input) return 0;
     const int64_t L = c->prog.n_rows, I = c->prog.n_internal;
-    const int64_t per_col = L + (algo == PMB_ALGO_SANKOFF ? 8 : 4) * I;
     const pmb_ctx* r = result_cctx(c);
-    return c->n_cols * per_col + 8 * (r->have_result ? std::max<int64_t>(0, r->n_mut) : 0);
-}
-
-}
+    const int64_t records = 8 * (r->have_result ? std::max<int64_t>(0, r->n_mut) : 0);
+    if (algo == PMB_ALGO_SANKOFF) return c->n_cols * (L + 8 * I) + records;
+    return c->n_cols * (L + I) + 2 * 8 * I * int64_t(c->T) + 2 * 64 * int64_t(r->set_pool_slots) + records;
+}
+
+}
diff --git a/panman_b200/csrc/pmb_kernels.cuh b/panman_b200/csrc/pmb_kernels.cuh
--- a/panman_b200/csrc/pmb_kernels.cuh
+++ b/panman_b200/csrc/pmb_kernels.cuh
@@ -24,6 +24,9 @@
     const uint4* leaf_planes;
     const uint8_t* leaf_present;
     uint4* sets;
+    uint4* set_pool;
+    unsigned long long* set_pool_count;
+    unsigned long long set_pool_cap;
     uint32_t* fstore;
     const uint4* colparams;
     uint4* states;
@@ -361,20 +364,25 @@
 struct BwdMeta {
     int4* ops;
     int2* leaves;
+    uint2* hdr;
     int lo;
     unsigned lb;
 };
-__device__ __forceinline__ void bwd_meta_load(const RunParams& p, BwdMeta& m, int top, int op_begin, int lane) {
+__device__ __forceinline__ void bwd_meta_load(const RunParams& p, BwdMeta& m, int top, int op_begin, int lane,
+                                              const uint2* hdr_tile = nullptr) {
     __syncwarp();
     m.lo = max(op_begin, top - (META_OPS - 1));
     int4 h0 = make_int4(0, 0, 0, 0), h1 = h0;
+    unsigned long long hd = 0;
     if (lane < META_OPS && m.lo + lane <= top) {
         h0 = __ldg(reinterpret_cast<const int4*>(p.bwd_ops + m.lo + lane));
         h1 = __ldg(reinterpret_cast<const int4*>(p.bwd_ops + m.lo + lane) + 1);
+        if (hdr_tile) hd = __ldcg(reinterpret_cast<const unsigned long long*>(hdr_tile + m.lo + lane));
     }
     if (lane < META_OPS) {
         m.ops[2 * lane] = h0;
         m.ops[2 * lane + 1] = h1;
+        if (hdr_tile) m.hdr[lane] = make_uint2(unsigned(hd), unsigned(hd >> 32));
     }
     m.lb = (unsigned)__shfl_sync(FULL, h0.w, 0);
 #pragma unroll
@@ -396,13 +404,18 @@
 struct TileCtx {
     const uint4* leaf;
     uint4* sets;
+    uint2* hdr;
     unsigned* done;
 };
+__device__ __forceinline__ uint2* fitch_hdr(const RunParams& p, int tile) {
+    return reinterpret_cast<uint2*>(p.sets + (size_t)p.T * p.n_ops * 32) + (size_t)tile * p.n_ops;
+}
 template <int JROW>
 __device__ __forceinline__ TileCtx tile_ctx(const RunParams& p, int tile, int lane) {
     TileCtx t;
     t.leaf = p.leaf_planes + (size_t)tile * p.n_rows * 32 + lane;
     t.sets = p.sets + (size_t)tile * p.n_ops * (JROW * 32) + lane;
+    t.hdr = JROW == 1 ? fitch_hdr(p, tile) : nullptr;
     t.done = p.done + (size_t)tile * p.n_ops;
     return t;
 }
@@ -420,6 +433,10 @@
     const uint4* row = tc.sets + (size_t)row_idx * (JROW * 32);
 #pragma unroll
     for (int j = 0; j < JS; j++) cp_async16(st + (2 + j) * 32, row + j * 32);
+    if (JROW == 1 && lane == 0) {
+        const uintptr_t h = reinterpret_cast<uintptr_t>(tc.hdr + row_idx);
+        cp_async16(st + 3 * 32, reinterpret_cast<const uint4*>(h & ~uintptr_t(15)));
+    }
     return true;
 }
 template <int JS, int JROW>
@@ -476,6 +493,86 @@
     }
 }
 
+constexpr int FITCH_POOL_BLOCK = 32;
+struct PoolCursor {
+    unsigned long long base = 0;
+    int left = 0;
+};
+__device__ __forceinline__ unsigned long long fitch_slot(uint2 h, int lane) {
+    return (unsigned long long)h.y + __popc(h.x & ((1u << lane) - 1u));
+}
+__device__ __forceinline__ uint2 fitch_hdr_load(const uint2* h, int lane) {
+    unsigned long long v = 0;
+    if (lane == 0) v = __ldcg(reinterpret_cast<const unsigned long long*>(h));
+    v = __shfl_sync(FULL, v, 0);
+    return make_uint2(unsigned(v), unsigned(v >> 32));
+}
+__device__ __forceinline__ uint2 fitch_stage_hdr(const uint4* st, const uint2* h, int lane) {
+    unsigned long long v = 0;
+    if (lane == 0) {
+        const uint4 w = st[3 * 32];
+        v = (reinterpret_cast<uintptr_t>(h) & 8) ? ((unsigned long long)w.w << 32 | w.z) : ((unsigned long long)w.y << 32 | w.x);
+    }
+    v = __shfl_sync(FULL, v, 0);
+    return make_uint2(unsigned(v), unsigned(v >> 32));
+}
+__device__ __forceinline__ void fitch_planes(const RunParams& p, uint2 h, const uint32_t c[4], int lane, uint32_t S[16]) {
+    if ((h.x >> lane) & 1u) {
+        const unsigned long long s = fitch_slot(h, lane);
+        if (s < p.set_pool_cap) {
+            const uint4* q = p.set_pool + s * 4;
+#pragma unroll
+            for (int j = 0; j < 4; j++) {
+                const uint4 v = ld_l2(q + j);
+                S[4 * j] = v.x; S[4 * j + 1] = v.y; S[4 * j + 2] = v.z; S[4 * j + 3] = v.w;
+            }
+        } else {
+#pragma unroll
+            for (int k = 0; k < 16; k++) S[k] = 0;
+        }
+    } else {
+        decode16(c, S);
+    }
+}
+__device__ __forceinline__ void fitch_row16(const RunParams& p, const TileCtx& tc, uint32_t row, int lane, uint32_t S[16]) {
+    const uint4 v = ld_l2(tc.sets + (size_t)row * 32);
+    const uint32_t c[4] = {v.x, v.y, v.z, v.w};
+    fitch_planes(p, fitch_hdr_load(tc.hdr + row, lane), c, lane, S);
+}
+__device__ __forceinline__ void fitch_store(const RunParams& p, PoolCursor& pc, const TileCtx& tc, int op, int lane, const uint32_t c[4],
+                                            uint32_t ns, const uint32_t S[16]) {
+    tc.sets[(size_t)op * 32] = make_uint4(c[0], c[1], c[2], c[3]);
+    const unsigned mask = __ballot_sync(FULL, ns != 0);
+    unsigned long long base = 0;
+    if (mask) {
+        const int n = __popc(mask);
+        if (n > pc.left) {
+            const int take = max(n, FITCH_POOL_BLOCK);
+            unsigned long long b = 0;
+            if (lane == 0) b = atomicAdd(p.set_pool_count, (unsigned long long)take);
+            pc.base = __shfl_sync(FULL, b, 0);
+            pc.left = take;
+        }
+        base = pc.base;
+        pc.base += n;
+        pc.left -= n;
+        if (ns) {
+            const unsigned long long s = fitch_slot(make_uint2(mask, unsigned(base)), lane);
+            if (s < p.set_pool_cap) {
+                uint4* q = p.set_pool + s * 4;
+#pragma unroll
+                for (int j = 0; j < 4; j++) q[j] = make_uint4(S[4 * j], S[4 * j + 1], S[4 * j + 2], S[4 * j + 3]);
+            }
+        }
+    }
+    if (lane == 0) tc.hdr[op] = make_uint2(mask, unsigned(base));
+}
+__device__ __forceinline__ void fitch_put(const RunParams& p, PoolCursor& pc, const TileCtx& tc, int op, int lane, const uint32_t S[16],
+                                          uint32_t c[4], uint32_t& ns) {
+    ns = fitch_encode(S, c);
+    fitch_store(p, pc, tc, op, lane, c, ns, S);
+}
+
 __device__ __forceinline__ bool fwd_on_path(const RunParams& p, const int4 w0, int op, int head) {
     for (int r = 0; r < w0.y; r++) {
         const uint32_t ref = __ldg(p.refs + w0.x + r), kind = ref >> 30;
@@ -503,7 +600,7 @@
                 fold.add_set(acc);
             } else {
                 uint32_t S[16];
-                row_set16(tc.sets + (size_t)(op - 1) * 128, S);
+                fitch_row16(p, tc, uint32_t(op - 1), lane, S);
                 fold.add_set(S);
             }
         } else {
@@ -512,7 +609,7 @@
                 if (!wait_dep(p, ck, tc.done, dc, int(idx), lane, tr)) return false;
             }
             uint32_t S[16];
-            row_set16(tc.sets + (size_t)ref_row(p, ck, ref) * 128, S);
+            fitch_row16(p, tc, ref_row(p, ck, ref), lane, S);
             fold.add_set(S);
         }
     }
@@ -527,24 +624,34 @@
 #pragma unroll
     for (int k = 0; k < 16; k++) S[k] = (rv & d[k]) | (~rv & S[k]);
 }
-__device__ __forceinline__ void store_set16(uint4* out, const uint32_t S[16]) {
-#pragma unroll
-    for (int j = 0; j < 4; j++) out[j * 32] = make_uint4(S[4 * j], S[4 * j + 1], S[4 * j + 2], S[4 * j + 3]);
-}
-
-constexpr int FITCH_FWD_STAGE = (2 + 4) * 32, FITCH_FWD_PER_WARP = FWD_DEPTH * FITCH_FWD_STAGE + FWD_META_U4;
+
+constexpr int FITCH_FWD_STAGE = 3 * 32 + 1, FITCH_FWD_PER_WARP = FWD_DEPTH * FITCH_FWD_STAGE + FWD_META_U4;
+__device__ __forceinline__ uint2 fitch_child(const TileCtx& tc, const uint4* st, uint32_t ref, uint32_t row, int op, int lane, uint32_t c[4]) {
+    uint4 v;
+    uint2 h;
+    if (fwd_set_prefetched(ref, op)) {
+        v = st[2 * 32];
+        h = fitch_stage_hdr(st, tc.hdr + row, lane);
+    } else {
+        v = ld_l2(tc.sets + (size_t)row * 32);
+        h = fitch_hdr_load(tc.hdr + row, lane);
+    }
+    c[0] = v.x; c[1] = v.y; c[2] = v.z; c[3] = v.w;
+    return h;
+}
 template <bool SPEC>
-__device__ __forceinline__ bool fitch_forward_item(const RunParams& p, uint4* ring, int chunk, int tile, int lane, TraceItem& tr) {
-    constexpr int JS = 4, STAGE = FITCH_FWD_STAGE;
+__device__ __forceinline__ bool fitch_forward_item(const RunParams& p, uint4* ring, PoolCursor& pc, int chunk, int tile, int lane,
+                                                   TraceItem& tr) {
+    constexpr int STAGE = FITCH_FWD_STAGE;
     FwdMeta m;
     m.ops = reinterpret_cast<int4*>(ring + FWD_DEPTH * STAGE);
     m.refs = reinterpret_cast<uint32_t*>(m.ops + 2 * META_OPS);
     uint4* const ring_l = ring + lane;
     {
         const Chunk ck = p.chunks[chunk];
-        const TileCtx tc = tile_ctx<4>(p, tile, lane);
+        const TileCtx tc = tile_ctx<1>(p, tile, lane);
         DepCursor dc;
-        uint32_t acc[16];
+        uint32_t acc[16], accc[4] = {0, 0, 0, 0}, accns = 0;
 #pragma unroll
         for (int k = 0; k < 16; k++) acc[k] = 0;
         const bool spec = SPEC && ck.chain_op >= 0 && p.leaf_present == nullptr;
@@ -561,7 +668,7 @@
                 if (!fitch_fold_known<true>(p, ck, tc, dc, w0, op, head, acc, lane, fold, tr)) return false;
                 if (!on_path) {
                     fold.finish(acc);
-                    store_set16(tc.sets + (size_t)op * 128, acc);
+                    fitch_put(p, pc, tc, op, lane, acc, accc, accns);
                     continue;
                 }
                 iv.step(fold.A, fold.O);
@@ -573,7 +680,7 @@
                 if (!__any_sync(FULL, iv.open() != 0)) {
 #pragma unroll
                     for (int k = 0; k < 16; k++) acc[k] = iv.lo[k];
-                    store_set16(tc.sets + (size_t)op * 128, acc);
+                    fitch_put(p, pc, tc, op, lane, acc, accc, accns);
                     if (w0.z & OPF_SIGNAL) signal_flag(tc.done + op, p.epoch, lane);
                     resolved = op;
                     first = op + 1;
@@ -583,7 +690,7 @@
         }
         if (first < ck.op_end) fwd_meta_load(p, m, first, ck.op_end, lane);
         for (int i = 0; i < FWD_DEPTH && first + i < ck.op_end; i++) {
-            if (!fwd_issue<JS, 4>(p, ck, m, tc, dc, ring_l + i * STAGE, first + i, lane, tr)) return false;
+            if (!fwd_issue<1, 1>(p, ck, m, tc, dc, ring_l + i * STAGE, first + i, lane, tr)) return false;
         }
         int stage = 0;
         for (int op = first; op < ck.op_end; op++) {
@@ -592,31 +699,52 @@
             cp_async_wait_stage<FWD_DEPTH>(ck.op_end - 1 - op);
             uint4* st = ring_l + stage * STAGE;
             const int type = p.leaf_present ? FT_GENERIC : ((w0.z >> OPF_TYPE_SHIFT) & 15);
-            if (type == FT_LEAF_LEAF) {
-                const uint4 l0 = st[0], l1 = st[32];
-                const uint32_t c0[4] = {l0.x, l0.y, l0.z, l0.w}, c1[4] = {l1.x, l1.y, l1.z, l1.w};
-                fitch_leaf_leaf(c0, c1, acc);
-            } else if (type == FT_LEAF_ACC) {
-                const uint4 l0 = st[0];
-                const uint32_t c0[4] = {l0.x, l0.y, l0.z, l0.w};
-                uint32_t X[16];
-#pragma unroll
-                for (int k = 0; k < 16; k++) X[k] = acc[k];
-                fitch_leaf_set(c0, X, acc);
-            } else if (type == FT_LEAF_INT || type == FT_INT_ACC) {
-                const uint32_t ref = (uint32_t)(type == FT_LEAF_INT ? w1.y : w1.x);
-                uint32_t X[16];
-                if (fwd_set_prefetched(ref, op)) stage_set16(st, X);
-                else row_set16(tc.sets + (size_t)(ref & REF_IDX_MASK) * 128, X);
-                if (type == FT_LEAF_INT) {
+            const bool root_ref = (w0.z & OPF_ROOT) && !(p.flags & RUN_BLOCK_MODE);
+            if (type == FT_LEAF_LEAF || type == FT_LEAF_ACC || type == FT_LEAF_INT || type == FT_INT_ACC) {
+                uint32_t a[4], b[4], bns = 0;
+                uint2 h = make_uint2(0u, 0u);
+                if (type == FT_INT_ACC) {
+                    h = fitch_child(tc, st, (uint32_t)w1.x, (uint32_t)w1.z, op, lane, a);
+                } else {
                     const uint4 l0 = st[0];
-                    const uint32_t c0[4] = {l0.x, l0.y, l0.z, l0.w};
-                    fitch_leaf_set(c0, X, acc);
+                    a[0] = l0.x; a[1] = l0.y; a[2] = l0.z; a[3] = l0.w;
+                }
+                if (type == FT_LEAF_LEAF) {
+                    const uint4 l1 = st[32];
+                    b[0] = l1.x; b[1] = l1.y; b[2] = l1.z; b[3] = l1.w;
+                } else if (type == FT_LEAF_INT) {
+                    h = fitch_child(tc, st, (uint32_t)w1.y, (uint32_t)w1.w, op, lane, b);
+                } else {
+                    b[0] = accc[0]; b[1] = accc[1]; b[2] = accc[2]; b[3] = accc[3];
+                    bns = accns;
+                }
+                const uint32_t ns = fitch_code_pair(a, b);
+                if (!root_ref && h.x == 0 && !__any_sync(FULL, (ns | bns) != 0)) {
+                    accc[0] = a[0]; accc[1] = a[1]; accc[2] = a[2]; accc[3] = a[3];
+                    accns = 0;
                 } else {
                     uint32_t Y[16];
-#pragma unroll
-                    for (int k = 0; k < 16; k++) Y[k] = acc[k];
-                    fitch_set_set(X, Y, acc);
+                    if (type == FT_LEAF_LEAF) {
+                        fitch_leaf_leaf(a, b, acc);
+                    } else {
+                        if (type == FT_LEAF_INT) {
+                            fitch_planes(p, h, b, lane, Y);
+                        } else if (bns) {
+#pragma unroll
+                            for (int k = 0; k < 16; k++) Y[k] = acc[k];
+                        } else {
+                            decode16(b, Y);
+                        }
+                        if (type == FT_INT_ACC) {
+                            uint32_t X[16];
+                            fitch_planes(p, h, a, lane, X);
+                            fitch_set_set(X, Y, acc);
+                        } else {
+                            fitch_leaf_set(a, Y, acc);
+                        }
+                    }
+                    if (root_ref) fitch_root_ref(p, tile, lane, acc);
+                    accns = fitch_encode(acc, accc);
                 }
             } else {
                 FitchFold fold;
@@ -633,40 +761,51 @@
                         uint32_t cc[4] = {c.x, c.y, c.z, c.w};
                         fold.add_leaf(cc, leaf_present_mask(p, idx));
                     } else if (kind == REF_ACC) {
-                        fold.add_set(acc);
+                        uint32_t S[16];
+                        if (accns) {
+#pragma unroll
+                            for (int k = 0; k < 16; k++) S[k] = acc[k];
+                        } else {
+                            decode16(accc, S);
+                        }
+                        fold.add_set(S);
                     } else if (SPEC && kind == REF_CHAIN) {
                         if (!wait_flag(tc.done + idx, p.epoch, p.error, lane, tr)) return false;
                         uint32_t S[16];
-                        row_set16(tc.sets + (size_t)idx * 128, S);
+                        fitch_row16(p, tc, idx, lane, S);
                         fold.add_set(S);
                     } else {
                         uint32_t S[16];
+                        const uint32_t row = ref_row(p, ck, ref);
                         if (ni == 0 && fwd_set_prefetched(ref, op)) {
-                            stage_set16(st, S);
+                            const uint4 v = st[2 * 32];
+                            const uint32_t c[4] = {v.x, v.y, v.z, v.w};
+                            fitch_planes(p, fitch_stage_hdr(st, tc.hdr + row, lane), c, lane, S);
                         } else {
                             if (ref & REF_EXT) {
                                 if (!wait_dep(p, ck, tc.done, dc, int(idx), lane, tr)) return false;
                             }
-                            row_set16(tc.sets + (size_t)ref_row(p, ck, ref) * 128, S);
+                            fitch_row16(p, tc, row, lane, S);
                         }
                         ni++;
                         fold.add_set(S);
                     }
                 }
                 fold.finish(acc);
-            }
-            if ((w0.z & OPF_ROOT) && !(p.flags & RUN_BLOCK_MODE)) fitch_root_ref(p, tile, lane, acc);
-            store_set16(tc.sets + (size_t)op * 128, acc);
+                if (root_ref) fitch_root_ref(p, tile, lane, acc);
+                accns = fitch_encode(acc, accc);
+            }
+            fitch_store(p, pc, tc, op, lane, accc, accns, acc);
             if (w0.z & OPF_SIGNAL) signal_flag(tc.done + op, p.epoch, lane);
             if (op + FWD_DEPTH < ck.op_end) {
-                if (!fwd_issue<JS, 4>(p, ck, m, tc, dc, st, op + FWD_DEPTH, lane, tr)) return false;
+                if (!fwd_issue<1, 1>(p, ck, m, tc, dc, st, op + FWD_DEPTH, lane, tr)) return false;
             }
             stage = (stage + 1 == FWD_DEPTH) ? 0 : stage + 1;
         }
         if (spec) {
             if (!wait_flag(tc.done + ck.chain_row, p.epoch, p.error, lane, tr)) return false;
-            uint32_t S[16];
-            row_set16(tc.sets + (size_t)ck.chain_row * 128, S);
+            uint32_t S[16], c[4], ns;
+            fitch_row16(p, tc, uint32_t(ck.chain_row), lane, S);
             const int end = resolved >= 0 ? resolved : ck.op_end;
             int head = -1;
             for (int op = ck.chain_op; op < end; op++) {
@@ -677,7 +816,7 @@
                 fold.add_set(S);
                 fold.finish(S);
                 if ((w0.z & OPF_ROOT) && !(p.flags & RUN_BLOCK_MODE)) fitch_root_ref(p, tile, lane, S);
-                store_set16(tc.sets + (size_t)op * 128, S);
+                fitch_put(p, pc, tc, op, lane, S, c, ns);
                 if (w0.z & OPF_SIGNAL) signal_flag(tc.done + op, p.epoch, lane);
                 head = op;
             }
@@ -694,9 +833,10 @@
     uint4* ring = smem + (size_t)(threadIdx.x >> 5) * FITCH_FWD_PER_WARP;
     ItemIter it;
     TraceItem tr;
+    PoolCursor pc;
     int chunk, tile;
     while (next_item(p, it, chunk_begin, n_chunks, chunk, tile, lane, tr))
-        if (!fitch_forward_item<SPEC>(p, ring, chunk, tile, lane, tr)) return;
+        if (!fitch_forward_item<SPEC>(p, ring, pc, chunk, tile, lane, tr)) return;
 }
 
 template <int J>
@@ -786,15 +926,33 @@
     }
 }
 
-constexpr int FITCH_BWD_STAGE = (4 + 2) * 32,
-              FITCH_BWD_PER_WARP = BWD_DEPTH * FITCH_BWD_STAGE + BWD_META_U4 + BWD_STACK_U4 + (PMB_BULK ? (BWD_DEPTH * 8 + 15) / 16 : 0);
+constexpr int FITCH_BWD_SET_U4 = PMB_BULK ? 1 : 4, FITCH_BWD_STAGE = (FITCH_BWD_SET_U4 + 2) * 32,
+              FITCH_BWD_BARS_U4 = PMB_BULK ? (BWD_DEPTH * 8 + 15) / 16 : 0,
+              FITCH_BWD_PER_WARP = BWD_DEPTH * FITCH_BWD_STAGE + BWD_META_U4 + BWD_STACK_U4 + FITCH_BWD_BARS_U4 + META_OPS / 2;
+__device__ __forceinline__ void fitch_bwd_issue(const RunParams& p, const BwdMeta& m, const TileCtx& tc, uint4* st, int op, int lane) {
+    const uint2 h = m.hdr[op - m.lo];
+    if ((h.x >> lane) & 1u) {
+        const unsigned long long s = fitch_slot(h, lane);
+        if (s < p.set_pool_cap) {
+#pragma unroll
+            for (int j = 0; j < 4; j++) cp_async16(st + j * 32, p.set_pool + s * 4 + j);
+        }
+    } else {
+        cp_async16(st, tc.sets + (size_t)op * 32);
+    }
+    const int4 b1 = m.ops[2 * (op - m.lo) + 1];
+    if (b1.x > 0) cp_async16(st + 4 * 32, tc.leaf + (size_t)b1.z * 32);
+    if (b1.x > 1) cp_async16(st + 5 * 32, tc.leaf + (size_t)b1.w * 32);
+    cp_async_commit();
+}
 template <bool SPEC>
 __device__ __forceinline__ bool fitch_backward_item(const RunParams& p, uint4* ring, StageCursor& sc, int chunk, int tile, int lane,
                                                     TraceItem& tr, unsigned& phases) {
-    constexpr int J = 4, STAGE = FITCH_BWD_STAGE;
+    constexpr int J = 1, STAGE = FITCH_BWD_STAGE;
     BwdMeta m;
     m.ops = reinterpret_cast<int4*>(ring + BWD_DEPTH * STAGE);
     m.leaves = reinterpret_cast<int2*>(m.ops + 2 * META_OPS);
+    m.hdr = reinterpret_cast<uint2*>(ring + BWD_DEPTH * STAGE + BWD_META_U4 + BWD_STACK_U4 + FITCH_BWD_BARS_U4);
     uint32_t* stack = reinterpret_cast<uint32_t*>(ring + BWD_DEPTH * STAGE + BWD_META_U4);
     uint4* const ring_l = ring + lane;
 #if PMB_BULK
@@ -816,7 +974,7 @@
             for (int op = last; op >= ck.op_begin; op--) {
                 if (op != last && !(__ldg(&p.bwd_ops[op].flags) & OPF_HEAVY)) continue;
                 uint32_t S[16];
-                row_set16(tc.sets + (size_t)op * 128, S);
+                fitch_row16(p, tc, uint32_t(op), lane, S);
                 fitch_candidates_step(Q, S);
                 if (!__any_sync(FULL, candidates_open(Q) != 0)) {
                     resolved = op;
@@ -831,18 +989,19 @@
         for (int range = (resolved >= 0 ? 0 : 1); range < 2; range++) {
         const int hi = range == 0 ? resolved : last;
         const int lo = (range == 1 && resolved >= 0) ? resolved : ck.op_begin;
-        bwd_meta_load(p, m, hi, lo, lane);
+        bwd_meta_load(p, m, hi, lo, lane, tc.hdr);
 #if PMB_BULK
         for (int i = 0; i < BWD_DEPTH && hi - i >= lo; i++) bwd_issue_bulk<J>(m, sets_base, leaf_base, ring + i * STAGE, bars + i, hi - i, lane);
 #else
-        for (int i = 0; i < BWD_DEPTH && hi - i >= lo; i++) bwd_issue<J>(m, tc, ring_l + i * STAGE, hi - i);
+        for (int i = 0; i < BWD_DEPTH && hi - i >= lo; i++) fitch_bwd_issue(p, m, tc, ring_l + i * STAGE, hi - i, lane);
 #endif
         int stage = 0;
         for (int op = hi; op >= lo; op--) {
-            if (op - BWD_DEPTH < m.lo && m.lo > lo) bwd_meta_load(p, m, op, lo, lane);
+            if (op - BWD_DEPTH < m.lo && m.lo > lo) bwd_meta_load(p, m, op, lo, lane, tc.hdr);
             BwdHead h;
             h.b0 = m.ops[2 * (op - m.lo)];
             h.b1 = m.ops[2 * (op - m.lo) + 1];
+            const uint2 shdr = m.hdr[op - m.lo];
             const bool given = range == 0 && op == resolved, own_only = range == 1 && op == resolved;
             uint32_t P[4] = {0, 0, 0, 0}, pvis = 0, F[4], vis;
             if (given) {
@@ -864,11 +1023,23 @@
             cp_async_wait_stage<BWD_DEPTH>(op - lo);
 #endif
             uint4* st = ring_l + stage * STAGE;
+            const uint4 cv = st[0];
+            const uint32_t code[4] = {cv.x, cv.y, cv.z, cv.w};
             uint32_t S[16];
-#pragma unroll
-            for (int j = 0; j < 4; j++) {
-                const uint4 v = st[j * 32];
-                S[4 * j] = v.x; S[4 * j + 1] = v.y; S[4 * j + 2] = v.z; S[4 * j + 3] = v.w;
+            if (shdr.x != 0 || h.b0.y == PARENT_ROOT) {
+#if PMB_BULK
+                fitch_planes(p, shdr, code, lane, S);
+#else
+                if ((shdr.x >> lane) & 1u) {
+#pragma unroll
+                    for (int j = 0; j < 4; j++) {
+                        const uint4 v = st[j * 32];
+                        S[4 * j] = v.x; S[4 * j + 1] = v.y; S[4 * j + 2] = v.z; S[4 * j + 3] = v.w;
+                    }
+                } else {
+                    decode16(code, S);
+                }
+#endif
             }
             if (given) {
                 F[0] = specF[0]; F[1] = specF[1]; F[2] = specF[2]; F[3] = specF[3];
@@ -888,15 +1059,17 @@
                 } else {
                     fitch_assign_root(S, o4, ov_valid, colmask, F, vis);
                 }
+            } else if (shdr.x == 0) {
+                fitch_assign_single(code, pvis, F, vis);
             } else {
                 fitch_assign(S, P, pvis, F, vis);
             }
             if (own_only) emit(p, sc, h.b0.x, tile, lane, vis & differs4(F, P), P, F);
-            else bwd_finish_op(p, m, tc, sc, h, st + J * 32, stack, tile, lane, P, F, vis, false, !given);
+            else bwd_finish_op(p, m, tc, sc, h, st + FITCH_BWD_SET_U4 * 32, stack, tile, lane, P, F, vis, false, !given);
 #if PMB_BULK
             if (op - BWD_DEPTH >= lo) bwd_issue_bulk<J>(m, sets_base, leaf_base, ring + stage * STAGE, bars + stage, op - BWD_DEPTH, lane);
 #else
-            if (op - BWD_DEPTH >= lo) bwd_issue<J>(m, tc, st, op - BWD_DEPTH);
+            if (op - BWD_DEPTH >= lo) fitch_bwd_issue(p, m, tc, st, op - BWD_DEPTH, lane);
 #endif
             stage = (stage + 1 == BWD_DEPTH) ? 0 : stage + 1;
             accF[0] = F[0]; accF[1] = F[1]; accF[2] = F[2]; accF[3] = F[3];
@@ -1463,7 +1636,8 @@
                                                                 const uint16_t* staging, long long col_base, int32_t* pos,
                                                                 uint8_t* type_code, unsigned long long* counters,
                                                                 unsigned long long* run_words, unsigned long long staging_cap,
-                                                                unsigned long long* tickets, int n_tickets) {
+                                                                unsigned long long* tickets, int n_tickets,
+                                                                unsigned long long* set_pool_count, unsigned long long set_pool_cap) {
     __shared__ unsigned s_w[CPT_GROUP / 32];
     __shared__ unsigned s_last;
     const int tid = threadIdx.x, lane = tid & 31, warp = tid >> 5;
@@ -1522,11 +1696,14 @@
             unsigned int* error = reinterpret_cast<unsigned int*>(run_words + 1);
             unsigned int* sticky = reinterpret_cast<unsigned int*>(counters + 2);
             const unsigned long long pool = run_words[0];
-            const unsigned int er0 = error[0], er1 = error[1];
+            const unsigned long long slots = set_pool_count ? *set_pool_count : 0ull;
+            const unsigned int er0 = error[0] | (slots > set_pool_cap ? 8u : 0u), er1 = error[1];
             const unsigned int st = er0 | (pool > staging_cap ? 4u : 0u);
             if (st) sticky[0] |= st;
             if ((er0 & 1u) && er1 < sticky[1]) sticky[1] = er1;
             counters[4] = pool;
+            counters[6] = slots;
+            if (set_pool_count) *set_pool_count = 0ull;
             reinterpret_cast<unsigned int*>(counters + 5)[0] = er0;
             reinterpret_cast<unsigned int*>(counters + 5)[1] = er1;
             run_words[0] = 0ull;
@@ -1551,7 +1728,8 @@
 __global__ void pack_result_kernel(const long long* offsets, const int32_t* pos, const uint8_t* type_code, long long n_nodes,
                                    long long cap, long long src_cap, const unsigned long long* counters, unsigned char* out) {
     const long long total = offsets[n_nodes];
-    const bool ok = total >= 0 && total <= cap && total <= src_cap && counters[4] <= (unsigned long long)src_cap;
+    const bool ok = total >= 0 && total <= cap && total <= src_cap && counters[4] <= (unsigned long long)src_cap &&
+                    !(reinterpret_cast<const unsigned int*>(counters + 5)[0] & 8u);
     const long long n = ok ? total : 0;
     long long* hdr = reinterpret_cast<long long*>(out);
     long long* off_out = hdr + 2;
```

After: 2527 billion, median of 6. About the same (-0.7%).
